# QualityMinds/cistgcn

Measured on AMD Instinct MI355X. Metric: sequences/sec (fwd+bwd) H3.6M 22-joint 50->25, higher is better.
Workload: dtype f32; 1 GPU; cistgcn64_b256_t50_v22; C=64, per_gpu_batch=256, global_batch=256, T_in=50, T_out=25, V=22, parallelism=dp1, graph=True, graph_branches=True, capture_kept=median, mixed_batches=False

## Files before the change

cistgcn_amd/_lib.py:

```python
import ctypes
import os
from ctypes import POINTER, c_double, c_float, c_int, c_int32, c_longlong, c_uint, c_ulonglong, c_void_p

HERE = os.path.dirname(os.path.abspath(__file__))
LIB_PATH = os.path.join(HERE, "libcistgcn_hip.so")

_handle = None
STAT_REPLICAS = 16
ALPHA_SLOTS = 64
_host_pointers_ok = False


class View4(ctypes.Structure):
    _fields_ = [("n", c_longlong * 4), ("s", c_longlong * 4)]


class NormAct(ctypes.Structure):
    _fields_ = [
        ("x", c_void_p), ("xv", View4),
        ("y", c_void_p), ("yv", View4),
        ("pre", c_void_p),
        ("add", c_void_p), ("av", View4),
        ("add_post", c_int),
        ("bn_mode", c_int),
        ("stats", c_void_p),
        ("gamma", c_void_p), ("beta", c_void_p),
        ("running_mean", c_void_p), ("running_var", c_void_p), ("num_batches_tracked", c_void_p),
        ("momentum", c_float), ("eps", c_float),
        ("save_mean", c_void_p), ("save_rstd", c_void_p),
        ("drop_p", c_float), ("seed", c_void_p), ("salt", c_uint),
        ("alpha", c_void_p), ("alpha_n", c_int),
        ("dy", c_void_p), ("dyv", View4),
        ("dx", c_void_p), ("dxv", View4),
        ("dadd", c_void_p), ("dav", View4),
        ("dpre", c_void_p),
        ("red", c_void_p),
        ("dgamma", c_void_p), ("dbeta", c_void_p), ("dalpha", c_void_p),
        ("ystats", c_void_p),
    ]


class ContractDesc(ctypes.Structure):
    _fields_ = [("A", c_void_p), ("X", c_void_p), ("Y", c_void_p), ("bias", c_void_p), ("stats", c_void_p), ("tab", c_void_p),
                ("G", c_int), ("M", c_int), ("N", c_int), ("K", c_int), ("splitk", c_int), ("kchunk", c_int),
                ("a_kfast", c_int), ("x_kfast", c_int), ("accumulate", c_int), ("x_vec", c_int), ("stat_ch", c_int), ("mode", c_int), ("block0", c_longlong),
                ("ws", c_void_p), ("chain", c_int), ("pad2", c_int)]


class StatsArgs(ctypes.Structure):
    _fields_ = [("x", c_void_p), ("xv", View4), ("pre", c_void_p), ("stats", c_void_p)]


class SumItem(ctypes.Structure):
    _fields_ = [("a", c_void_p), ("av", View4)]


class Rank1(ctypes.Structure):
    _fields_ = [("s", c_void_p), ("q", c_void_p), ("o", c_void_p), ("dout", c_void_p), ("ds", c_void_p), ("dq", c_void_p),
                ("domain", c_int), ("pad", c_int)]


class CopyItem(ctypes.Structure):
    _fields_ = [("y", c_void_p), ("yv", View4), ("a", c_void_p), ("av", View4)]


class TailBN(ctypes.Structure):
    _fields_ = [("stats", c_void_p), ("gamma", c_void_p), ("beta", c_void_p), ("running_mean", c_void_p), ("running_var", c_void_p),
                ("num_batches_tracked", c_void_p), ("momentum", c_float), ("eps", c_float), ("save", c_void_p)]


class DstdTail(ctypes.Structure):
    _fields_ = [("B", c_int), ("C", c_int), ("T", c_int), ("V", c_int), ("train", c_int), ("pad0", c_int),
                ("y", c_void_p * 2), ("r", c_void_p * 2), ("w", c_void_p * 2),
                ("bn_t", TailBN * 2), ("alpha_d", c_void_p * 2),
                ("bn_p", TailBN * 2), ("alpha_p", c_void_p * 2),
                ("Wc", c_void_p), ("bn_c", TailBN), ("alpha_c", c_void_p),
                ("gate", c_void_p), ("bres", c_void_p),
                ("drop_p", c_float), ("salt", c_uint * 2), ("pad1", c_int), ("seed", c_void_p),
                ("h0", c_void_p), ("pooled", c_void_p), ("out", c_void_p), ("ostats", c_void_p),
                ("tap_x", c_void_p * 2), ("tap_a", c_void_p * 2), ("tap_h", c_void_p),
                ("dout", c_void_p), ("dpooled", c_void_p), ("dgate", c_void_p), ("red_c", c_void_p),
                ("gp", c_void_p * 2), ("red_p", c_void_p * 2), ("dWc_ws", c_void_p), ("dWc", c_void_p),
                ("dr", c_void_p * 2), ("dw", c_void_p * 2), ("red_t", c_void_p * 2), ("dy", c_void_p * 2),
                ("dgamma_t", c_void_p * 2), ("dbeta_t", c_void_p * 2), ("dalpha_d", c_void_p * 2),
                ("dgamma_p", c_void_p * 2), ("dbeta_p", c_void_p * 2), ("dalpha_p", c_void_p * 2),
                ("dgamma_c", c_void_p), ("dbeta_c", c_void_p), ("dalpha_c", c_void_p)]


class AdjTail(ctypes.Structure):
    _fields_ = [("B", c_int), ("Kc", c_int), ("J", c_int), ("domain", c_int), ("train", c_int), ("pad0", c_int),
                ("s", c_void_p), ("q", c_void_p), ("W0", c_void_p), ("bn", TailBN), ("alpha", c_void_p), ("W4", c_void_p),
                ("drop_p", c_float), ("salt", c_uint), ("seed", c_void_p),
                ("e", c_void_p), ("adj", c_void_p), ("tap", c_void_p),
                ("dadj", c_void_p), ("g", c_void_p), ("red", c_void_p), ("ds", c_void_p), ("dq", c_void_p), ("part", c_void_p),
                ("dW0_ws", c_void_p), ("dW4_ws", c_void_p),
                ("dW0", c_void_p), ("dW4", c_void_p), ("dgamma", c_void_p), ("dbeta", c_void_p), ("dalpha", c_void_p)]


class PwMaps(ctypes.Structure):
    _fields_ = [("B", c_int), ("Cin", c_int), ("P", c_int), ("n", c_int), ("x", c_void_p),
                ("W", c_void_p * 4), ("M", c_int * 4), ("y", c_void_p * 4), ("stats", c_void_p * 4),
                ("dy", c_void_p * 4), ("dx", c_void_p), ("dW", c_void_p * 4), ("dW_ws", c_void_p),
                ("bias", c_void_p * 4), ("db", c_void_p * 4),
                ("yraw", c_void_p * 4), ("bn_save", c_void_p * 4), ("bn_gamma", c_void_p * 4), ("bn_beta", c_void_p * 4),
                ("bn_red", c_void_p * 4), ("prelu", c_void_p * 4), ("bn_train", c_int), ("pad", c_int)]


class FpnConv(ctypes.Structure):
    _fields_ = [("B", c_int), ("C", c_int), ("O", c_int), ("H", c_int), ("W", c_int), ("n", c_int), ("dil", c_int * 3), ("pad", c_int),
                ("x", c_void_p), ("xs", c_longlong * 3), ("w", c_void_p * 3), ("bias", c_void_p * 3), ("y", c_void_p * 3),
                ("dy", c_void_p * 3), ("dx", c_void_p), ("dw", c_void_p * 3), ("db", c_void_p * 3), ("ws", c_void_p)]


class RowsConv(ctypes.Structure):
    _fields_ = [("B", c_int), ("C", c_int), ("T", c_int), ("V", c_int), ("O", c_int), ("pad", c_int),
                ("x", c_void_p), ("W", c_void_p), ("y", c_void_p), ("stats", c_void_p),
                ("dy", c_void_p), ("dx", c_void_p), ("dW", c_void_p), ("ws", c_void_p),
                ("in_on", c_int), ("in_train", c_int), ("in_bn", TailBN), ("in_alpha", c_void_p), ("in_tap", c_void_p),
                ("sums", c_void_p), ("red", c_void_p), ("dgamma", c_void_p), ("dbeta", c_void_p), ("dalpha", c_void_p)]


class BlockInput(ctypes.Structure):
    _fields_ = [("B", c_int), ("C", c_int), ("T", c_int), ("V", c_int), ("train", c_int), ("ng", c_int),
                ("x", c_void_p), ("bn", TailBN), ("xn", c_void_p), ("rm", c_void_p), ("rq", c_void_p), ("out", c_void_p),
                ("g", c_void_p * 8), ("dout", c_void_p * 2), ("dout_ld", c_longlong * 2), ("pq", c_void_p), ("gsum", c_void_p), ("red", c_void_p),
                ("dx", c_void_p), ("dgamma", c_void_p), ("dbeta", c_void_p)]


class GatePath(ctypes.Structure):
    _fields_ = [("z", c_void_p), ("stats", c_void_p), ("stats_ld", c_longlong),
                ("bn2", TailBN), ("alpha2", c_void_p), ("Wl", c_void_p), ("bn3", TailBN), ("alpha3", c_void_p), ("W2", c_void_p),
                ("salt2", c_uint), ("salt3", c_uint), ("y", c_void_p), ("w", c_void_p), ("tap2", c_void_p), ("tap3", c_void_p),
                ("dw", c_void_p), ("dz", c_void_p), ("dstats", c_void_p), ("dWl", c_void_p), ("dW2", c_void_p),
                ("dgamma2", c_void_p), ("dbeta2", c_void_p), ("dalpha2", c_void_p), ("dgamma3", c_void_p), ("dbeta3", c_void_p), ("dalpha3", c_void_p),
                ("scratch", c_void_p), ("red", c_void_p)]


class GateHead(ctypes.Structure):
    _fields_ = [("B", c_int), ("C", c_int), ("S", c_int), ("train", c_int), ("n", c_int), ("pad", c_int),
                ("drop_p", c_float), ("pad2", c_int), ("seed", c_void_p), ("p", GatePath * 2)]


class MidItem(ctypes.Structure):
    _fields_ = [("kind", c_int), ("C", c_int), ("L", c_int), ("O", c_int), ("sb_", c_int), ("ns_", c_int),
                ("x", c_void_p), ("x_ld", c_longlong), ("bn", TailBN), ("stats_ld", c_longlong), ("alpha", c_void_p), ("W", c_void_p),
                ("salt", c_uint), ("pad", c_int), ("y", c_void_p), ("tap", c_void_p),
                ("dy", c_void_p), ("dx", c_void_p), ("dW", c_void_p), ("dgamma", c_void_p), ("dbeta", c_void_p), ("dalpha", c_void_p),
                ("g", c_void_p), ("part", c_void_p), ("wpart", c_void_p)]


class BlockMid(ctypes.Structure):
    _fields_ = [("B", c_int), ("train", c_int), ("n", c_int), ("pad", c_int),
                ("drop_p", c_float), ("pad2", c_int), ("seed", c_void_p), ("it", MidItem * 6)]


class CtxHeads(ctypes.Structure):
    _fields_ = [("B", c_int), ("P", c_int), ("C", c_int), ("train", c_int), ("x", c_void_p), ("xstats", c_void_p),
                ("w", c_void_p * 2), ("bn", TailBN * 2), ("alpha", c_void_p * 2),
                ("y", c_void_p * 2), ("arg", c_void_p), ("xsave", c_void_p), ("tap", c_void_p * 2),
                ("dy", c_void_p * 2), ("red", c_void_p), ("dx", c_void_p),
                ("dw", c_void_p * 2), ("dgamma", c_void_p * 2), ("dbeta", c_void_p * 2), ("dalpha", c_void_p * 2)]


class AttackStep(ctypes.Structure):
    _fields_ = [("B", c_int), ("T", c_int), ("V", c_int), ("mode", c_int), ("iterations", c_int), ("patience", c_int),
                ("epsilon", c_float), ("mu", c_float),
                ("x0", c_void_p), ("x", c_void_p), ("grad", c_void_p), ("g", c_void_p), ("mask", c_void_p), ("loss", c_void_p),
                ("best", c_void_p), ("stall", c_void_p), ("active", c_void_p), ("w", c_void_p), ("queries", c_void_p), ("n_active", c_void_p),
                ("steps", c_void_p), ("frozen_at", c_void_p)]


class DeepfoolStep(ctypes.Structure):
    _fields_ = [("B", c_int), ("T", c_int), ("To", c_int), ("V", c_int), ("patience", c_int), ("pad", c_int),
                ("x", c_void_p), ("grad", c_void_p), ("pred", c_void_p), ("mask", c_void_p), ("loss", c_void_p),
                ("best", c_void_p), ("stall", c_void_p), ("active", c_void_p), ("w", c_void_p), ("queries", c_void_p), ("n_active", c_void_p),
                ("steps", c_void_p), ("frozen_at", c_void_p)]


class EvalMetricsArgs(ctypes.Structure):
    _fields_ = [("B", c_int), ("To", c_int), ("J", c_int), ("Nb", c_int), ("frames", c_int), ("pad", c_int),
                ("pred", c_void_p), ("target", c_void_p), ("speeds", c_void_p), ("bones", c_void_p),
                ("out", c_void_p * 9), ("ws", c_void_p)]


class AttackMetricsArgs(ctypes.Structure):
    _fields_ = [("B", c_int), ("T", c_int), ("J", c_int), ("pad", c_int),
                ("adv", c_void_p), ("orig", c_void_p), ("out", c_void_p * 33), ("counts", c_void_p), ("gmax", c_void_p), ("ws", c_void_p)]


P = c_void_p
LL = c_longlong
_SIGNATURES = {
    "cg_contract": [P, P, P, P, P, P, c_int, c_int, c_int, c_int, c_int, c_int, c_int, LL, P],
    "cg_contract_many": [POINTER(ContractDesc), c_int, P],
    "cg_contract_kred_ws_floats": [c_int, c_int, c_int],
    "cg_chan_stats": [P, POINTER(View4), P, P, P],
    "cg_chan_stats_many": [POINTER(StatsArgs), c_int, P],
    "cg_norm_act_fwd_many": [POINTER(NormAct), c_int, P],
    "cg_norm_act_bwd_many": [POINTER(NormAct), POINTER(c_int), c_int, P],
    "cg_norm_act_bwd_reduce_many": [POINTER(NormAct), c_int, P],
    "cg_copy_many": [POINTER(CopyItem), c_int, P],
    "cg_chan_sum": [P, POINTER(View4), P, P],
    "cg_norm_act_fwd": [POINTER(NormAct), P],
    "cg_norm_act_bwd": [POINTER(NormAct), c_int, P],
    "cg_reduce_bc": [P, POINTER(View4), c_int, P, P, P],
    "cg_reduce_bc_bwd": [P, P, c_int, P, POINTER(View4), P],
    "cg_sum_many": [P, POINTER(View4), POINTER(SumItem), c_int, P],
    "cg_rank1_adj_fwd": [POINTER(Rank1), c_int, c_int, c_int, c_int, P],
    "cg_rank1_adj_bwd": [POINTER(Rank1), c_int, c_int, c_int, c_int, P],
    "cg_gather_joints": [P, P, P, LL, c_int, c_int, P],
    "cg_eval_scatter_mpjpe": [P, P, P, P, P, c_int, c_int, c_int, c_int, P],
    "cg_add3": [P, POINTER(View4), P, POINTER(View4), P, POINTER(View4), P, POINTER(View4), P],
    "cg_zero": [P, LL, P],
    "cg_feature_lift_fwd": [P, P, LL, LL, LL, P],
    "cg_feature_lift_bwd": [P, P, P, LL, LL, LL, P],
    "cg_dstd_stats_fwd": [P, P, c_int, c_int, c_int, c_int, P],
    "cg_dstd_stats_bwd": [P, P, P, c_int, c_int, c_int, c_int, P],
    "cg_se_gate_fwd": [P, P, P, P, c_int, c_int, c_int, P],
    "cg_se_gate_bwd": [P, P, P, P, P, P, P, P, c_int, c_int, c_int, c_int, P],
    "cg_cumsum": [P, POINTER(View4), P, POINTER(View4), c_int, P],
    "cg_mpjpe_fwd": [P, P, P, LL, P],
    "cg_mpjpe_bwd": [P, P, P, P, LL, P],
    "cg_seed_bump": [P, P],
    "cg_stgcn_domain_fwd": [P, P, P, P, P, P, c_int, c_int, c_int, c_int, c_int, c_int, P],
    "cg_stgcn_domain_bwd": [P, P, P, P, P, P, P, P, P, c_int, c_int, c_int, c_int, c_int, c_int, c_int, P],
    "cg_stgcn_domain_bwd_ws_floats": [c_int, c_int],
    "cg_stgcn_domain_planes_min_workgroups": [c_longlong],
    "cg_multi_copy": [P, P, P, P, P, c_int, P, c_int, c_float, P],
    "cg_scale": [P, LL, c_float, P],
    "cg_dstd_tail_fwd": [POINTER(DstdTail), c_int, P],
    "cg_dstd_tail_bwd": [POINTER(DstdTail), c_int, P],
    "cg_dstd_tail_ws_floats": [c_int],
    "cg_collapse_rows_fwd": [POINTER(RowsConv), P],
    "cg_collapse_rows_bwd": [POINTER(RowsConv), P],
    "cg_collapse_rows_ws_floats": [c_int, c_int, c_int],
    "cg_collapse_cols_fwd": [POINTER(RowsConv), P],
    "cg_collapse_cols_bwd": [POINTER(RowsConv), P],
    "cg_collapse_cols_supported": [c_int, c_int, c_int, c_int],
    "cg_collapse_cols_ws_floats": [c_int, c_int, c_int],
# ... 82 lines not shown
```

cistgcn_amd/csrc/dstd_tail.h:

```cpp
#pragma once

#define CG_TAIL_MAXW 8

struct CgTailBN {
  double* stats;
  const float* gamma; const float* beta;
  float* running_mean; float* running_var; long long* num_batches_tracked;
  float momentum, eps;
  float* save;
};

struct CgDstdTail {
  int B, C, T, V, train, pad0;
  const float* y[2];
  const float* r[2];
  const float* w[2];
  CgTailBN bn_t[2]; const float* alpha_d[2];
  CgTailBN bn_p[2]; const float* alpha_p[2];
  const float* Wc; CgTailBN bn_c; const float* alpha_c;
  const float* gate; const float* bres;
  float drop_p; unsigned int salt[2]; int pad1; const unsigned long long* seed;
  float* h0; float* pooled; float* out; double* ostats;
  float* tap_x[2]; float* tap_a[2]; float* tap_h;
  const float* dout; const float* dpooled; float* dgate;
  double* red_c;
  float* gp[2]; double* red_p[2];
  float* dWc_ws; float* dWc;
  float* dr[2]; float* dw[2]; double* red_t[2]; float* dy[2];
  float* dgamma_t[2]; float* dbeta_t[2]; float* dalpha_d[2];
  float* dgamma_p[2]; float* dbeta_p[2]; float* dalpha_p[2];
  float* dgamma_c; float* dbeta_c; float* dalpha_c;
};
```

cistgcn_amd/csrc/dstd_tail.hip:

```cpp
#include "cg_common.h"
#include "dstd_tail.h"
#include "cg_phase.h"
#include <stdlib.h>

HIP_DYNAMIC_SHARED(unsigned char, cg_dyn_lds)

static int cg_tail_rows(long long B, long long C, long long P) {
  long long target = (B * C * P) / 2048;
  target = target < 4096 ? 4096 : (target > 32768 ? 32768 : target);
  long long rb = target / (P > 0 ? P : 1);
  if (rb < 1) rb = 1;
  if (rb > B) rb = B;
  while (rb > 1 && C * ((B + rb - 1) / rb) < 512) rb = (rb + 1) / 2;
  return (int)rb;
}

__device__ __forceinline__ float cg_tail_x(const CgAff& at, float alpha_d, float y, float r, float keep, float& u) {
  u = cg_bn(at, y) * keep + r;
  return cg_prelu(u, alpha_d);
}

__device__ __forceinline__ float cg_tail_keep(const CgDstdTail& t, int i, unsigned long long seed, int b, int c, int p) {
  if (!(t.train && t.drop_p > 0.f)) return 1.f;
  const long long P = (long long)t.T * t.V;
  return cg_drop_scale(t.drop_p, seed, t.salt[i], ((unsigned long long)b * t.C + c) * P + p);
}

__device__ __forceinline__ void cg_tail_keep4(const CgDstdTail& t, int i, unsigned long long seed, unsigned long long idx0, float keep[4]);

__global__ void cg_tail_f1_kernel(CgDstdTail t, int rb) {
  __shared__ double red[32];
  const int i = blockIdx.z, c = blockIdx.x, b0 = blockIdx.y * rb;
  if (b0 >= t.B) return;
  const int P = t.T * t.V, nb = min(rb, t.B - b0), C = t.C;
  const int lane = threadIdx.x & 63, wave = __builtin_amdgcn_readfirstlane(threadIdx.x >> 6), nw = blockDim.x >> 6;
  const double cnt = (double)t.B * P;
  const CgAff at = cg_tail_aff(t.bn_t[i], c, C, cnt, t.train, false, blockIdx.y == 0 && threadIdx.x == 0);
  const float ad = t.alpha_d[i][0];
  const unsigned long long seed = (t.train && t.drop_p > 0.f) ? *t.seed : 0ull;
  const float* __restrict__ y = t.y[i]; const float* __restrict__ r = t.r[i];
  float* const tap = t.tap_x[i];
  double s = 0.0, q = 0.0;
  for (int br = wave; br < nb; br += nw) {
    const int b = b0 + br;
    const long long base = ((long long)b * C + c) * P;
    const float wv = t.w[i][(long long)b * C + c];
    if ((P & 3) == 0) {
      for (int p = 4 * lane; p < P; p += 256) {
        float keep[4];
        cg_tail_keep4(t, i, seed, (unsigned long long)(base + p), keep);
        const float4 y4 = *reinterpret_cast<const float4*>(y + base + p), r4 = *reinterpret_cast<const float4*>(r + base + p);
        const float yv[4] = {y4.x, y4.y, y4.z, y4.w}, rv[4] = {r4.x, r4.y, r4.z, r4.w};
        float xv[4];
#pragma unroll
        for (int j = 0; j < 4; ++j) {
          float u;
          xv[j] = cg_tail_x(at, ad, yv[j], rv[j], keep[j], u);
          const double z = (double)(wv * xv[j]);
          s += z; q += z * z;
        }
        if (tap) *reinterpret_cast<float4*>(tap + base + p) = make_float4(xv[0], xv[1], xv[2], xv[3]);
      }
    } else {
      for (int p = lane; p < P; p += 64) {
        float u;
        const float x = cg_tail_x(at, ad, y[base + p], r[base + p], cg_tail_keep(t, i, seed, b, c, p), u);
        const float z = wv * x;
        if (tap) tap[base + p] = x;
        s += (double)z; q += (double)z * (double)z;
      }
    }
  }
  s = cg_block_sum(s, red);
  q = cg_block_sum(q, red + 16);
  if (threadIdx.x == 0) {
    double* rep = t.bn_p[i].stats + (long long)(blockIdx.y % CG_STAT_REPLICAS) * 2 * C;
    atomicAdd(&rep[2 * c], s); atomicAdd(&rep[2 * c + 1], q);
  }
}

#define CG_TAIL_PT 64
#define CG_TAIL_PS (CG_TAIL_PT + 4)
#define CG_TAIL_THREADS 256
#define CG_TAIL_PT3 32
#define CG_TAIL_PS3 (CG_TAIL_PT3 + 4)
#define CG_TAIL_K3_TASKS 2

__device__ __forceinline__ void cg_tail_consts(const CgDstdTail& t, float* sK, bool backward, bool owner) {
  const int C = t.C;
  const double cnt = (double)t.B * t.T * t.V;
  for (int e = threadIdx.x; e < 2 * C; e += blockDim.x) {
    const int i = e / C, c = e - i * C;
    const CgAff at = cg_tail_aff(t.bn_t[i], c, C, cnt, t.train, backward || t.train != 0, owner);
    const CgAff ap = cg_tail_aff(t.bn_p[i], c, C, cnt, t.train, backward, owner);
    float* k = sK + 8 * e;
    k[0] = at.mean; k[1] = at.gamma * at.rstd; k[2] = at.beta; k[3] = t.alpha_d[i][0];
    k[4] = ap.mean; k[5] = ap.rstd; k[6] = ap.gamma; k[7] = ap.beta;
  }
}

struct CgTailHot {
  int C, P, train;
  float drop_p;
  unsigned int salt[2];
  float alpha_p[2];
  float* tap_a[2]; float* tap_x[2];
};
__device__ __forceinline__ CgTailHot cg_tail_hot(const CgDstdTail& t) {
  CgTailHot h;
  h.C = t.C; h.P = t.T * t.V; h.train = t.train; h.drop_p = t.drop_p;
#pragma unroll
  for (int i = 0; i < 2; ++i) {
    h.salt[i] = t.salt[i];
    h.alpha_p[i] = __builtin_bit_cast(float, __builtin_amdgcn_readfirstlane(__builtin_bit_cast(int, t.alpha_p[i][0])));
    h.tap_a[i] = t.tap_a[i]; h.tap_x[i] = t.tap_x[i];
  }
  return h;
}
__device__ __forceinline__ void cg_tail_keep4(const CgTailHot& h, int i, unsigned long long seed, unsigned long long idx0, float keep[4]) {
  if (!(h.train && h.drop_p > 0.f)) { keep[0] = keep[1] = keep[2] = keep[3] = 1.f; return; }
  const unsigned long long bits = cg_drop_bits(seed, h.salt[i], idx0 >> 2);
#pragma unroll
  for (int j = 0; j < 4; ++j) keep[j] = cg_drop_pick(bits, j, h.drop_p);
}

__device__ __forceinline__ void cg_tail_keep4(const CgDstdTail& t, int i, unsigned long long seed, unsigned long long idx0, float keep[4]) {
  if (!(t.train && t.drop_p > 0.f)) { keep[0] = keep[1] = keep[2] = keep[3] = 1.f; return; }
  const unsigned long long bits = cg_drop_bits(seed, t.salt[i], idx0 >> 2);
#pragma unroll
  for (int j = 0; j < 4; ++j) keep[j] = cg_drop_pick(bits, j, t.drop_p);
}

template <int PT>
__device__ __forceinline__ void cg_tail_act_load(const CgDstdTail& t, int b, int p0, int np, float4 yq[PT / 8], float4 rq[PT / 8], float wq[PT / 8]) {
  const int C = t.C, P = t.T * t.V;
#pragma unroll
  for (int q = 0; q < PT / 8; ++q) {
    const int i = q / (PT / 16), e = threadIdx.x + (q - i * (PT / 16)) * CG_TAIL_THREADS;
    const int c = e / (PT / 4), pp = 4 * (e - c * (PT / 4));
    yq[q] = make_float4(0.f, 0.f, 0.f, 0.f); rq[q] = yq[q]; wq[q] = 0.f;
    if (c < C && pp < np) {
      const float* yb = t.y[i] + (long long)b * C * P + p0;
      const float* rb = t.r[i] + (long long)b * C * P + p0;
      const int off = c * P + pp;
      yq[q] = *reinterpret_cast<const float4*>(yb + off); rq[q] = *reinterpret_cast<const float4*>(rb + off);
      wq[q] = t.w[i][(long long)b * C + c];
    }
  }
}

__device__ __forceinline__ float cg_tail_pre_p(float z, float mean, float rstd, float gamma, float beta) {
  const float zhat = (z - mean) * rstd;
  return gamma * zhat + beta;
}

template <int PT>
__device__ __forceinline__ void cg_tail_act_finish(const CgTailHot& t, const float* sK, unsigned long long seed, int b, int p0, int np,
                                                   const float4 yq[PT / 8], const float4 rq[PT / 8], const float wq[PT / 8], float* img, int what) {
  constexpr int PS = PT + 4;
  const int C = t.C, P = t.P;
#pragma unroll
  for (int q = 0; q < PT / 8; ++q) {
    const int i = q / (PT / 16), e = threadIdx.x + (q - i * (PT / 16)) * CG_TAIL_THREADS;
    const int c = e / (PT / 4), pp = 4 * (e - c * (PT / 4)), c2 = i * C + c;
    if (c >= C) continue;
    float val[4] = {0.f, 0.f, 0.f, 0.f};
    if (pp < np) {
      const float4 k0 = *reinterpret_cast<const float4*>(sK + 8 * c2), k1 = *reinterpret_cast<const float4*>(sK + 8 * c2 + 4);
      const long long off = ((long long)b * C + c) * P + p0 + pp;
      const float yv[4] = {yq[q].x, yq[q].y, yq[q].z, yq[q].w}, rv[4] = {rq[q].x, rq[q].y, rq[q].z, rq[q].w};
      float keep[4];
      cg_tail_keep4(t, i, seed, (unsigned long long)off, keep);
      const float wv = wq[q], ap = t.alpha_p[i];
      float xv[4];
#pragma unroll
      for (int j = 0; j < 4; ++j) {
        const float u = ((yv[j] - k0.x) * k0.y + k0.z) * keep[j] + rv[j];
        xv[j] = cg_prelu(u, k0.w);
        const float z = wv * xv[j];
        val[j] = what == 0 ? cg_prelu(cg_tail_pre_p(z, k1.x, k1.y, k1.z, k1.w), ap) : (z - k1.x) * k1.y;
      }
      if (what == 0) {
        if (t.tap_a[i]) *reinterpret_cast<float4*>(t.tap_a[i] + off) = make_float4(val[0], val[1], val[2], val[3]);
        if (!t.train && t.tap_x[i]) *reinterpret_cast<float4*>(t.tap_x[i] + off) = make_float4(xv[0], xv[1], xv[2], xv[3]);
      }
    }
    *reinterpret_cast<float4*>(img + c2 * PS + pp) = make_float4(val[0], val[1], val[2], val[3]);
  }
}

template <int PT>
__device__ __forceinline__ void cg_tail_stage_act(const CgDstdTail& t, const float* sK, unsigned long long seed, int b, int p0, int np,
                                                  float* img, int what) {
  constexpr int PS = PT + 4;
  const int C = t.C, P = t.T * t.V;
  if ((P & 3) == 0) {
#pragma unroll
    for (int i = 0; i < 2; ++i)
#pragma unroll 2
    for (int e = threadIdx.x; e < C * (PT / 4); e += CG_TAIL_THREADS) {
      const int c = e / (PT / 4), pp = 4 * (e - c * (PT / 4)), c2 = i * C + c;
      float val[4] = {0.f, 0.f, 0.f, 0.f};
      if (pp < np) {
        const int p = p0 + pp;
        const float4 k0 = *reinterpret_cast<const float4*>(sK + 8 * c2), k1 = *reinterpret_cast<const float4*>(sK + 8 * c2 + 4);
        const long long off = ((long long)b * C + c) * P + p;
        const float4 y4 = *reinterpret_cast<const float4*>(t.y[i] + off), r4 = *reinterpret_cast<const float4*>(t.r[i] + off);
        const float yv[4] = {y4.x, y4.y, y4.z, y4.w}, rv[4] = {r4.x, r4.y, r4.z, r4.w};
        float keep[4];
        cg_tail_keep4(t, i, seed, (unsigned long long)off, keep);
        const float wv = t.w[i][(long long)b * C + c], ap = t.alpha_p[i][0];
        float xv[4];
#pragma unroll
        for (int j = 0; j < 4; ++j) {
          const float u = ((yv[j] - k0.x) * k0.y + k0.z) * keep[j] + rv[j];
          xv[j] = cg_prelu(u, k0.w);
          const float z = wv * xv[j];
          val[j] = what == 0 ? cg_prelu(cg_tail_pre_p(z, k1.x, k1.y, k1.z, k1.w), ap) : (z - k1.x) * k1.y;
        }
        if (what == 0) {
          if (t.tap_a[i]) *reinterpret_cast<float4*>(t.tap_a[i] + off) = make_float4(val[0], val[1], val[2], val[3]);
          if (!t.train && t.tap_x[i]) *reinterpret_cast<float4*>(t.tap_x[i] + off) = make_float4(xv[0], xv[1], xv[2], xv[3]);
        }
      }
      *reinterpret_cast<float4*>(img + c2 * PS + pp) = make_float4(val[0], val[1], val[2], val[3]);
    }
    return;
  }
  for (int e = threadIdx.x; e < 2 * C * PT; e += CG_TAIL_THREADS) {
    const int c2 = e / PT, pp = e - c2 * PT;
    float val = 0.f;
    if (pp < np) {
      const int i = c2 / C, c = c2 - i * C, p = p0 + pp;
      const float* k = sK + 8 * c2;
      const long long off = ((long long)b * C + c) * P + p;
      const float keep = cg_tail_keep(t, i, seed, b, c, p);
      const float u = ((t.y[i][off] - k[0]) * k[1] + k[2]) * keep + t.r[i][off];
      const float z = t.w[i][(long long)b * C + c] * cg_prelu(u, k[3]);
      if (what == 0) {
        val = cg_prelu(cg_tail_pre_p(z, k[4], k[5], k[6], k[7]), t.alpha_p[i][0]);
        if (t.tap_a[i]) t.tap_a[i][off] = val;
        if (!t.train && t.tap_x[i]) t.tap_x[i][off] = cg_prelu(u, k[3]);
      }
      else val = (z - k[4]) * k[5];
    }
    img[c2 * PS + pp] = val;
  }
}

template <int MT_, int NT2_>
__global__ __launch_bounds__(CG_TAIL_THREADS, 2) void cg_tail_f2_kernel(CgDstdTail t, int tiles_per_sample, int total, int per) {
  const int C = t.C, C2 = 2 * C, CM = MT_ ? 16 * MT_ : (C + 15) & ~15, C2M = NT2_ ? 16 * NT2_ : (C2 + 15) & ~15, P = t.T * t.V;
  const int WS = C2M + 4;
  float* sAct = reinterpret_cast<float*>(cg_dyn_lds);
  float* sW = sAct + C2M * CG_TAIL_PS;
  float* sK = sW + CM * WS;
  double* sStat = reinterpret_cast<double*>(sK + 8 * C2M);
  const int tid = threadIdx.x, lane = tid & 63, wave = __builtin_amdgcn_readfirstlane(tid >> 6), l15 = lane & 15, slot = lane >> 4;
  const int wg = blockIdx.x;
  if (wg * per >= total) return;
  for (int e = tid; e < C2M * CG_TAIL_PS + CM * WS; e += CG_TAIL_THREADS) sAct[e] = 0.f;
  for (int e = tid; e < 2 * CM; e += CG_TAIL_THREADS) sStat[e] = 0.0;
  __syncthreads();
  for (int e = tid; e < C * C2; e += CG_TAIL_THREADS) { const int co = e / C2, c2 = e - co * C2; sW[co * WS + c2] = t.Wc[e]; }
  cg_tail_consts(t, sK, false, wg == 0);
  const unsigned long long seed = (t.train && t.drop_p > 0.f) ? *t.seed : 0ull;
  const CgTailHot hot = cg_tail_hot(t);
  const int MT = CM / 16;
  constexpr int nw = CG_TAIL_THREADS / 64;
  const bool vec = (P & 3) == 0;
  float4 yq[CG_TAIL_PT / 8], rq[CG_TAIL_PT / 8];
  float wq[CG_TAIL_PT / 8];
  double fsum[MT_ ? (2 * MT_ + nw - 1) / nw : 1][2];
#pragma unroll
  for (int i = 0; i < (MT_ ? (2 * MT_ + nw - 1) / nw : 1); ++i) fsum[i][0] = fsum[i][1] = 0.0;
  if (vec) {
    const int lid = wg * per, b = lid / tiles_per_sample, p0 = (lid - b * tiles_per_sample) * CG_TAIL_PT;
    cg_tail_act_load<CG_TAIL_PT>(t, b, p0, min(CG_TAIL_PT, P - p0), yq, rq, wq);
  }
  for (int it = 0; it < per; ++it) {
    const int lid = wg * per + it;
    if (lid >= total) break;
    const int b = lid / tiles_per_sample, tile = lid - b * tiles_per_sample, p0 = tile * CG_TAIL_PT, np = min(CG_TAIL_PT, P - p0);
    __syncthreads();
    if (vec) cg_tail_act_finish<CG_TAIL_PT>(hot, sK, seed, b, p0, np, yq, rq, wq, sAct, 0);
    else cg_tail_stage_act<CG_TAIL_PT>(t, sK, seed, b, p0, np, sAct, 0);
    __syncthreads();
    if (vec && it + 1 < per && lid + 1 < total) {
      const int l2 = lid + 1, b2 = l2 / tiles_per_sample, q0 = (l2 - b2 * tiles_per_sample) * CG_TAIL_PT;
      cg_tail_act_load<CG_TAIL_PT>(t, b2, q0, min(CG_TAIL_PT, P - q0), yq, rq, wq);
    }
    float* hb = t.h0 + (long long)b * C * P + p0;
    constexpr int NTASK = MT_ ? (2 * MT_ + nw - 1) / nw : 1;
    cg_f32x4 facc[NTASK][2];
    if (MT_) {
#pragma unroll
      for (int ti = 0; ti < NTASK; ++ti) facc[ti][0] = facc[ti][1] = cg_f32x4{0.f, 0.f, 0.f, 0.f};
      if (2 * MT_ >= nw || wave < 2 * MT_) {
        const int n0 = 32 * (wave & 1);
#pragma unroll
        for (int k0 = 0; k0 < 16 * NT2_; k0 += 16) {
          float b0v[4], b1v[4];
          cg_tfrag<1>(cg_tfrag_ptr<1>(sAct + n0, CG_TAIL_PS, l15, slot), CG_TAIL_PS, k0, b0v);
          cg_tfrag<1>(cg_tfrag_ptr<1>(sAct + n0 + 16, CG_TAIL_PS, l15, slot), CG_TAIL_PS, k0, b1v);
#pragma unroll
          for (int ti = 0; ti < NTASK; ++ti) {
            float av[4];
            cg_tfrag<0>(cg_tfrag_ptr<0>(sW + 16 * ((wave >> 1) + (nw / 2) * ti) * WS, WS, l15, slot), WS, k0, av);
#pragma unroll
            for (int s = 0; s < 4; ++s) {
              facc[ti][0] = __builtin_amdgcn_mfma_f32_16x16x4f32(b0v[s], av[s], facc[ti][0], 0, 0, 0);
              facc[ti][1] = __builtin_amdgcn_mfma_f32_16x16x4f32(b1v[s], av[s], facc[ti][1], 0, 0, 0);
            }
          }
        }
      }
    }
#pragma unroll
    for (int ti = 0; ti < (MT_ ? NTASK : 2); ++ti) {
      const int w = wave + nw * ti;
      if (w >= MT * 2) break;
      const int mt = w >> 1, n0 = 32 * (w & 1), n1 = n0 + 16;
      cg_f32x4 c0 = cg_f32x4{0.f, 0.f, 0.f, 0.f}, c1 = c0;
      if (MT_) { c0 = facc[MT_ ? ti : 0][0]; c1 = facc[MT_ ? ti : 0][1]; }
      else {
        const float* ap = cg_tfrag_ptr<0>(sW + 16 * mt * WS, WS, l15, slot);
        const float* bp0 = cg_tfrag_ptr<1>(sAct + n0, CG_TAIL_PS, l15, slot);
        const float* bp1 = cg_tfrag_ptr<1>(sAct + n1, CG_TAIL_PS, l15, slot);
        for (int k0 = 0; k0 < C2M; k0 += 16) {
          float av[4], b0v[4], b1v[4];
          cg_tfrag<0>(ap, WS, k0, av); cg_tfrag<1>(bp0, CG_TAIL_PS, k0, b0v); cg_tfrag<1>(bp1, CG_TAIL_PS, k0, b1v);
#pragma unroll
          for (int s = 0; s < 4; ++s) {
            c0 = __builtin_amdgcn_mfma_f32_16x16x4f32(b0v[s], av[s], c0, 0, 0, 0);
            c1 = __builtin_amdgcn_mfma_f32_16x16x4f32(b1v[s], av[s], c1, 0, 0, 0);
          }
        }
      }
      const int co = 16 * mt + l15;
      const bool cok = co < C;
      float s1 = 0.f, s2 = 0.f;
#pragma unroll
      for (int h = 0; h < 2; ++h) {
        const int pq = (h ? n1 : n0) + 4 * slot;
        const cg_f32x4 cc = h ? c1 : c0;
        if (cok && pq < np) {
          float* dst = hb + (long long)co * P + pq;
          if (vec) *reinterpret_cast<float4*>(dst) = make_float4(cc[0], cc[1], cc[2], cc[3]);
#pragma unroll
          for (int q = 0; q < 4; ++q) {
            if (pq + q < np) {
              if (!vec) dst[q] = cc[q];
              s1 += cc[q]; s2 += cc[q] * cc[q];
            }
          }
        }
      }
      if (t.train) {
        if (MT_) { fsum[MT_ ? ti : 0][0] += (double)s1; fsum[MT_ ? ti : 0][1] += (double)s2; }
        else {
          s1 += __shfl_xor(s1, 16, 64); s2 += __shfl_xor(s2, 16, 64);
          s1 += __shfl_xor(s1, 32, 64); s2 += __shfl_xor(s2, 32, 64);
          if (slot == 0 && cok) { atomicAdd(&sStat[2 * co], (double)s1); atomicAdd(&sStat[2 * co + 1], (double)s2); }
        }
      }
    }
  }
  if (t.train && MT_) {
#pragma unroll
    for (int ti = 0; ti < (MT_ ? (2 * MT_ + nw - 1) / nw : 1); ++ti) {
      const int w = wave + nw * ti, co = 16 * (w >> 1) + l15;
      if (w < MT * 2 && co < C) { atomicAdd(&sStat[2 * co], fsum[ti][0]); atomicAdd(&sStat[2 * co + 1], fsum[ti][1]); }
    }
  }
  if (t.train) {
    __syncthreads();
    double* rep = t.bn_c.stats + (long long)(blockIdx.x % CG_STAT_REPLICAS) * 2 * C;
    for (int e = tid; e < 2 * C; e += CG_TAIL_THREADS) atomicAdd(&rep[e], sStat[e]);
  }
}

__global__ void cg_tail_f3_kernel(CgDstdTail t, int rb) {
  const int c = blockIdx.x, b0 = blockIdx.y * rb, P = t.T * t.V, C = t.C;
  if (b0 >= t.B) return;
  const int nb = min(rb, t.B - b0), lane = threadIdx.x & 63, wave = __builtin_amdgcn_readfirstlane(threadIdx.x >> 6), nw = blockDim.x >> 6;
  const CgAff ac = cg_tail_aff(t.bn_c, c, C, (double)t.B * P, t.train, false, blockIdx.y == 0 && threadIdx.x == 0);
  const float alpha = t.alpha_c[0];
  for (int br = wave; br < nb; br += nw) {
    const int b = b0 + br;
    const float* __restrict__ h0 = t.h0 + ((long long)b * C + c) * P;
    float s = 0.f;
    if ((P & 3) == 0) {
      for (int p = 4 * lane; p < P; p += 256) {
        const float4 h4 = *reinterpret_cast<const float4*>(h0 + p);
        s += (cg_prelu(cg_bn(ac, h4.x), alpha) + cg_prelu(cg_bn(ac, h4.y), alpha)) + (cg_prelu(cg_bn(ac, h4.z), alpha) + cg_prelu(cg_bn(ac, h4.w), alpha));
      }
    } else {
      for (int p = lane; p < P; p += 64) s += cg_prelu(cg_bn(ac, h0[p]), alpha);
    }
    const double sd = cg_wave_sum((double)s);
    if (lane == 0) t.pooled[(long long)b * C + c] = (float)(sd / (double)P);
  }
}

__global__ void cg_tail_f4_kernel(CgDstdTail t, int rb) {
  __shared__ double red[32];
  const int c = blockIdx.x, b0 = blockIdx.y * rb;
  if (b0 >= t.B) return;
  const int P = t.T * t.V, nb = min(rb, t.B - b0), C = t.C;
  const int lane = threadIdx.x & 63, wave = __builtin_amdgcn_readfirstlane(threadIdx.x >> 6), nw = blockDim.x >> 6;
  const CgAff ac = cg_tail_aff(t.bn_c, c, C, (double)t.B * P, t.train, true, false);
  const float alpha = t.alpha_c[0];
  float* const tap = t.tap_h;
  double s = 0.0, q = 0.0;
  for (int br = wave; br < nb; br += nw) {
    const int b = b0 + br;
    const long long base = ((long long)b * C + c) * P;
    const float gate = t.gate[(long long)b * C + c];
    if ((P & 3) == 0) {
      for (int p = 4 * lane; p < P; p += 256) {
        const float4 h4 = *reinterpret_cast<const float4*>(t.h0 + base + p), r4 = *reinterpret_cast<const float4*>(t.bres + base + p);
        const float hv[4] = {h4.x, h4.y, h4.z, h4.w}, rv[4] = {r4.x, r4.y, r4.z, r4.w};
        float h[4], v[4];
#pragma unroll
        for (int j = 0; j < 4; ++j) { h[j] = cg_prelu(cg_bn(ac, hv[j]), alpha); v[j] = h[j] * gate + rv[j]; s += (double)v[j]; q += (double)v[j] * (double)v[j]; }
        if (tap) *reinterpret_cast<float4*>(tap + base + p) = make_float4(h[0], h[1], h[2], h[3]);
        *reinterpret_cast<float4*>(t.out + base + p) = make_float4(v[0], v[1], v[2], v[3]);
      }
    } else {
      for (int p = lane; p < P; p += 64) {
        const float h = cg_prelu(cg_bn(ac, t.h0[base + p]), alpha);
        if (tap) tap[base + p] = h;
        const float v = h * gate + t.bres[base + p];
        t.out[base + p] = v;
        s += (double)v; q += (double)v * (double)v;
      }
    }
  }
  if (t.ostats) {
    s = cg_block_sum(s, red);
    q = cg_block_sum(q, red + 16);
    if (threadIdx.x == 0) {
      double* rep = t.ostats + (long long)(blockIdx.y % CG_STAT_REPLICAS) * 2 * C;
      atomicAdd(&rep[2 * c], s); atomicAdd(&rep[2 * c + 1], q);
    }
  }
}

__global__ void cg_tail_k1_kernel(CgDstdTail t, int rb) {
  const int c = blockIdx.x, b0 = blockIdx.y * rb, P = t.T * t.V, C = t.C;
  if (b0 >= t.B) return;
  const int nb = min(rb, t.B - b0), lane = threadIdx.x & 63, wave = __builtin_amdgcn_readfirstlane(threadIdx.x >> 6), nw = blockDim.x >> 6;
  const CgAff ac = cg_tail_aff(t.bn_c, c, C, 0.0, t.train, true, false);
  const float alpha = t.alpha_c[0];
  for (int br = wave; br < nb; br += nw) {
    const int b = b0 + br;
    const long long base = ((long long)b * C + c) * P;
    float s = 0.f;
    if ((P & 3) == 0) {
      for (int p = 4 * lane; p < P; p += 256) {
        const float4 d4 = *reinterpret_cast<const float4*>(t.dout + base + p), h4 = *reinterpret_cast<const float4*>(t.h0 + base + p);
        s += (d4.x * cg_prelu(cg_bn(ac, h4.x), alpha) + d4.y * cg_prelu(cg_bn(ac, h4.y), alpha)) +
             (d4.z * cg_prelu(cg_bn(ac, h4.z), alpha) + d4.w * cg_prelu(cg_bn(ac, h4.w), alpha));
      }
    } else {
      for (int p = lane; p < P; p += 64) s += t.dout[base + p] * cg_prelu(cg_bn(ac, t.h0[base + p]), alpha);
    }
    const double sd = cg_wave_sum((double)s);
    if (lane == 0) t.dgate[(long long)b * C + c] = (float)sd;
  }
}

__device__ __forceinline__ float cg_tail_gc(const CgDstdTail& t, const CgAff& ac, float alpha, long long off, int b, int c, float invP, float& u) {
  u = cg_bn(ac, t.h0[off]);
  const float dh = t.dout[off] * t.gate[(long long)b * t.C + c] + t.dpooled[(long long)b * t.C + c] * invP;
  return u > 0.f ? dh : alpha * dh;
}

__global__ void cg_tail_k2_kernel(CgDstdTail t, int rb) {
  __shared__ double red[48];
  const int c = blockIdx.x, b0 = blockIdx.y * rb;
  if (b0 >= t.B) return;
  const int P = t.T * t.V, nb = min(rb, t.B - b0), C = t.C;
  const int lane = threadIdx.x & 63, wave = __builtin_amdgcn_readfirstlane(threadIdx.x >> 6), nw = blockDim.x >> 6;
  const CgAff ac = cg_tail_aff(t.bn_c, c, C, 0.0, t.train, true, false);
  const float alpha = t.alpha_c[0], invP = 1.f / (float)P;
  double s1 = 0.0, s2 = 0.0, sa = 0.0;
  for (int br = wave; br < nb; br += nw) {
    const int b = b0 + br;
    const long long base = ((long long)b * C + c) * P;
    const float gate = t.gate[(long long)b * C + c], dp = t.dpooled[(long long)b * C + c] * invP;
    if ((P & 3) == 0) {
      for (int p = 4 * lane; p < P; p += 256) {
        const float4 d4 = *reinterpret_cast<const float4*>(t.dout + base + p), h4 = *reinterpret_cast<const float4*>(t.h0 + base + p);
        const float dv[4] = {d4.x, d4.y, d4.z, d4.w}, hv[4] = {h4.x, h4.y, h4.z, h4.w};
#pragma unroll
        for (int j = 0; j < 4; ++j) {
          const float u = cg_bn(ac, hv[j]), dh = dv[j] * gate + dp;
          const float g = u > 0.f ? dh : alpha * dh;
          s1 += (double)g; s2 += (double)g * (double)((hv[j] - ac.mean) * ac.rstd);
          sa += u > 0.f ? 0.0 : (double)dh * (double)u;
        }
      }
    } else {
      for (int p = lane; p < P; p += 64) {
        float u;
        const float g = cg_tail_gc(t, ac, alpha, base + p, b, c, invP, u);
        s1 += (double)g;
        s2 += (double)g * (double)((t.h0[base + p] - ac.mean) * ac.rstd);
        if (!(u > 0.f)) sa += (double)(t.dout[base + p] * gate + dp) * (double)u;
      }
    }
  }
  s1 = cg_block_sum(s1, red); s2 = cg_block_sum(s2, red + 16); sa = cg_block_sum(sa, red + 32);
  if (threadIdx.x == 0) {
    atomicAdd(&t.red_c[2 * c], s1); atomicAdd(&t.red_c[2 * c + 1], s2); atomicAdd(&t.red_c[2 * C + ((c + 5 * (int)blockIdx.y) & (CG_ALPHA_SLOTS - 1))], sa);
  }
}

#ifdef CG_TAIL_STAMPS
__device__ unsigned long long* cg_tail_stamp_buf = nullptr;
extern "C" int cg_tail_set_stamps(void* p) { return (int)hipMemcpyToSymbol(HIP_SYMBOL(cg_tail_stamp_buf), &p, sizeof(p)); }
#define CG_TSTAMP()                                                                                     \
  do {                                                                                                  \
    if (threadIdx.x == 0 && cg_tail_stamp_buf && nst < 255) cg_tail_stamp_buf[blockIdx.x * 256 + (++nst)] = __builtin_amdgcn_s_memtime(); \
  } while (0)
#define CG_TSTAMP_END() do { if (threadIdx.x == 0 && cg_tail_stamp_buf) cg_tail_stamp_buf[blockIdx.x * 256] = nst; } while (0)
#else
#define CG_TSTAMP() do { } while (0)
#define CG_TSTAMP_END() do { } while (0)
#endif

template <int MT_, int NT2_>
__global__ __launch_bounds__(CG_TAIL_THREADS, 2) void cg_tail_k3_kernel(CgDstdTail t, int tiles_per_sample, int total, int per, int replicas) {
  const int C = t.C, C2 = 2 * C, CM = MT_ ? 16 * MT_ : (C + 15) & ~15, C2M = NT2_ ? 16 * NT2_ : (C2 + 15) & ~15, P = t.T * t.V;
  const int WS = C2M + 4;
  float* sZ = reinterpret_cast<float*>(cg_dyn_lds);
  float* sDH = sZ + C2M * CG_TAIL_PS3;
  float* sW = sDH + CM * CG_TAIL_PS3;
  float* sK = sW + CM * WS;
  float* sKc = sK + 8 * C2M;
  double* sRed = reinterpret_cast<double*>(sKc + 8 * CM);
  const int tid = threadIdx.x, lane = tid & 63, wave = __builtin_amdgcn_readfirstlane(tid >> 6), l15 = lane & 15, slot = lane >> 4, nw = CG_TAIL_THREADS / 64;
  const int wg = blockIdx.x;
  if (wg * per >= total) return;
  int nst = 0; (void)nst;
  CG_TSTAMP();
  for (int e = tid; e < C2M * CG_TAIL_PS3 + CM * CG_TAIL_PS3 + CM * WS; e += CG_TAIL_THREADS) sZ[e] = 0.f;
  for (int e = tid; e < 2 * C2M + 2; e += CG_TAIL_THREADS) sRed[e] = 0.0;
  __syncthreads();
  for (int e = tid; e < C * C2; e += CG_TAIL_THREADS) { const int co = e / C2, c2 = e - co * C2; sW[co * WS + c2] = t.Wc[e]; }
  cg_tail_consts(t, sK, true, false);
  const double cnt = (double)t.B * P;
  for (int c = tid; c < C; c += CG_TAIL_THREADS) {
    const CgAff ac = cg_tail_aff(t.bn_c, c, C, 0.0, t.train, true, false);
    float* kc = sKc + 8 * c;
    kc[0] = ac.mean; kc[1] = ac.rstd; kc[2] = ac.gamma * ac.rstd; kc[3] = ac.beta;
    kc[4] = t.train ? (float)(t.red_c[2 * c] / cnt) : 0.f; kc[5] = t.train ? (float)(t.red_c[2 * c + 1] / cnt) : 0.f;
  }
  const unsigned long long seed = (t.train && t.drop_p > 0.f) ? *t.seed : 0ull;
  const CgTailHot hot = cg_tail_hot(t);
  const bool train = t.train != 0;
  float* const gp0 = t.gp[0]; float* const gp1 = t.gp[1];
  const int MT = CM / 16, NT2 = C2M / 16;
  const float invP = 1.f / (float)P;
  cg_f32x4 wacc[CG_TAIL_MAXW];
#pragma unroll
  for (int u = 0; u < CG_TAIL_MAXW; ++u) wacc[u] = cg_f32x4{0.f, 0.f, 0.f, 0.f};
  const float alpha_c = t.alpha_c[0];
  const float alpha_p0 = t.alpha_p[0][0], alpha_p1 = t.alpha_p[1][0];
  float racc[CG_TAIL_K3_TASKS][3];
#pragma unroll
  for (int i = 0; i < CG_TAIL_K3_TASKS * 3; ++i) (&racc[0][0])[i] = 0.f;
  CG_TSTAMP();
  const bool vec = (P & 3) == 0;
  constexpr int DQ = CG_TAIL_PT3 / 16;
  float4 yq[CG_TAIL_PT3 / 8], rq[CG_TAIL_PT3 / 8];
  float wq[CG_TAIL_PT3 / 8];
  float4 h4[DQ], d4[DQ];
  float gt[DQ], dp[DQ];
  auto dh_load = [&](int b, int p0, int np) {
#pragma unroll
    for (int q = 0; q < DQ; ++q) {
      const int e = tid + q * CG_TAIL_THREADS, c = e / (CG_TAIL_PT3 / 4), pp = 4 * (e - c * (CG_TAIL_PT3 / 4));
      h4[q] = make_float4(0.f, 0.f, 0.f, 0.f); d4[q] = h4[q]; gt[q] = 0.f; dp[q] = 0.f;
      if (c < C && pp < np) {
        const long long off = ((long long)b * C + c) * P + p0 + pp;
        h4[q] = *reinterpret_cast<const float4*>(t.h0 + off); d4[q] = *reinterpret_cast<const float4*>(t.dout + off);
        gt[q] = t.gate[(long long)b * C + c]; dp[q] = t.dpooled[(long long)b * C + c];
      }
    }
  };
  if (vec) {
    const int lid = wg * per, b = lid / tiles_per_sample, p0 = (lid - b * tiles_per_sample) * CG_TAIL_PT3;
    cg_tail_act_load<CG_TAIL_PT3>(t, b, p0, min(CG_TAIL_PT3, P - p0), yq, rq, wq);
    dh_load(b, p0, min(CG_TAIL_PT3, P - p0));
  }
  for (int it = 0; it < per; ++it) {
    const int lid = wg * per + it;
    if (lid >= total) break;
    const int b = lid / tiles_per_sample, tile = lid - b * tiles_per_sample, p0 = tile * CG_TAIL_PT3, np = min(CG_TAIL_PT3, P - p0);
    __syncthreads();
    CG_TSTAMP();
    if (vec) {
      cg_tail_act_finish<CG_TAIL_PT3>(hot, sK, seed, b, p0, np, yq, rq, wq, sZ, 1);
      CG_TSTAMP();
#pragma unroll
      for (int q = 0; q < DQ; ++q) {
        const int e = tid + q * CG_TAIL_THREADS, c = e / (CG_TAIL_PT3 / 4), pp = 4 * (e - c * (CG_TAIL_PT3 / 4));
        if (c >= C) continue;
        float val[4] = {0.f, 0.f, 0.f, 0.f};
        if (pp < np) {
          const float4 kcA = *reinterpret_cast<const float4*>(sKc + 8 * c);
          const float2 kcB = *reinterpret_cast<const float2*>(sKc + 8 * c + 4);
          const float hv[4] = {h4[q].x, h4[q].y, h4[q].z, h4[q].w}, dv[4] = {d4[q].x, d4[q].y, d4[q].z, d4[q].w};
#pragma unroll
          for (int j = 0; j < 4; ++j) {
            const float u = (hv[j] - kcA.x) * kcA.z + kcA.w;
            const float dh = dv[j] * gt[q] + dp[q] * invP;
            const float g = u > 0.f ? dh : alpha_c * dh;
            val[j] = train ? kcA.z * (g - kcB.x - (hv[j] - kcA.x) * kcA.y * kcB.y) : g * kcA.z;
          }
        }
        *reinterpret_cast<float4*>(sDH + c * CG_TAIL_PS3 + pp) = make_float4(val[0], val[1], val[2], val[3]);
      }
    } else {
      cg_tail_stage_act<CG_TAIL_PT3>(t, sK, seed, b, p0, np, sZ, 1);
      CG_TSTAMP();
      for (int e = tid; e < C * CG_TAIL_PT3; e += CG_TAIL_THREADS) {
        const int c = e / CG_TAIL_PT3, pp = e - c * CG_TAIL_PT3;
        float val = 0.f;
        if (pp < np) {
          const float* kc = sKc + 8 * c;
          const long long off = ((long long)b * C + c) * P + p0 + pp;
          const float hv = t.h0[off];
          const float u = (hv - kc[0]) * kc[2] + kc[3];
          const float dh = t.dout[off] * t.gate[(long long)b * C + c] + t.dpooled[(long long)b * C + c] * invP;
          const float g = u > 0.f ? dh : alpha_c * dh;
          val = t.train ? kc[2] * (g - kc[4] - (hv - kc[0]) * kc[1] * kc[5]) : g * kc[2];
        }
        sDH[c * CG_TAIL_PS3 + pp] = val;
      }
    }
    __syncthreads();
    if (vec && it + 1 < per && lid + 1 < total) {
      const int b2 = (lid + 1) / tiles_per_sample, q0 = (lid + 1 - b2 * tiles_per_sample) * CG_TAIL_PT3;
      cg_tail_act_load<CG_TAIL_PT3>(t, b2, q0, min(CG_TAIL_PT3, P - q0), yq, rq, wq);
      dh_load(b2, q0, min(CG_TAIL_PT3, P - q0));
    }
    CG_TSTAMP();
    if (MT_) {
      constexpr int G = NT2_ >= nw ? NT2_ / nw : 1;
      static_assert(NT2_ == 0 || NT2_ % nw == 0 || (NT2_ < nw && MT_ == 1), "tile split of the four waves");
      if (NT2_ >= nw || wave < NT2_) {
#pragma unroll
        for (int k0 = 0; k0 < CG_TAIL_PT3; k0 += 16) {
          float afr[G][4];
#pragma unroll
          for (int g = 0; g < G; ++g) {
            const int n2 = g * nw + wave, c2 = 16 * n2 + l15;
            const bool cok = c2 < C2;
            const float gam = cok ? sK[8 * c2 + 6] : 0.f, bet = cok ? sK[8 * c2 + 7] : 0.f, alp = cok ? (c2 >= C ? alpha_p1 : alpha_p0) : 0.f;
            float bv[4];
            cg_tfrag<0>(cg_tfrag_ptr<0>(sZ + 16 * n2 * CG_TAIL_PS3, CG_TAIL_PS3, l15, slot), CG_TAIL_PS3, k0, bv);
#pragma unroll
            for (int s = 0; s < 4; ++s) afr[g][s] = cg_prelu(gam * bv[s] + bet, alp);
          }
#pragma unroll
          for (int mt = 0; mt < (MT_ ? MT_ : 1); ++mt) {
            float av[4];
            cg_tfrag<0>(cg_tfrag_ptr<0>(sDH + 16 * mt * CG_TAIL_PS3, CG_TAIL_PS3, l15, slot), CG_TAIL_PS3, k0, av);
#pragma unroll
            for (int g = 0; g < G; ++g)
#pragma unroll
              for (int s = 0; s < 4; ++s)
                wacc[mt * G + g] = __builtin_amdgcn_mfma_f32_16x16x4f32(av[s], afr[g][s], wacc[mt * G + g], 0, 0, 0);
          }
        }
      }
    } else {
#pragma unroll
    for (int u = 0; u < CG_TAIL_MAXW; ++u) {      const int id = u * nw + wave;
      if (id < MT * NT2) {
        const int mt = id / NT2, n2 = id - mt * NT2, c2 = 16 * n2 + l15;
        const int i = c2 >= C ? 1 : 0, c = c2 - i * C;
        const bool cok = c2 < C2;
        const float gam = cok ? sK[8 * c2 + 6] : 0.f, bet = cok ? sK[8 * c2 + 7] : 0.f, alp = cok ? (i ? alpha_p1 : alpha_p0) : 0.f;
        (void)c;
        const float* ap = cg_tfrag_ptr<0>(sDH + 16 * mt * CG_TAIL_PS3, CG_TAIL_PS3, l15, slot);
        const float* bp = cg_tfrag_ptr<0>(sZ + 16 * n2 * CG_TAIL_PS3, CG_TAIL_PS3, l15, slot);
        for (int k0 = 0; k0 < CG_TAIL_PT3; k0 += 16) {
          float av[4], bv[4];
          cg_tfrag<0>(ap, CG_TAIL_PS3, k0, av); cg_tfrag<0>(bp, CG_TAIL_PS3, k0, bv);
#pragma unroll
          for (int s = 0; s < 4; ++s) {
            const float a = cg_prelu(gam * bv[s] + bet, alp);
            wacc[u] = __builtin_amdgcn_mfma_f32_16x16x4f32(av[s], a, wacc[u], 0, 0, 0);
          }
        }
      }
    }
    }
    CG_TSTAMP();
    static_assert(CG_TAIL_PT3 == 32, "one pair of position tiles per task: task w = channel tile w");
    cg_f32x4 dacc[CG_TAIL_K3_TASKS][2];
    if (MT_) {
#pragma unroll
      for (int ti = 0; ti < CG_TAIL_K3_TASKS; ++ti) dacc[ti][0] = dacc[ti][1] = cg_f32x4{0.f, 0.f, 0.f, 0.f};
      if (NT2_ >= nw || wave < NT2_) {
#pragma unroll
        for (int k0 = 0; k0 < 16 * (MT_ ? MT_ : 1); k0 += 16) {
          float b0v[4], b1v[4];
          cg_tfrag<1>(cg_tfrag_ptr<1>(sDH, CG_TAIL_PS3, l15, slot), CG_TAIL_PS3, k0, b0v);
          cg_tfrag<1>(cg_tfrag_ptr<1>(sDH + 16, CG_TAIL_PS3, l15, slot), CG_TAIL_PS3, k0, b1v);
#pragma unroll
          for (int ti = 0; ti < CG_TAIL_K3_TASKS; ++ti) {
            if (nw * ti >= NT2_ && ti > 0) break;
            float av[4];
            cg_tfrag<1>(cg_tfrag_ptr<1>(sW + 16 * (wave + nw * ti), WS, l15, slot), WS, k0, av);
#pragma unroll
            for (int s = 0; s < 4; ++s) {
              dacc[ti][0] = __builtin_amdgcn_mfma_f32_16x16x4f32(b0v[s], av[s], dacc[ti][0], 0, 0, 0);
              dacc[ti][1] = __builtin_amdgcn_mfma_f32_16x16x4f32(b1v[s], av[s], dacc[ti][1], 0, 0, 0);
            }
          }
        }
      }
    }
#pragma unroll
    for (int ti = 0; ti < CG_TAIL_K3_TASKS; ++ti) {
      const int w = wave + nw * ti;
      if (w >= NT2 * (CG_TAIL_PT3 / 32)) break;
      const int mt = w / (CG_TAIL_PT3 / 32), n0 = 32 * (w % (CG_TAIL_PT3 / 32)), n1 = n0 + 16;
      cg_f32x4 c0 = cg_f32x4{0.f, 0.f, 0.f, 0.f}, c1 = c0;
      if (MT_) { c0 = dacc[ti][0]; c1 = dacc[ti][1]; }
      else {
        const float* ap = cg_tfrag_ptr<1>(sW + 16 * mt, WS, l15, slot);
        const float* bp0 = cg_tfrag_ptr<1>(sDH + n0, CG_TAIL_PS3, l15, slot);
        const float* bp1 = cg_tfrag_ptr<1>(sDH + n1, CG_TAIL_PS3, l15, slot);
        for (int k0 = 0; k0 < CM; k0 += 16) {
          float av[4], b0v[4], b1v[4];
          cg_tfrag<1>(ap, WS, k0, av); cg_tfrag<1>(bp0, CG_TAIL_PS3, k0, b0v); cg_tfrag<1>(bp1, CG_TAIL_PS3, k0, b1v);
#pragma unroll
          for (int s = 0; s < 4; ++s) {
            c0 = __builtin_amdgcn_mfma_f32_16x16x4f32(b0v[s], av[s], c0, 0, 0, 0);
            c1 = __builtin_amdgcn_mfma_f32_16x16x4f32(b1v[s], av[s], c1, 0, 0, 0);
          }
        }
      }
      const int c2 = 16 * mt + l15;
      const bool cok = c2 < C2;
      const int i = c2 >= C ? 1 : 0, c = cok ? c2 - i * C : 0;
      const float gam = cok ? sK[8 * c2 + 6] : 0.f, bet = cok ? sK[8 * c2 + 7] : 0.f, alp = cok ? (i ? alpha_p1 : alpha_p0) : 0.f;
      float* gpr = (i ? gp1 : gp0) + ((long long)b * C + c) * P + p0;
#pragma unroll
      for (int h = 0; h < 2; ++h) {
        const int pq = (h ? n1 : n0) + 4 * slot;
        const cg_f32x4 cc = h ? c1 : c0;
        if (cok && pq < np) {
          const float4 z4 = *reinterpret_cast<const float4*>(sZ + c2 * CG_TAIL_PS3 + pq);
          const float zh[4] = {z4.x, z4.y, z4.z, z4.w};
          float gq[4];
#pragma unroll
          for (int q = 0; q < 4; ++q) {
            const float v = gam * zh[q] + bet, da = cc[q];
            const bool in = pq + q < np;
            gq[q] = v > 0.f ? da : alp * da;
            if (in) {
              racc[ti][0] += gq[q]; racc[ti][1] += gq[q] * zh[q];
              if (!(v > 0.f)) racc[ti][2] += da * v;
            }
          }
          if (vec) *reinterpret_cast<float4*>(gpr + pq) = make_float4(gq[0], gq[1], gq[2], gq[3]);
          else {
#pragma unroll
            for (int q = 0; q < 4; ++q) if (pq + q < np) gpr[pq + q] = gq[q];
          }
        }
      }
    }
  }
  CG_TSTAMP();
#pragma unroll
  for (int ti = 0; ti < CG_TAIL_K3_TASKS; ++ti) {
    const int w = wave + nw * ti;
    if (w >= NT2 * (CG_TAIL_PT3 / 32)) break;
    const int c2 = 16 * (w / (CG_TAIL_PT3 / 32)) + l15;
    float s1 = racc[ti][0], s2 = racc[ti][1], sa = racc[ti][2];
    s1 += __shfl_xor(s1, 16, 64); s2 += __shfl_xor(s2, 16, 64); sa += __shfl_xor(sa, 16, 64);
    s1 += __shfl_xor(s1, 32, 64); s2 += __shfl_xor(s2, 32, 64); sa += __shfl_xor(sa, 32, 64);
    if (slot == 0 && c2 < C2) {
      atomicAdd(&sRed[2 * c2], (double)s1); atomicAdd(&sRed[2 * c2 + 1], (double)s2); atomicAdd(&sRed[2 * C2M + (c2 >= C ? 1 : 0)], (double)sa);
    }
  }
  __syncthreads();
  for (int e = tid; e < 2 * C2; e += CG_TAIL_THREADS) {
    const int c2 = e >> 1, i = c2 >= C ? 1 : 0, c = c2 - i * C;
    atomicAdd(&t.red_p[i][2 * c + (e & 1)], sRed[e]);
  }
  if (tid < 2) atomicAdd(&t.red_p[tid][2 * C + ((int)blockIdx.x & (CG_ALPHA_SLOTS - 1))], sRed[2 * C2M + tid]);
  float* dW = t.dWc_ws + (long long)(blockIdx.x % replicas) * C * C2;
#pragma unroll
  for (int u = 0; u < CG_TAIL_MAXW; ++u) {
    const int id = u * nw + wave;
    if (id < MT * NT2) {
      const int mt = id / NT2, n2 = id - mt * NT2;
#pragma unroll
      for (int q = 0; q < 4; ++q) {
        const int co = 16 * mt + 4 * slot + q, c2 = 16 * n2 + l15;
        if (co < C && c2 < C2) atomicAdd(&dW[co * C2 + c2], wacc[u][q]);
      }
    }
  }
  CG_TSTAMP();
  CG_TSTAMP_END();
}

__global__ void cg_tail_k4_kernel(CgDstdTail t, int rb) {
  const int i = blockIdx.z, c = blockIdx.x, b0 = blockIdx.y * rb, P = t.T * t.V;
  if (b0 >= t.B) return;
  const int nb = min(rb, t.B - b0), lane = threadIdx.x & 63, wave = __builtin_amdgcn_readfirstlane(threadIdx.x >> 6), nw = blockDim.x >> 6;
  const double cnt = (double)t.B * P;
  const CgAff at = cg_tail_aff(t.bn_t[i], c, t.C, 0.0, t.train, true, false);
  const CgAff ap = cg_tail_aff(t.bn_p[i], c, t.C, 0.0, t.train, true, false);
  const float ad = t.alpha_d[i][0], scale_p = ap.gamma * ap.rstd;
  const unsigned long long seed = (t.train && t.drop_p > 0.f) ? *t.seed : 0ull;
  float m1 = 0.f, m2 = 0.f;
  if (t.train) { m1 = (float)(t.red_p[i][2 * c] / cnt); m2 = (float)(t.red_p[i][2 * c + 1] / cnt); }
  double s1 = 0.0, s2 = 0.0, sa = 0.0;
  for (int br = wave; br < nb; br += nw) {
    const int b = b0 + br;
    const float wv = t.w[i][(long long)b * t.C + c];
    const long long base = ((long long)b * t.C + c) * P;
    float sw = 0.f;
    if ((P & 3) == 0) {
      for (int p = 4 * lane; p < P; p += 256) {
        float keep[4];
        cg_tail_keep4(t, i, seed, (unsigned long long)(base + p), keep);
        const float4 y4 = *reinterpret_cast<const float4*>(t.y[i] + base + p), r4 = *reinterpret_cast<const float4*>(t.r[i] + base + p);
        const float4 g4 = *reinterpret_cast<const float4*>(t.gp[i] + base + p);
        const float yv[4] = {y4.x, y4.y, y4.z, y4.w}, rv[4] = {r4.x, r4.y, r4.z, r4.w}, gv[4] = {g4.x, g4.y, g4.z, g4.w};
        float gd[4];
#pragma unroll
        for (int j = 0; j < 4; ++j) {
          float u;
          const float x = cg_tail_x(at, ad, yv[j], rv[j], keep[j], u);
          const float z = wv * x;
          const float dz = t.train ? scale_p * (gv[j] - m1 - (z - ap.mean) * ap.rstd * m2) : gv[j] * scale_p;
          sw += dz * x;
          const float dx = wv * dz;
          gd[j] = u > 0.f ? dx : ad * dx;
          if (!(u > 0.f)) sa += (double)dx * (double)u;
          const float gt = gd[j] * keep[j];
          s1 += (double)gt; s2 += (double)gt * (double)((yv[j] - at.mean) * at.rstd);
        }
        *reinterpret_cast<float4*>(t.dr[i] + base + p) = make_float4(gd[0], gd[1], gd[2], gd[3]);
      }
    } else {
      for (int p = lane; p < P; p += 64) {
        const float keep = cg_tail_keep(t, i, seed, b, c, p);
        float u;
        const float yv = t.y[i][base + p];
        const float x = cg_tail_x(at, ad, yv, t.r[i][base + p], keep, u);
        const float z = wv * x;
        const float g = t.gp[i][base + p];
        const float dz = t.train ? scale_p * (g - m1 - (z - ap.mean) * ap.rstd * m2) : g * scale_p;
        sw += dz * x;
        const float dx = wv * dz;
        const float gd = u > 0.f ? dx : ad * dx;
        t.dr[i][base + p] = gd;
        if (!(u > 0.f)) sa += (double)dx * (double)u;
        const float gt = gd * keep;
        s1 += (double)gt; s2 += (double)gt * (double)((yv - at.mean) * at.rstd);
      }
    }
    double swd = (double)sw;
    swd = cg_wave_sum(swd);
    if (lane == 0) t.dw[i][(long long)b * t.C + c] = (float)swd;
  }
  s1 = cg_wave_sum(s1); s2 = cg_wave_sum(s2); sa = cg_wave_sum(sa);
  if (lane == 0) {
    atomicAdd(&t.red_t[i][2 * c], s1); atomicAdd(&t.red_t[i][2 * c + 1], s2);
    atomicAdd(&t.red_t[i][2 * t.C + ((c + 5 * (int)blockIdx.y + 17 * wave) & (CG_ALPHA_SLOTS - 1))], sa);
  }
}

__global__ void cg_tail_k5_kernel(CgDstdTail t, int rb) {
  const int i = blockIdx.z, c = blockIdx.x, b0 = blockIdx.y * rb;
  if (b0 >= t.B) return;
  const int P = t.T * t.V, nb = min(rb, t.B - b0), C = t.C;
  const int lane = threadIdx.x & 63, wave = __builtin_amdgcn_readfirstlane(threadIdx.x >> 6), nw = blockDim.x >> 6;
  const double cnt = (double)t.B * P;
  const CgAff at = cg_tail_aff(t.bn_t[i], c, C, 0.0, t.train, true, false);
  const unsigned long long seed = (t.train && t.drop_p > 0.f) ? *t.seed : 0ull;
  const bool train = t.train != 0;
  float m1 = 0.f, m2 = 0.f;
  if (train) { m1 = (float)(t.red_t[i][2 * c] / cnt); m2 = (float)(t.red_t[i][2 * c + 1] / cnt); }
  const float scale = at.gamma * at.rstd, rm2 = at.rstd * m2;
  const float* __restrict__ dr = t.dr[i]; const float* __restrict__ y = t.y[i]; float* __restrict__ dy = t.dy[i];
  for (int br = wave; br < nb; br += nw) {
    const int b = b0 + br;
    const long long base = ((long long)b * C + c) * P;
    if ((P & 3) == 0) {
      for (int p = 4 * lane; p < P; p += 256) {
        float keep[4];
        cg_tail_keep4(t, i, seed, (unsigned long long)(base + p), keep);
        const float4 g4 = *reinterpret_cast<const float4*>(dr + base + p);
        const float gv[4] = {g4.x, g4.y, g4.z, g4.w};
        float o[4];
        if (train) {
          const float4 y4 = *reinterpret_cast<const float4*>(y + base + p);
          const float yv[4] = {y4.x, y4.y, y4.z, y4.w};
#pragma unroll
          for (int j = 0; j < 4; ++j) o[j] = scale * (gv[j] * keep[j] - m1 - (yv[j] - at.mean) * rm2);
        } else {
#pragma unroll
          for (int j = 0; j < 4; ++j) o[j] = gv[j] * keep[j] * scale;
        }
        *reinterpret_cast<float4*>(dy + base + p) = make_float4(o[0], o[1], o[2], o[3]);
      }
    } else {
      for (int p = lane; p < P; p += 64) {
        const float gt = dr[base + p] * cg_tail_keep(t, i, seed, b, c, p);
        dy[base + p] = train ? scale * (gt - m1 - (y[base + p] - at.mean) * rm2) : gt * scale;
      }
    }
  }
  if (blockIdx.y == 0 && threadIdx.x == 0) {
    t.dgamma_t[i][c] = (float)t.red_t[i][2 * c + 1]; t.dbeta_t[i][c] = (float)t.red_t[i][2 * c];
    t.dgamma_p[i][c] = (float)t.red_p[i][2 * c + 1]; t.dbeta_p[i][c] = (float)t.red_p[i][2 * c];
    if (i == 0) { t.dgamma_c[c] = (float)t.red_c[2 * c + 1]; t.dbeta_c[c] = (float)t.red_c[2 * c]; }
    if (c == 0) {
      t.dalpha_d[i][0] = (float)cg_alpha_sum(t.red_t[i] + 2 * t.C); t.dalpha_p[i][0] = (float)cg_alpha_sum(t.red_p[i] + 2 * t.C);
      if (i == 0) t.dalpha_c[0] = (float)cg_alpha_sum(t.red_c + 2 * t.C);
    }
  }
}

__global__ void cg_tail_fold_kernel(const float* __restrict__ ws, int replicas, int n, float* __restrict__ dW) {
  const int i = blockIdx.x * blockDim.x + threadIdx.x;
  if (i >= n) return;
  float s = 0.f;
  for (int r = 0; r < replicas; ++r) s += ws[(long long)r * n + i];
  dW[i] = s;
}

#define CG_TAIL_REPLICAS 16

static int cg_tail_shape_ok(int B, int C, int T, int V) { return B > 0 && C > 0 && T > 0 && V > 0 && C <= 64 && B <= 65535; }
static dim3 cg_tail_row_grid(int B, int C, int rb) { return dim3((unsigned)C, (unsigned)((B + rb - 1) / rb), 1); }

static int cg_tail_check(const CgDstdTail* t) {
  if (!t) return CG_EARG;
  if (!cg_tail_shape_ok(t->B, t->C, t->T, t->V)) return CG_ESHAPE;
  for (int i = 0; i < 2; ++i)
    if (!t->y[i] || !t->r[i] || !t->w[i] || !t->alpha_d[i] || !t->alpha_p[i] || !t->bn_t[i].gamma || !t->bn_p[i].gamma || !t->bn_t[i].save ||
        !t->bn_p[i].save) return CG_EARG;
  if (!t->Wc || !t->bn_c.gamma || !t->bn_c.save || !t->alpha_c || !t->h0) return CG_EARG;
  if (t->train && t->drop_p > 0.f && !t->seed) return CG_EARG;
  return CG_OK;
}

extern "C" long long cg_dstd_tail_ws_floats(int C) { return (long long)CG_TAIL_REPLICAS * C * 2 * C; }

struct CgTailRanges { int tps, total, per, nwg; };
static CgTailRanges cg_tail_ranges(int B, int P, int PT) {
  CgTailRanges r;
  r.tps = (P + PT - 1) / PT; r.total = B * r.tps;
  r.per = (r.total + 511) / 512; r.nwg = (r.total + r.per - 1) / r.per;
  return r;
}

static size_t cg_tail_gemm_lds(int C, bool bwd) {
  const int CM = (C + 15) & ~15, C2M = (2 * C + 15) & ~15, WS = C2M + 4;
  size_t f = (size_t)C2M * (bwd ? CG_TAIL_PS3 : CG_TAIL_PS) + (size_t)CM * WS + (size_t)8 * C2M;
  if (bwd) f += (size_t)CM * CG_TAIL_PS3 + (size_t)8 * CM;
  return f * sizeof(float) + (bwd ? (size_t)(2 * C2M + 2) : (size_t)2 * CM) * sizeof(double) + 16;
}

extern "C" int cg_dstd_tail_geometry(int B, int C, int T, int V, int* out) {
  if (!out) return CG_EARG;
  if (!cg_tail_shape_ok(B, C, T, V)) return CG_ESHAPE;
  const int P = T * V;
  const int rb = cg_tail_rows(B, C, P);
  out[0] = rb; out[1] = (int)cg_tail_row_grid(B, C, rb).y;
  const CgTailRanges f2 = cg_tail_ranges(B, P, CG_TAIL_PT), k3 = cg_tail_ranges(B, P, CG_TAIL_PT3);
  out[2] = CG_TAIL_PT; out[3] = f2.tps; out[4] = f2.total; out[5] = f2.per; out[6] = f2.nwg;
  out[7] = CG_TAIL_PT3; out[8] = k3.tps; out[9] = k3.total; out[10] = k3.per; out[11] = k3.nwg;
  return CG_OK;
}

extern "C" int cg_dstd_tail_fwd(const CgDstdTail* t, int phase, void* stream_) {
  int st = cg_tail_check(t);
  if (st != CG_OK) return st;
  hipStream_t stream = (hipStream_t)stream_;
  const int P = t->T * t->V;
  const int rb = cg_tail_rows(t->B, t->C, P);
  const dim3 rows = cg_tail_row_grid(t->B, t->C, rb);
  if (phase == 1) {
    if (!t->train) return CG_OK;
    if (!t->bn_t[0].stats || !t->bn_t[1].stats || !t->bn_p[0].stats || !t->bn_p[1].stats) return CG_EARG;
    hipLaunchKernelGGL(cg_tail_f1_kernel, dim3(rows.x, rows.y, 2), dim3(256), 0, stream, *t, rb);
  } else if (phase == 2) {
    if (t->train && (!t->bn_p[0].stats || !t->bn_p[1].stats || !t->bn_c.stats)) return CG_EARG;
    const CgTailRanges rg = cg_tail_ranges(t->B, P, CG_TAIL_PT);
    const int tps = rg.tps, total = rg.total, per = rg.per, nwg = rg.nwg;
    const size_t lds = cg_tail_gemm_lds(t->C, false);
    const int mt = (t->C + 15) / 16, nt2 = (2 * t->C + 15) / 16;
#define CG_TAIL_F2_LAUNCH(M, N)                                                                                               \
    {                                                                                                                        \
      hipError_t e = cg_lds_limit((const void*)cg_tail_f2_kernel<M, N>, lds);                                                \
      if (e != hipSuccess) return (int)e;                                                                                    \
      hipLaunchKernelGGL((cg_tail_f2_kernel<M, N>), dim3((unsigned)nwg), dim3(CG_TAIL_THREADS), lds, stream, *t, tps, total, per); \
    }
    if (mt == 4 && nt2 == 8) CG_TAIL_F2_LAUNCH(4, 8)
    else if (mt == 2 && nt2 == 4) CG_TAIL_F2_LAUNCH(2, 4)
    else if (mt == 1 && nt2 == 2) CG_TAIL_F2_LAUNCH(1, 2)
    else if (mt == 1 && nt2 == 1) CG_TAIL_F2_LAUNCH(1, 1)
    else CG_TAIL_F2_LAUNCH(0, 0)
#undef CG_TAIL_F2_LAUNCH
  } else if (phase == 3) {
    if (!t->pooled || (t->train && !t->bn_c.stats)) return CG_EARG;
    hipLaunchKernelGGL(cg_tail_f3_kernel, rows, dim3(256), 0, stream, *t, rb);
  } else if (phase == 4) {
    if (!t->gate || !t->bres || !t->out) return CG_EARG;
    hipLaunchKernelGGL(cg_tail_f4_kernel, rows, dim3(256), 0, stream, *t, rb);
  } else return CG_EARG;
  return cg_launch_status();
}

extern "C" int cg_dstd_tail_bwd(const CgDstdTail* t, int phase, void* stream_) {
  int st = cg_tail_check(t);
  if (st != CG_OK) return st;
  if (!t->dout || !t->gate) return CG_EARG;
  hipStream_t stream = (hipStream_t)stream_;
  const int P = t->T * t->V, C = t->C;
  const int rb = cg_tail_rows(t->B, C, P);
  const dim3 rows = cg_tail_row_grid(t->B, C, rb);
  if (phase == 1) {
    if (!t->dgate) return CG_EARG;
    hipLaunchKernelGGL(cg_tail_k1_kernel, rows, dim3(256), 0, stream, *t, rb);
  } else if (phase == 2) {
    if (!t->dpooled || !t->red_c) return CG_EARG;
    hipLaunchKernelGGL(cg_tail_k2_kernel, rows, dim3(256), 0, stream, *t, rb);
  } else if (phase == 3) {
    if (!t->dpooled || !t->red_c || !t->gp[0] || !t->gp[1] || !t->red_p[0] || !t->red_p[1] || !t->dWc_ws || !t->dWc) return CG_EARG;
    const CgTailRanges rg = cg_tail_ranges(t->B, P, CG_TAIL_PT3);
    const int tps = rg.tps, total = rg.total, per = rg.per, nwg = rg.nwg;
    const size_t lds = cg_tail_gemm_lds(C, true);
    const int mt = (C + 15) / 16, nt2 = (2 * C + 15) / 16;
#define CG_TAIL_K3_LAUNCH(M, N)                                                                                               \
    {                                                                                                                        \
      hipError_t e = cg_lds_limit((const void*)cg_tail_k3_kernel<M, N>, lds);                                                \
      if (e != hipSuccess) return (int)e;                                                                                    \
      hipLaunchKernelGGL((cg_tail_k3_kernel<M, N>), dim3((unsigned)nwg), dim3(CG_TAIL_THREADS), lds, stream, *t, tps, total, per, CG_TAIL_REPLICAS); \
    }
    if (mt == 4 && nt2 == 8) CG_TAIL_K3_LAUNCH(4, 8)
    else if (mt == 2 && nt2 == 4) CG_TAIL_K3_LAUNCH(2, 4)
    else if (mt == 1 && nt2 == 2) CG_TAIL_K3_LAUNCH(1, 2)
    else if (mt == 1 && nt2 == 1) CG_TAIL_K3_LAUNCH(1, 1)
    else CG_TAIL_K3_LAUNCH(0, 0)
#undef CG_TAIL_K3_LAUNCH
    st = cg_launch_status();
    if (st != CG_OK) return st;
    const int n = C * 2 * C;
    hipLaunchKernelGGL(cg_tail_fold_kernel, dim3((unsigned)((n + 255) / 256)), dim3(256), 0, stream, t->dWc_ws, CG_TAIL_REPLICAS, n, t->dWc);
  } else if (phase == 4) {
    if (!t->gp[0] || !t->gp[1] || !t->dr[0] || !t->dr[1] || !t->dw[0] || !t->dw[1] || !t->red_t[0] || !t->red_t[1] || !t->red_p[0]) return CG_EARG;
    hipLaunchKernelGGL(cg_tail_k4_kernel, dim3(rows.x, rows.y, 2), dim3(256), 0, stream, *t, rb);
  } else if (phase == 5) {
    if (!t->dy[0] || !t->dy[1] || !t->dr[0] || !t->dr[1] || !t->red_t[0] || !t->red_t[1] || !t->dgamma_t[0] || !t->dgamma_p[0] || !t->dgamma_c) return CG_EARG;
    hipLaunchKernelGGL(cg_tail_k5_kernel, dim3(rows.x, rows.y, 2), dim3(256), 0, stream, *t, rb);
  } else return CG_EARG;
  return cg_launch_status();
}
```

cistgcn_amd/models/CISTGCN/CISTGCN.py:

```python
import torch
import torch.nn as nn

from ... import ops
from ..layers.SE import SELayer1d, SELayer2d


class Stage(nn.Module):

    def __init__(self, **slots):
        super().__init__()
        for k, m in slots.items():
            self.add_module(k.lstrip("s"), m)

    def __getitem__(self, i):
        return self._modules[str(i)]


def _conv(cin, cout, k=1, bias=False, **kw):
    return nn.Conv2d(cin, cout, k, bias=bias, **kw)


def _init_small(root, gain, convs):
    for m in root.modules():
        if isinstance(m, nn.Linear):
# ... 18 lines not shown
        self.expansor = Stage(s0=_conv(ch, ch), s1=nn.BatchNorm2d(ch), s3=nn.PReLU(), s4=_conv(ch, ch))
        for part in (self.time_compress, self.joint_compress, self.expansor):
            _init_small(part, 0.05, True)


class GraphWeights(nn.Module):

    def __init__(self, time_dim, joints_dim, domain, interpretable):
        super().__init__()
        if not interpretable:
            n, s = (time_dim, joints_dim) if domain == "time" else (joints_dim, time_dim)
            self.A = nn.Parameter(torch.empty(n, s, s).uniform_(-1.0 / s ** 0.5, 1.0 / s ** 0.5))


class DomainLayer(nn.Module):

    def __init__(self, cin, cout, time_dim, joints_dim, domain, interpretable):
        super().__init__()
        self.domain, self.interpretable = domain, bool(interpretable)
        self.gcn = GraphWeights(time_dim, joints_dim, domain, interpretable)
        self.tcn = Stage(s0=_conv(cin, cout, bias=True), s1=nn.BatchNorm2d(cout))
        self.residual = Stage(s0=_conv(cin, cout, bias=True), s1=nn.BatchNorm2d(cout)) if cin != cout else nn.Identity()
        self.map_to_adj = Map2Adj(cin, time_dim, joints_dim, domain) if interpretable else nn.Identity()
        self.prelu = nn.PReLU()


class DSTDBlock(nn.Module):

    def __init__(self, cin, cout, interpretable, time_dim, joints_dim, reduction):
        super().__init__()
        self.dsgn = DomainLayer(cin, cout, time_dim, joints_dim, "space", interpretable)
        self.tsgn = DomainLayer(cin, cout, time_dim, joints_dim, "time", interpretable)
        self.compressor = Stage(s0=_conv(2 * cout, cout), s1=nn.BatchNorm2d(cout), s2=nn.PReLU(),
                                s3=SELayer2d(cout, reduction=reduction))
        self.residual = Stage(s0=_conv(cin, cout, bias=True), s1=nn.BatchNorm2d(cout)) if cin != cout else nn.Identity()
        mid = max(1, cout // 2)
        self.global_norm = nn.BatchNorm2d(cin)
        def gate_conv():
            return Stage(s0=_conv(cin, mid, (time_dim, 1)), s1=nn.BatchNorm2d(mid), s3=nn.PReLU(),
                         s4=_conv(mid, cout, (1, joints_dim)), s5=nn.BatchNorm2d(cout), s7=nn.PReLU())
        def gate_map():
            return Stage(s0=nn.Linear(cout + 2 + 2 * time_dim, cout, bias=False), s1=nn.BatchNorm1d(cout), s3=nn.PReLU(),
                         s4=nn.Linear(cout, cout, bias=False))
        self.conv_s, self.conv_t = gate_conv(), gate_conv()
        self.map_s, self.map_t = gate_map(), gate_map()
        self.prelu1 = Stage(s0=nn.BatchNorm2d(cout), s1=nn.PReLU())
        self.prelu2 = Stage(s0=nn.BatchNorm2d(cout), s1=nn.PReLU())


class FPN(nn.Module):

    def __init__(self, cin, cout, k):
        super().__init__()
        if k != 3:
            raise ValueError("txc_kernel_size %d is not supported by the MI355X path (reference YAMLs use 3)" % k)
        for i, d in enumerate((1, 2, 3)):
            self.add_module("block%d" % (i + 1), Stage(s0=_conv(cin, cout, 3, bias=True, padding=d, dilation=d),
                                                       s1=nn.BatchNorm2d(cout), s3=nn.PReLU()))
        self.compress = _conv(3 * cout + cin, cout, bias=True)


class ContextLayer(nn.Module):

    def __init__(self, hidden, out_seq, joints, reduction):
        super().__init__()
        def ctx_conv(k):
            return Stage(s0=_conv(1, hidden, k), s1=nn.BatchNorm2d(hidden), s2=nn.PReLU())
        self.context_conv1, self.context_conv2, self.context_conv3 = ctx_conv(1), ctx_conv((out_seq, 1)), ctx_conv(1)
        def head():
            return Stage(s0=nn.Linear(hidden, out_seq, bias=False), s2=nn.PReLU())
        self.map1, self.map2, self.map3 = head(), head(), head()
        self.fmap_s = Stage(s0=nn.Linear(3 * out_seq, joints, bias=False), s1=nn.BatchNorm1d(joints))
        self.fmap_t = Stage(s0=nn.Linear(3 * out_seq, out_seq, bias=False), s1=nn.BatchNorm1d(out_seq))
        self.norm_map = Stage(s0=nn.Conv1d(out_seq, out_seq, 1, bias=False), s1=nn.BatchNorm1d(out_seq), s3=nn.PReLU(),
                              s4=SELayer1d(out_seq, reduction=reduction),
                              s5=nn.Conv1d(out_seq, out_seq, 1, bias=False), s6=nn.BatchNorm1d(out_seq), s8=nn.PReLU())
        self.fconv = Stage(s0=_conv(1, 3), s1=nn.BatchNorm2d(3), s2=nn.PReLU(), s3=_conv(3, 3), s4=nn.BatchNorm2d(3), s5=nn.PReLU())
        self.SE = SELayer2d(out_seq, reduction=reduction)


def _pointwise(x, conv, stats=False):
    w = conv.weight.view(conv.out_channels, conv.in_channels)
    if x.dim() == 4 and x.shape[0] * x.shape[2] * x.shape[3] >= _PWM_MIN_POSITIONS and ops.pointwise_maps_ok(x, [w]):
        return ops.pointwise_maps(x, [w], stats, biases=[conv.bias])[0]
    spec = "oc,bchw->bohw" if x.dim() == 4 else "oc,bcv->bov"
    bl = "o" if conv.bias is not None else None
    return ops.contract_stats(spec, w, x, conv.bias, bl) if stats else (ops.contract(spec, w, x, conv.bias, bl), None)


_PWM_MIN_POSITIONS = 32768


def _collapse_rows(x, conv, stats=False):
    w = conv.weight.view(conv.out_channels, conv.in_channels, x.shape[2])
    y, st = ops.contract_stats("och,bchw->bow", w, x) if stats else (ops.contract("och,bchw->bow", w, x), None)
    return y.view(y.shape[0], y.shape[1], 1, y.shape[2]), st


def _collapse_cols(x, conv, stats=False):
    w = conv.weight.view(conv.out_channels, conv.in_channels, x.shape[3])
    y, st = ops.contract_stats("ocw,bchw->boh", w, x) if stats else (ops.contract("ocw,bchw->boh", w, x), None)
    return y.view(y.shape[0], y.shape[1], y.shape[2], 1), st


def _linear(x, lin, stats=False):
    return ops.contract_stats("oi,bi->bo", lin.weight, x) if stats else (ops.contract("oi,bi->bo", lin.weight, x), None)


def _pw_item(x, conv, stats):
    w = conv.weight.view(conv.out_channels, conv.in_channels)
    spec = "oc,bchw->bohw" if x.dim() == 4 else "oc,bcv->bov"
    return (spec, w, x, conv.bias, "o" if conv.bias is not None else None, "o" if stats else None), None


def _rows_item(x, conv, stats):
    w = conv.weight.view(conv.out_channels, conv.in_channels, x.shape[2])
    return ("och,bchw->bow", w, x, None, None, "o" if stats else None), (lambda y: y.view(y.shape[0], y.shape[1], 1, y.shape[2]))


def _cols_item(x, conv, stats):
    w = conv.weight.view(conv.out_channels, conv.in_channels, x.shape[3])
    return ("ocw,bchw->boh", w, x, None, None, "o" if stats else None), (lambda y: y.view(y.shape[0], y.shape[1], y.shape[2], 1))


def _lin_item(x, lin, stats):
    return ("oi,bi->bo", lin.weight, x, None, None, "o" if stats else None), None


def _run_items(items):
    outs = ops.contract_many([it for it, _ in items])
    return [((post(y) if post is not None else y), st) for (y, st), (_, post) in zip(outs, items)]


class CISTGCN(nn.Module):

    def __init__(self, arch, learn):
        super().__init__()
        p = arch.model_params
        self.clipping = p.clipping
        self.n_input, self.n_output, self.n_joints = p.input_n, p.output_n, p.joints
        self.n_txcnn_layers = p.n_txcnn_layers
        self.txc_kernel_size = [p.txc_kernel_size] * 2
        self.input_gcn, self.output_gcn = p.input_gcn, p.output_gcn
        self.reduction, self.hidden_dim = p.reduction, p.hidden_dim
        self.dropout = float(learn.dropout)
        self.in_ch = 10
        self.fused_domain = True
        self.staged = True
        self.fused_tail = True
        self.fused_adj = True
        self.fused_maps = True
        self.fused_defer = True
        self.fused_mid = True
        self.stack_min_elements = 1 << 21
        widths = [self.in_ch] + list(p.input_gcn.model_complexity) + [self.in_ch]
        widths_o = [3] + list(p.output_gcn.model_complexity)
        T, V, To = self.n_input, self.n_joints, self.n_output

        self.st_gcnns = nn.ModuleList()
        self.txcnns = nn.ModuleList()
        self.se = nn.ModuleList()
        self.in_conv = nn.ModuleList()
        self.context_layer = nn.ModuleList()
        self.trans = nn.ModuleList()
        for i in range(len(widths) - 1):
            self.st_gcnns.append(DSTDBlock(widths[i], widths[i + 1], p.input_gcn.interpretable[i], T, V, self.reduction))
        self.context_layer = ContextLayer(self.hidden_dim, To, V, self.reduction)
        self.txcnns.append(FPN(T, To, p.txc_kernel_size))
        for _ in range(1, self.n_txcnn_layers):
            self.txcnns.append(FPN(To, To, p.txc_kernel_size))
        self.prelus = nn.ModuleList(nn.PReLU() for _ in range(self.n_txcnn_layers))
        self.dim_conversor = Stage(s0=_conv(self.in_ch, 3), s1=nn.BatchNorm2d(3), s2=nn.PReLU(), s3=_conv(3, 3), s4=nn.PReLU(3))
        self.st_gcnns_o = nn.ModuleList()
        for i in range(len(widths_o) - 1):
            self.st_gcnns_o.append(DSTDBlock(widths_o[i], widths_o[i + 1], p.output_gcn.interpretable[i], V, To, self.reduction))
        for part in (self.st_gcnns_o, self.st_gcnns, self.txcnns):
            _init_small(part, 0.1, False)
        self._site = 0
        self.backward_cut = None
        self.act_trace = None
        self.drop_trace = None
        self.branch_streams = False
        self._streams, self._next_stream = [], 0

    def _parallel(self, thunks, inputs):
        if not (self.branch_streams and inputs[0].is_cuda) or len(thunks) < 2:
            return [t() for t in thunks]
        cur = torch.cuda.current_stream()
        while len(self._streams) < len(thunks) - 1:
            self._streams.append(torch.cuda.Stream(device=inputs[0].device))
        results = []
        for t, s in zip(thunks[:-1], self._streams):
            s.wait_stream(cur)
            with torch.cuda.stream(s):
                results.append(t())
        results.append(thunks[-1]())
        for s in self._streams[:len(thunks) - 1]:
            cur.wait_stream(s)
        return results

    def _na(self, x, bn=None, prelu=None, drop=False, **kw):
        return self._na_many([dict(x=x, bn=bn, prelu=prelu, drop=drop, **kw)])[0]

    def _lin(self, fn, x, layer, bn=True):
        return fn(x, layer, stats=bn and self.training)

    def _adjacency(self, layer, x):
        m = layer.map_to_adj
        B, _, T, V = x.shape

        def tower(t, collapse):
            h = self._na(self._lin(_pointwise, x, t[0]), bn=t[1], prelu=t[2])
            h = self._na(self._lin(collapse, h, t[3]), bn=t[4], drop=True)
            return _pointwise(h, t[6])[0]

        q, s = self._parallel([lambda: tower(m.time_compress, _collapse_rows), lambda: tower(m.joint_compress, _collapse_cols)], [x])
        q, s = q.view(B, T, V), s.view(B, V, T)
        if layer.domain == "space":
            o = ops.contract("bvt,bxv->bvtx", s, q)
        else:
            o = ops.contract("bvt,btw->btvw", s, q)
        e = m.expansor
        h = self._na(self._lin(_pointwise, o, e[0]), bn=e[1], drop=True, prelu=e[3])
        return _pointwise(h, e[4])[0]

    def _fused_stage_ok(self, conv):
        return self.fused_domain and conv.in_channels <= 128 and conv.out_channels <= 128

    def _domain(self, layer, xn):
        res = xn if isinstance(layer.residual, nn.Identity) else self._na(self._lin(_pointwise, xn, layer.residual[0]), bn=layer.residual[1])
        conv = layer.tcn[0]
        if layer.interpretable:
            adj = self._adjacency(layer, xn)
            layer.Adj = adj
            if self._fused_stage_ok(conv):
                w = conv.weight.view(conv.out_channels, conv.in_channels)
                y = ops.stgcn_domain(xn, adj, w, conv.bias, 0 if layer.domain == "space" else 1, self.training)
            else:
                spec = "bctv,bvtq->bcqv" if layer.domain == "space" else "bctv,btvw->bctw"
                y = self._lin(_pointwise, ops.contract(spec, xn, adj), conv)
        else:
            layer.Adj = xn
            spec = "bctv,vtq->bcqv" if layer.domain == "space" else "bctv,tvw->bctw"
            y = self._lin(_pointwise, ops.contract(spec, xn, layer.gcn.A), conv)
        return self._na(y, bn=layer.tcn[1], drop=True, add=res, prelu=layer.prelu)

    def _gate(self, conv, mp, xn, stats):
        h = self._na(self._lin(_collapse_rows, xn, conv[0]), bn=conv[1], drop=True, prelu=conv[3])
        h = self._na(self._lin(_collapse_cols, h, conv[4]), bn=conv[5], drop=True, prelu=conv[7])
        h = ops.cat_channels([h.view(h.shape[0], -1), stats])
        h = self._na(self._lin(_linear, h, mp[0]), bn=mp[1], drop=True, prelu=mp[3])
        return _linear(h, mp[4])[0]

    def _block(self, m, x):
        xn = self._na(x, bn=m.global_norm)
        stats = ops.dstd_stats(xn)
        m.w1, m.w2, x1, x2 = self._parallel([lambda: self._gate(m.conv_s, m.map_s, xn, stats),
                                             lambda: self._gate(m.conv_t, m.map_t, xn, stats),
                                             lambda: self._domain(m.dsgn, xn), lambda: self._domain(m.tsgn, xn)], [xn, stats])
        a = self._na(x1, pre=m.w1, bn=m.prelu1[0], prelu=m.prelu1[1])
        b = self._na(x2, pre=m.w2, bn=m.prelu2[0], prelu=m.prelu2[1])
        c = m.compressor
        h = self._na(self._lin(_pointwise, ops.cat_channels([a, b]), c[0]), bn=c[1], prelu=c[2])
        gate = ops.se_gate(ops.mean_bc(h), c[3].w1, c[3].w2)
        res = xn if isinstance(m.residual, nn.Identity) else self._na(self._lin(_pointwise, xn, m.residual[0]), bn=m.residual[1])
        return self._na(h, pre=gate, add=res, add_post=True)

    def _na_many(self, calls):
        out = []
        for kw in calls:
            kw = dict(kw)
            self._site += 1
            drop = kw.pop("drop", False)
            kw.update(train=self.training, drop_p=self.dropout if drop else 0.0, salt=self._site)
            if drop and self.drop_trace is not None:
                self.drop_trace[kw.get("bn") if kw.get("bn") is not None else kw.get("prelu")] = self._site
            out.append(kw)
        ys = ops.norm_act_many(out)
        if self.act_trace is not None:
            for kw, y in zip(out, ys):
                if kw.get("prelu") is not None:
                    y = y[0] if isinstance(y, tuple) else y
                    add = kw.get("add") if kw.get("add_post") else None
                    self.act_trace[kw["prelu"]] = (y.detach(), add.detach() if add is not None else None)
        return ys

    @staticmethod
    def _map_groups(x, ws):
        groups, rows = [], 0
        for i, w in enumerate(ws):
            if not ops.pointwise_maps_ok(x, [w]):
                return None
            r = (w.shape[0] + 15) // 16 * 16
            if not groups or rows + r > 128 or len(groups[-1]) == 4:
                groups.append([])
                rows = 0
            groups[-1].append(i)
            rows += r
        return groups

    def _block_staged(self, m, x):
        tr = self.training
        doms = (m.dsgn, m.tsgn)
        if not all(d.interpretable for d in doms):
            return self._block(m, x)
        x_in, x_sums = x if isinstance(x, tuple) else (x, None)
# ... 132 lines not shown
        if res_done is not None:
            self._site += len(res_done)
            r = r + res_done
        gs, gt, t1 = r[0], r[1], r[2:6]
        res = r[6:8] if has_res else x_res
        bres = r[-1] if has_bres else x_bres
        items = [] if mid_g else [_cols_item(gs, m.conv_s[4], tr), _cols_item(gt, m.conv_t[4], tr)]
        rows3, cols3 = {}, {}
        for i, a in enumerate(maps):
            c3 = a.time_compress[3]
            x3 = t1[2 * i][0] if isinstance(t1[2 * i], tuple) else t1[2 * i]
            w3 = c3.weight.view(c3.out_channels, c3.in_channels, -1)
            if big and c3.bias is None and ops.collapse_rows_ok(x3, w3):
                y3, st3 = ops.collapse_rows(x3, w3, tr, transform=tower_tr[2 * i] if tower_tr else None)
                rows3[i] = (y3.unsqueeze(2), st3)
            else:
                assert tower_tr is None, "a deferred tower map needs its collapsing kernel"
                items.append(_rows_item(t1[2 * i], c3, tr))
            c4 = a.joint_compress[3]
            x4 = t1[2 * i + 1][0] if isinstance(t1[2 * i + 1], tuple) else t1[2 * i + 1]
            w4 = c4.weight.view(c4.out_channels, c4.in_channels, -1)
            if big and c4.bias is None and ops.collapse_cols_ok(x4, w4):
                y4, st4 = ops.collapse_cols(x4, w4, tr, transform=tower_tr[2 * i + 1] if tower_tr else None)
                cols3[i] = (y4.unsqueeze(3), st4)
            else:
                assert tower_tr is None, "a deferred tower map needs its collapsing kernel"
                items.append(_cols_item(t1[2 * i + 1], c4, tr))
        if tower_tr and self.act_trace is not None:
            tp_ = [b_ for a_ in maps for b_ in (a_.time_compress[2], a_.joint_compress[2])]
            for mod, tr_ in zip(tp_, tower_tr):
                self.act_trace[mod] = (tr_["tap"].detach(), None)
        o = ([None, None] if mid_g else []) + (_run_items(items) if items else [])
        if rows3 or cols3:
            rest, o = o[2:], o[:2]
            for i in range(len(maps)):
                o.append(rows3[i] if i in rows3 else rest.pop(0))
                o.append(cols3[i] if i in cols3 else rest.pop(0))
        Cg = m.conv_s[4].out_channels
        gate_fused = mid_g or (o[0][0].shape[1] == Cg and o[0][0].numel() == B * Cg and
                               ops.gate_head_ok(B, Cg, stats_s.shape[1], (m.conv_s[7], m.conv_t[7], m.map_s[3], m.map_t[3])))
        tower_calls = []
        for i, a in enumerate(maps):
            tower_calls += [dict(x=o[2 + 2 * i], bn=a.time_compress[4], drop=True), dict(x=o[3 + 2 * i], bn=a.joint_compress[4], drop=True)]
        tower_mid = [(a.time_compress, a.joint_compress)[k] for a in maps for k in (0, 1)]
        mid_t = (mid_on and gate_fused and len(rows3) == len(maps) and len(cols3) == len(maps) and all(c[6].bias is None for c in tower_mid)
                 and ops.block_mid_ok(B, [(1, o[2 + k][0].shape[1], o[2 + k][0].numel() // (B * o[2 + k][0].shape[1]), c[6].out_channels, None)
                                          for k, c in enumerate(tower_mid)]))
        if gate_fused:
            s2 = (self._site + 1, self._site + 2)
            self._site += 2
            if mid_t:
                tower_salts = tuple(self._site + 1 + k for k in range(len(tower_mid)))
                self._site += len(tower_mid)
                if self.drop_trace is not None:
                    for c, salt in zip(tower_mid, tower_salts):
                        self.drop_trace[c[4]] = salt
                r = [None] * (2 + len(tower_mid))
            else:
                r = [None, None] + self._na_many(tower_calls)
            s3 = (self._site + 1, self._site + 2)
            self._site += 2
            if self.drop_trace is not None:
                self.drop_trace[m.conv_s[5]], self.drop_trace[m.conv_t[5]], self.drop_trace[m.map_s[1]], self.drop_trace[m.map_t[1]] = s2[0], s2[1], s3[0], s3[1]
            mid_out = []
            if mid_g or mid_t:
                mitems = []
                if mid_g:
                    for i, cv in enumerate((m.conv_s, m.conv_t)):
                        mitems.append(dict(kind=0, x=mid_x[i], bn=cv[1], prelu=cv[3], weight=cv[4].weight.view(Cg, -1, V), salt=mid_salts[i],
                                           stats=(gate_sums, i * mid_x[i].shape[1], 2 * mid_x[i].shape[1]) if tr else None))
                if mid_t:
                    for k, c in enumerate(tower_mid):
                        y, st = o[2 + k]
                        mitems.append(dict(kind=1, x=y.view(B, y.shape[1], -1), bn=c[4], prelu=None, weight=c[6].weight.view(c[6].out_channels, y.shape[1]),
                                           salt=tower_salts[k], stats=(st, 0, y.shape[1]) if tr else None))
                mtaps = [] if self.act_trace is not None else None
                mid_out = ops.block_mid(mitems, tr, drop_p=self.dropout, taps=mtaps)
                if mid_g:
                    o[0], o[1] = (mid_out[0], None), (mid_out[1], None)
                    mid_out = mid_out[2:]
                    if mtaps is not None:
                        self.act_trace[m.conv_s[3]], self.act_trace[m.conv_t[3]] = (mtaps[0].unsqueeze(2), None), (mtaps[1].unsqueeze(2), None)
            taps = [] if self.act_trace is not None else None
            m.w1, m.w2 = ops.gate_head([o[0][0].view(B, Cg), o[1][0].view(B, Cg)], [stats_s, stats_t], [m.conv_s, m.conv_t], [m.map_s, m.map_t], tr,
                                       drop_p=self.dropout, salts=((s2[0], s3[0]), (s2[1], s3[1])), taps=taps)
            if taps is not None:
                self.act_trace[m.conv_s[7]], self.act_trace[m.map_s[3]] = (taps[0], None), (taps[1], None)
                self.act_trace[m.conv_t[7]], self.act_trace[m.map_t[3]] = (taps[2], None), (taps[3], None)
            items, g = [], None
        else:
            calls = [dict(x=o[0], bn=m.conv_s[5], drop=True, prelu=m.conv_s[7]), dict(x=o[1], bn=m.conv_t[5], drop=True, prelu=m.conv_t[7])]
            r = self._na_many(calls + tower_calls)
            hs = ops.cat_channels([r[0].view(B, -1), stats_s])
            ht = ops.cat_channels([r[1].view(B, -1), stats_t])
            items = [_lin_item(hs, m.map_s[0], tr), _lin_item(ht, m.map_t[0], tr)]
        if mid_t:
            o = [(y, None) for y in mid_out]
        else:
            for i, a in enumerate(maps):
                items += [_pw_item(r[2 + 2 * i], a.time_compress[6], False), _pw_item(r[3 + 2 * i], a.joint_compress[6], False)]
            o = _run_items(items)
        if gate_fused:
            o = [None, None] + o
        else:
            g = self._na_many([dict(x=o[0], bn=m.map_s[1], drop=True, prelu=m.map_s[3]), dict(x=o[1], bn=m.map_t[1], drop=True, prelu=m.map_t[3])])
        seeds = []
        for i, d in enumerate(doms):
            q, s = o[2 + 2 * i][0].view(B, T, V), o[3 + 2 * i][0].view(B, V, T)
            seeds.append((0 if d.domain == "space" else 1, s, q))
        if adj_fused:
            if not gate_fused:
                o = _run_items([_lin_item(g[0], m.map_s[4], False), _lin_item(g[1], m.map_t[4], False)])
                m.w1, m.w2 = o[0][0], o[1][0]
            self._site += 2
            if self.drop_trace is not None:
                self.drop_trace[maps[0].expansor[1]], self.drop_trace[maps[1].expansor[1]] = self._site - 1, self._site
            taps = [] if self.act_trace is not None else None
            adj = ops.map2adj_tail(seeds, [a.expansor for a in maps], tr, drop_p=self.dropout, salts=(self._site - 1, self._site), taps=taps)
            adj = [(a, None) for a in adj]
            if taps is not None:
                for a, tap in zip(maps, taps):
                    self.act_trace[a.expansor[3]] = (tap, None)
        else:
            if T <= 64 and V <= 64:
                oo = ops.rank1_adj(seeds)
            else:
                oo = [y for y, _ in ops.contract_many([("bvt,bxv->bvtx" if dom == 0 else "bvt,btw->btvw", s, q, None, None, None)
                                                       for dom, s, q in seeds])]
            items = [] if gate_fused else [_lin_item(g[0], m.map_s[4], False), _lin_item(g[1], m.map_t[4], False)]
            items += [_pw_item(oo[i], a.expansor[0], tr) for i, a in enumerate(maps)]
            o = _run_items(items)
            if gate_fused:
                o = [None, None] + o
            else:
                m.w1, m.w2 = o[0][0], o[1][0]
            e = self._na_many([dict(x=o[2 + i], bn=a.expansor[1], drop=True, prelu=a.expansor[3]) for i, a in enumerate(maps)])
            adj = _run_items([_pw_item(e[i], a.expansor[4], False) for i, a in enumerate(maps)])
        ys = []
        for i, d in enumerate(doms):
            d.Adj = adj[i][0]
            conv = d.tcn[0]
            if self._fused_stage_ok(conv):
                wmat = conv.weight.view(conv.out_channels, conv.in_channels)
                ys.append(ops.stgcn_domain(x_dom[i], d.Adj, wmat, conv.bias, 0 if d.domain == "space" else 1, tr))
            else:
                spec = "bctv,bvtq->bcqv" if d.domain == "space" else "bctv,btvw->bctw"
                ys.append(self._lin(_pointwise, ops.contract(spec, x_dom[i], d.Adj), conv))
        c = m.compressor
        if self.fused_tail and c[0].out_channels <= 64 and all(isinstance(y, tuple) and (y[1] is not None or not tr) for y in ys):
            self._site += 2
            if self.drop_trace is not None:
                self.drop_trace[doms[0].tcn[1]], self.drop_trace[doms[1].tcn[1]] = self._site - 1, self._site
            taps = [] if self.act_trace is not None else None
            out, ost = ops.dstd_tail([y[0] for y in ys], [y[1] for y in ys], res, (m.w1, m.w2),
                                     (doms[0].tcn[1], doms[1].tcn[1], m.prelu1[0], m.prelu2[0], c[1]),
                                     (doms[0].prelu, doms[1].prelu, m.prelu1[1], m.prelu2[1], c[2]), c[0].weight, c[3], bres, tr,
                                     drop_p=self.dropout, salts=(self._site - 1, self._site), emit_stats=tr, taps=taps)
            if taps is not None:
                for mod, tap in zip((doms[0].prelu, doms[1].prelu, m.prelu1[1], m.prelu2[1], c[2]), taps):
                    self.act_trace[mod] = (tap, None)
            self._site += 4
            return (out, ost) if tr else out
        x12 = self._na_many([dict(x=ys[i], bn=d.tcn[1], drop=True, add=res[i], prelu=d.prelu) for i, d in enumerate(doms)])
        ab = self._na_many([dict(x=x12[0], pre=m.w1, bn=m.prelu1[0], prelu=m.prelu1[1]),
                            dict(x=x12[1], pre=m.w2, bn=m.prelu2[0], prelu=m.prelu2[1])])
        h = self._na(self._lin(_pointwise, ops.cat_channels(ab), c[0]), bn=c[1], prelu=c[2])
        h_pool, h = ops.fanout(h, 2)
        gate = ops.se_gate(ops.mean_bc(h_pool), c[3].w1, c[3].w2)
        return self._na(h, pre=gate, add=bres, add_post=True, emit_stats=tr)

    def _fpn(self, m, x, x_pool=None):
        blocks = (m.block1, m.block2, m.block3)
        ys = ops.dilated_convs(x, [b[0] for b in blocks])
        outs = self._na_many([dict(x=y, bn=b[1], prelu=b[3]) for y, b in zip(ys, blocks)])
        outs.append(ops.mean_bc(x if x_pool is None else x_pool))
        return _pointwise(ops.cat_channels(outs, bcast=(False, False, False, True)), m.compress)[0]

    def _context(self, m, x7):
        B, To, V, _ = x7.shape
        x = x7.view(B, 1, To, V * 3)
        c1, c2, c3 = m.context_conv1, m.context_conv2, m.context_conv3
        tr = self.training
        w13 = [c[0].weight.view(c[0].out_channels, c[0].in_channels) for c in (c1, c3)]
        if c1[0].bias is None and c3[0].bias is None and ops.context_heads_ok(x, c1[0].out_channels):
            xa, xb = ops.fanout(x, 2)
            taps = [] if self.act_trace is not None else None
            y1, ym = ops.context_heads(xa, c1, c3, tr, taps=taps)
            if taps is not None:
                self.act_trace[c1[2]], self.act_trace[c3[2]] = (taps[0], None), (taps[1], None)
            y2 = ops.max_bc(self._na(_run_items([_rows_item(xb, c2[0], tr)])[0], bn=c2[1], prelu=c2[2]))
            self._site += 2
            return self._context_tail(m, x7, y1, y2, ym)
        if self.fused_maps and B * To * V * 3 * sum(w.shape[0] for w in w13) >= self.stack_min_elements and ops.pointwise_maps_ok(x, w13):
            xa, xb = ops.fanout(x, 2)
            y13 = ops.pointwise_maps(xa, w13, tr, biases=[c1[0].bias, c3[0].bias])
            o = [y13[0], _run_items([_rows_item(xb, c2[0], tr)])[0], y13[1]]
        else:
            o = _run_items([_pw_item(x, c1[0], tr), _rows_item(x, c2[0], tr), _pw_item(x, c3[0], tr)])
        r = self._na_many([dict(x=o[i], bn=c[1], prelu=c[2]) for i, c in enumerate((c1, c2, c3))])
        return self._context_tail(m, x7, ops.max_bc(r[0]), ops.max_bc(r[1]), ops.mean_bc(r[2]))

    def _context_tail(self, m, x7, y1, y2, ym):
        B, To, V, _ = x7.shape
        tr = self.training
        o = _run_items([_lin_item(y, h[0], False) for y, h in ((y1, m.map1), (y2, m.map2), (ym, m.map3))])
        heads = self._na_many([dict(x=o[i][0], drop=True, prelu=h[2]) for i, h in enumerate((m.map1, m.map2, m.map3))])
        y = ops.cat_channels(heads)
        o = _run_items([_lin_item(y, m.fmap_s[0], tr), _lin_item(y, m.fmap_t[0], tr)])
        m.joints, m.displacements = self._na_many([dict(x=o[0], bn=m.fmap_s[1], drop=True), dict(x=o[1], bn=m.fmap_t[1], drop=True)])
        m.seq_joints = ops.contract("bt,bv->btv", m.displacements, m.joints)
        n = m.norm_map
        h = self._na(self._lin(_pointwise, m.seq_joints, n[0]), bn=n[1], drop=True, prelu=n[3])
        h_pool, h = ops.fanout(h, 2)
        h = self._na(h, pre=ops.se_gate(ops.mean_bc(h_pool), n[4].w1, n[4].w2))
        h = self._na(self._lin(_pointwise, h, n[5]), bn=n[6], drop=True, prelu=n[8])
        m.seq_joints_n = h
        f = m.fconv
        h = self._na(self._lin(_pointwise, h.view(B, 1, To, V), f[0]), bn=f[1], prelu=f[2])
        h = self._na(self._lin(_pointwise, h, f[3]), bn=f[4], prelu=f[5])
        m.seq_joints_dims = h
        hp_pool, hp = ops.fanout(h.permute(0, 2, 3, 1), 2)
        return self._na(hp, pre=ops.se_gate(ops.mean_bc(hp_pool), m.SE.w1, m.SE.w2))

    def forward(self, x):
        if x.dim() != 4 or x.shape[1] != self.n_input or x.shape[2] != self.n_joints or x.shape[3] != 3:
            raise ValueError("expected input of shape (B, %d, %d, 3), got %s" % (self.n_input, self.n_joints, tuple(x.shape)))
        if torch.jit.is_tracing():
            net = self

            class HotPath(torch.autograd.Function):
                @staticmethod
                def forward(ctx, inp):
                    state = torch._C._get_tracing_state()
                    torch._C._set_tracing_state(None)
                    try:
                        with torch.no_grad():
                            return net._forward(inp.detach(), bump_seed=False)[0]
                    finally:
                        torch._C._set_tracing_state(state)

                @staticmethod
                def backward(ctx, g):
                    raise RuntimeError("the traced CISTGCN graph is for display only")

            return HotPath.apply(x),
        return self._forward(x, bump_seed=self.training and self.dropout > 0.0)

    def _forward(self, x, bump_seed):
        ops.begin_step(x.device, bump_seed=bump_seed)
        self._site, self._next_stream = 0, 0
        h = ops.feature_lift(x)
        block = self._block_staged if self.staged else self._block
        for i, blk in enumerate(self.st_gcnns):
            h = block(blk, h)
            if self.backward_cut is not None and self.backward_cut[0] == i:
                h = self.backward_cut[1](h)
        h = h[0] if isinstance(h, tuple) else h
        h = h.permute(0, 2, 1, 3)
        ha = ops.fanout(h, 2)
        z = self._na(self._fpn(self.txcnns[0], ha[0], ha[1]), prelu=self.prelus[0])
        for i in range(1, self.n_txcnn_layers):
            za = ops.fanout(z, 3)
            z = self._na(self._fpn(self.txcnns[i], za[0], za[1]), prelu=self.prelus[i], add=za[2], add_post=True)
        d = self.dim_conversor
        z = self._na(self._lin(_pointwise, z.permute(0, 2, 1, 3), d[0]), bn=d[1], prelu=d[2])
        z = self._na(_pointwise(z, d[3])[0], prelu=d[4])
        x7, x7o = ops.fanout(ops.cumsum_time(z.permute(0, 2, 3, 1)), 2)
        def output_blocks():
            x8 = x7o.permute(0, 3, 2, 1)
            for blk in self.st_gcnns_o:
                x8 = block(blk, x8)
            return x8[0] if isinstance(x8, tuple) else x8
        act, x8 = self._parallel([lambda: self._context(self.context_layer, x7), output_blocks], [x7])
        return ops.add3(x[:, -1:], x8.permute(0, 3, 2, 1), act),
```

cistgcn_amd/ops.py:

```python
import ctypes
import os

import numpy as np
import torch

from . import _lib
from ._lib import NormAct, View4

_vp = ctypes.c_void_p


def _ptr(t):
    return _vp(t.data_ptr()) if t is not None else None


def _stream(t):
    if t.is_cuda:
        return _vp(torch.cuda.current_stream(t.device).cuda_stream)
    if not _lib._host_pointers_ok:
        raise RuntimeError("cistgcn_amd operators run on MI355X only: got a %s tensor (no CPU path exists)" % t.device)
    return None


def _chk(t, name="tensor"):
# ... 1451 lines not shown
        if t.dim() != 4 or t.shape != x.shape or t.shape[-1] != 3 or not t.is_contiguous():
            raise ValueError("attack_step: %s must be a contiguous (B,T,V,3) tensor like x, got %s" % (name, tuple(t.shape)))
    B, T, V, _ = x.shape
    a = _lib.AttackStep()
    a.B, a.T, a.V, a.mode, a.iterations, a.patience = B, T, V, m, int(iterations), int(patience)
    a.epsilon, a.mu = float(epsilon), float(mu)
    a.x0, a.x, a.grad = _ptr(x0), _ptr(x), _ptr(grad)
    if mask is not None:
        _chk(mask, "mask")
        if tuple(mask.shape) != (T, V) or not mask.is_contiguous():
            raise ValueError("attack_step: mask must be a contiguous (T,V) tensor, got %s" % (tuple(mask.shape),))
        a.mask = _ptr(mask)
    if m == 2:
        if g is None or g.shape != x.shape or g.dtype != torch.float32 or not g.is_contiguous():
            raise ValueError("attack_step: MI-FGSM needs its momentum g, float32 and shaped like x")
        a.g = _ptr(g)
    if m != 0:
        if loss is None or state is None or loss.numel() != B or state.B != B or loss.dtype != torch.float32 or not loss.is_contiguous():
            raise ValueError("attack_step: the iterative modes need loss (B,) and an AttackState of the same batch")
        a.loss, a.best, a.stall, a.active = _ptr(loss), _ptr(state.best), _ptr(state.stall), _ptr(state.active)
        a.w, a.queries, a.n_active = _ptr(state.w), _ptr(state.queries), _ptr(state.n_active)
        a.steps, a.frozen_at = _ptr(state.steps), _ptr(state.frozen_at)
    _lib.call("cg_attack_step", ctypes.byref(a), _stream(x))
    return x


def deepfool_step(x, grad, pred, mask=None, loss=None, state=None, patience=5):
    for t, name in ((x, "x"), (grad, "grad")):
        if t.dtype != torch.float32 or t.dim() != 4 or t.shape != x.shape or t.shape[-1] != 3 or not t.is_contiguous():
            raise ValueError("deepfool_step: %s must be a contiguous float32 (B,T,V,3) tensor like x, got %s %s" % (name, t.dtype, tuple(t.shape)))
    B, T, V, _ = x.shape
    if pred.dtype != torch.float32 or pred.dim() != 4 or pred.shape[0] != B or pred.shape[3] != 3 or not pred.is_contiguous():
        raise ValueError("deepfool_step: pred must be a contiguous float32 (B,To,V,3) tensor, got %s %s" % (pred.dtype, tuple(pred.shape)))
    if pred.shape[2] != V:
        raise ValueError("deepfool_step: the prediction's joints are broadcast onto the input's, so both need the same V: got %d and %d"
                         % (pred.shape[2], V))
    if min(B, T, V, pred.shape[1]) < 1:
        raise ValueError("deepfool_step: empty operand, x %s pred %s" % (tuple(x.shape), tuple(pred.shape)))
    for t, name in ((grad, "grad"), (pred, "pred"), (mask, "mask"), (loss, "loss")):
        if t is not None and t.device != x.device:
            raise ValueError("deepfool_step: x is on %s, %s on %s" % (x.device, name, t.device))
    a = _lib.DeepfoolStep()
    a.B, a.T, a.To, a.V, a.patience = B, T, pred.shape[1], V, int(patience)
    a.x, a.grad, a.pred = _ptr(x), _ptr(grad), _ptr(pred)
    if mask is not None:
        if mask.dtype != torch.float32 or tuple(mask.shape) != (T, V) or not mask.is_contiguous():
            raise ValueError("deepfool_step: mask must be a contiguous float32 (T,V) tensor, got %s %s" % (mask.dtype, tuple(mask.shape)))
        a.mask = _ptr(mask)
    if (loss is None) != (state is None):
        raise ValueError("deepfool_step: loss (B,) and an AttackState go together")
    if state is not None:
        if loss.numel() != B or state.B != B or loss.dtype != torch.float32 or not loss.is_contiguous():
            raise ValueError("deepfool_step: loss must be a contiguous float32 (B,) tensor and the AttackState of the same batch")
        a.loss, a.best, a.stall, a.active = _ptr(loss), _ptr(state.best), _ptr(state.stall), _ptr(state.active)
        a.w, a.queries, a.n_active = _ptr(state.w), _ptr(state.queries), _ptr(state.n_active)
        a.steps, a.frozen_at = _ptr(state.steps), _ptr(state.frozen_at)
    _lib.call("cg_deepfool_step", ctypes.byref(a), _stream(x))
    return x


class _StgcnDomain(torch.autograd.Function):
    @staticmethod
    def forward(ctx, x, adj, w, bias, domain, want_stats):
        ctx.set_materialize_grads(False)
        if not (x.is_contiguous() and adj.is_contiguous() and w.is_contiguous()):
            raise ValueError("stgcn_domain expects contiguous x (B,C,T,V), Adj and W")
        B, Cin, T, V = x.shape
        Cout = w.shape[0]
        exp = (B, V, T, T) if domain == 0 else (B, T, V, V)
        if tuple(adj.shape) != exp or w.numel() != Cout * Cin:
            raise ValueError("stgcn_domain: adjacency %s / weight %s do not match x %s" % (tuple(adj.shape), tuple(w.shape), tuple(x.shape)))
        y = torch.empty(B, Cout, T, V, dtype=torch.float32, device=x.device)
        stats = _arena(x.device).take(2 * Cout * _lib.STAT_REPLICAS) if want_stats else None
        _lib.call("cg_stgcn_domain_fwd", _ptr(x), _ptr(adj), _ptr(w), _ptr(bias), _ptr(y), _ptr(stats),
                  B, Cin, Cout, T, V, domain, _stream(x))
        ctx.domain = domain
        ctx.save_for_backward(x, adj, w)
        if want_stats:
            ctx.mark_non_differentiable(stats)
            return y, stats
        return y, None

    @staticmethod
    def backward(ctx, dy, _):
        x, adj, w = ctx.saved_tensors
        B, Cin, T, V = x.shape
        Cout = w.shape[0]
        dy = dy if dy.is_contiguous() else _copy(dy)
        dx = torch.empty_like(x)
        dadj = torch.empty_like(adj)
        dw = torch.empty_like(w)
        db = torch.empty(Cout, dtype=torch.float32, device=x.device)
        ws, _ = _zeros(_lib.lib().cg_stgcn_domain_bwd_ws_floats(Cin, Cout), x.device)
        _lib.call("cg_stgcn_domain_bwd", _ptr(x), _ptr(adj), _ptr(w), _ptr(dy), _ptr(dx), _ptr(dadj), _ptr(dw), _ptr(db),
                  _ptr(ws), B, Cin, Cout, T, V, ctx.domain, 1, _stream(x))
        return dx, dadj, dw, db, None, None


def stgcn_domain(x, adj, w, bias, domain, want_stats=False):
    return _StgcnDomain.apply(x, adj, w, bias, domain, want_stats)


def _tail_bn(dst, bn, stats, save, train):
    dst.stats = stats.data_ptr() if stats is not None else None
    dst.gamma, dst.beta = bn.weight.data_ptr(), bn.bias.data_ptr()
    dst.running_mean, dst.running_var = bn.running_mean.data_ptr(), bn.running_var.data_ptr()
    dst.num_batches_tracked = bn.num_batches_tracked.data_ptr() if train else None
    dst.momentum, dst.eps = bn.momentum, bn.eps
    dst.save = save.data_ptr()


class _DstdTail(torch.autograd.Function):

    @staticmethod
    def forward(ctx, cfg, *ts):
        ctx.set_materialize_grads(False)
        (y1, y2, r1, r2, w1, w2, gt1, bt1, ad1, gt2, bt2, ad2, gp1, bp1, ap1, gp2, bp2, ap2, wc, gc, bc, ac, sw1, sw2, bres) = ts
        for t in (y1, y2, r1, r2, w1, w2, bres):
            _chk(t)
            if not t.is_contiguous():
                raise ValueError("dstd_tail expects contiguous tensors")
        B, C, T, V = y1.shape
        dev, train = y1.device, bool(cfg["train"])
        f32 = torch.float32
        t = _lib.DstdTail()
        t.B, t.C, t.T, t.V, t.train = B, C, T, V, 1 if train else 0
        saves = torch.empty(5, 2, C, dtype=f32, device=dev)
        t.y[0], t.y[1], t.r[0], t.r[1], t.w[0], t.w[1] = (v.data_ptr() for v in (y1, y2, r1, r2, w1, w2))
        arena = _arena(dev)
        zst = [arena.take(2 * C * _lib.STAT_REPLICAS) for _ in range(2)] if train else [None, None]
        hst = arena.take(2 * C * _lib.STAT_REPLICAS) if train else None
        bns = cfg["bn"]
        _tail_bn(t.bn_t[0], bns[0], cfg["ystats"][0], saves[0], train); _tail_bn(t.bn_t[1], bns[1], cfg["ystats"][1], saves[1], train)
        _tail_bn(t.bn_p[0], bns[2], zst[0], saves[2], train); _tail_bn(t.bn_p[1], bns[3], zst[1], saves[3], train)
        _tail_bn(t.bn_c, bns[4], hst, saves[4], train)
        t.alpha_d[0], t.alpha_d[1], t.alpha_p[0], t.alpha_p[1] = ad1.data_ptr(), ad2.data_ptr(), ap1.data_ptr(), ap2.data_ptr()
        t.Wc, t.alpha_c, t.bres = wc.data_ptr(), ac.data_ptr(), bres.data_ptr()
        p = float(cfg.get("drop_p", 0.0)) if train else 0.0
        t.drop_p = p
        if p > 0.0:
            t.seed = seed_state(dev).data_ptr()
        t.salt[0], t.salt[1] = cfg["salts"]
        h0 = torch.empty(B, C, T, V, dtype=f32, device=dev)
        pooled = torch.empty(B, C, dtype=f32, device=dev)
        out = torch.empty(B, C, T, V, dtype=f32, device=dev)
        ostats = arena.take(2 * C * _lib.STAT_REPLICAS) if cfg.get("emit_stats") else None
        t.h0, t.pooled, t.out, t.ostats = h0.data_ptr(), pooled.data_ptr(), out.data_ptr(), _ptr(ostats)
        taps = cfg.get("taps")
        if taps is not None:
            for k in range(5):
                taps.append(torch.empty(B, C, T, V, dtype=f32, device=dev))
            t.tap_x[0], t.tap_x[1], t.tap_a[0], t.tap_a[1], t.tap_h = (v.data_ptr() for v in taps[-5:])
        stream = _stream(y1)
        for phase in (1, 2, 3):
            _lib.call("cg_dstd_tail_fwd", ctypes.byref(t), phase, stream)
        gate = torch.empty(B, C, dtype=f32, device=dev)
        H = sw1.shape[0]
        _lib.call("cg_se_gate_fwd", _ptr(pooled), _ptr(sw1), _ptr(sw2), _ptr(gate), B, C, H, stream)
        t.gate = gate.data_ptr()
        _lib.call("cg_dstd_tail_fwd", ctypes.byref(t), 4, stream)
        ctx.cfg, ctx.p = cfg, p
        ctx.seed_epoch = seed_epoch(dev) if p > 0.0 else None
        ctx.save_for_backward(*ts, h0, pooled, gate, saves)
        if ostats is not None:
            ctx.mark_non_differentiable(ostats)
        return out, ostats

    @staticmethod
    def backward(ctx, dout, _=None):
        sv = ctx.saved_tensors
        (y1, y2, r1, r2, w1, w2, gt1, bt1, ad1, gt2, bt2, ad2, gp1, bp1, ap1, gp2, bp2, ap2, wc, gc, bc, ac, sw1, sw2, bres) = sv[:25]
        h0, pooled, gate, saves = sv[25:]
        cfg = ctx.cfg
        _check_seed_epoch(ctx, y1.device, "dstd_tail")
        B, C, T, V = y1.shape
        dev, train, f32 = y1.device, bool(cfg["train"]), torch.float32
        dout = dout if dout.is_contiguous() else _copy(dout)
        t = _lib.DstdTail()
        t.B, t.C, t.T, t.V, t.train = B, C, T, V, 1 if train else 0
        t.y[0], t.y[1], t.r[0], t.r[1], t.w[0], t.w[1] = (v.data_ptr() for v in (y1, y2, r1, r2, w1, w2))
        bns = cfg["bn"]
        for dst, bn, k in ((t.bn_t[0], bns[0], 0), (t.bn_t[1], bns[1], 1), (t.bn_p[0], bns[2], 2), (t.bn_p[1], bns[3], 3), (t.bn_c, bns[4], 4)):
            _tail_bn(dst, bn, None, saves[k], False)
        t.alpha_d[0], t.alpha_d[1], t.alpha_p[0], t.alpha_p[1] = ad1.data_ptr(), ad2.data_ptr(), ap1.data_ptr(), ap2.data_ptr()
        t.Wc, t.alpha_c, t.bres, t.gate, t.h0 = wc.data_ptr(), ac.data_ptr(), bres.data_ptr(), gate.data_ptr(), h0.data_ptr()
        t.drop_p = ctx.p
        if ctx.p > 0.0:
            t.seed = seed_state(dev).data_ptr()
        t.salt[0], t.salt[1] = cfg["salts"]
        t.dout = dout.data_ptr()
        stream = _stream(y1)
        dgate = torch.empty(B, C, dtype=f32, device=dev)
        t.dgate = dgate.data_ptr()
        _lib.call("cg_dstd_tail_bwd", ctypes.byref(t), 1, stream)
        H = sw1.shape[0]
        dpooled = torch.empty(B, C, dtype=f32, device=dev)
        ws_floats = int(_lib.lib().cg_dstd_tail_ws_floats(C))
        zb, _ = _zeros(2 * C * H + ws_floats, dev)
        dsw1, dsw2 = zb[:C * H].view(sw1.shape), zb[C * H:2 * C * H].view(sw2.shape)
        _lib.call("cg_se_gate_bwd", _ptr(pooled), _ptr(sw1), _ptr(sw2), _ptr(gate), _ptr(dgate), _ptr(dpooled), _ptr(dsw1), _ptr(dsw2),
                  B, C, H, 1, stream)
        arena = _arena(dev)
        red_c = arena.take(2 * C + _lib.ALPHA_SLOTS)
        red_p = [arena.take(2 * C + _lib.ALPHA_SLOTS) for _ in range(2)]
        red_t = [arena.take(2 * C + _lib.ALPHA_SLOTS) for _ in range(2)]
        big = [torch.empty(B, C, T, V, dtype=f32, device=dev) for _ in range(6)]
        dws = [torch.empty(B, C, dtype=f32, device=dev) for _ in range(2)]
        small = torch.empty(15, C, dtype=f32, device=dev)
        dwc = torch.empty(C, 2 * C, dtype=f32, device=dev)
        t.dpooled, t.red_c = dpooled.data_ptr(), red_c.data_ptr()
        for i in range(2):
            t.gp[i], t.red_p[i], t.dr[i], t.dw[i], t.red_t[i], t.dy[i] = (big[i].data_ptr(), red_p[i].data_ptr(), big[2 + i].data_ptr(),
                                                                          dws[i].data_ptr(), red_t[i].data_ptr(), big[4 + i].data_ptr())
            t.dgamma_t[i], t.dbeta_t[i], t.dgamma_p[i], t.dbeta_p[i] = (small[2 * i].data_ptr(), small[2 * i + 1].data_ptr(),
                                                                        small[4 + 2 * i].data_ptr(), small[5 + 2 * i].data_ptr())
            t.dalpha_d[i], t.dalpha_p[i] = small[10 + i].data_ptr(), small[12 + i].data_ptr()
        t.dgamma_c, t.dbeta_c, t.dalpha_c = small[8].data_ptr(), small[9].data_ptr(), small[14].data_ptr()
        t.dWc_ws, t.dWc = zb[2 * C * H:].data_ptr(), dwc.data_ptr()
        for phase in (2, 3, 4, 5):
            _lib.call("cg_dstd_tail_bwd", ctypes.byref(t), phase, stream)
        al = lambda k: small[k, :1].reshape(1)
        grads = (big[4], big[5], big[2], big[3], dws[0], dws[1],
                 small[0], small[1], al(10), small[2], small[3], al(11),
                 small[4], small[5], al(12), small[6], small[7], al(13),
                 dwc.view(wc.shape), small[8], small[9], al(14), dsw1, dsw2, dout)
        return (None,) + tuple(g if ctx.needs_input_grad[1 + k] else None for k, g in enumerate(grads))


def dstd_tail(ys, ystats, rs, ws, bns, alphas, wc, se, bres, train, drop_p=0.0, salts=(0, 0), emit_stats=False, taps=None):
    C = ys[0].shape[1]
    cfg = {"train": bool(train), "drop_p": float(drop_p), "salts": tuple(int(s) for s in salts), "ystats": tuple(ystats), "bn": tuple(bns),
           "emit_stats": bool(emit_stats), "taps": taps}
    ts = (ys[0], ys[1], rs[0], rs[1], ws[0], ws[1],
          bns[0].weight, bns[0].bias, alphas[0].weight, bns[1].weight, bns[1].bias, alphas[1].weight,
          bns[2].weight, bns[2].bias, alphas[2].weight, bns[3].weight, bns[3].bias, alphas[3].weight,
          wc.view(C, 2 * C), bns[4].weight, bns[4].bias, alphas[4].weight, se.w1, se.w2, bres)
    return _DstdTail.apply(cfg, *ts)


class _Map2AdjTail(torch.autograd.Function):

    @staticmethod
    def _items(cfg, ts, train, saves, stats, e, dev, p):
        n = len(ts) // 7
        items = (_lib.AdjTail * n)()
        for i in range(n):
            s, q, w0, gamma, beta, alpha, w4 = ts[7 * i:7 * i + 7]
            B, V, T = s.shape
            t = items[i]
            dom = cfg["domains"][i]
            t.B, t.domain, t.train = B, dom, 1 if train else 0
            t.Kc, t.J = (V, T) if dom == 0 else (T, V)
            t.s, t.q, t.W0, t.alpha, t.W4 = s.data_ptr(), q.data_ptr(), w0.data_ptr(), alpha.data_ptr(), w4.data_ptr()
            _tail_bn(t.bn, cfg["bn"][i], stats[i] if stats is not None else None, saves[i], train and stats is not None)
            t.drop_p, t.salt = p, cfg["salts"][i]
            if p > 0.0:
                t.seed = seed_state(dev).data_ptr()
            t.e = e[i].data_ptr()
        return items

    @staticmethod
    def forward(ctx, cfg, *ts):
        ctx.set_materialize_grads(False)
        n = len(ts) // 7
        for i in range(n):
            for t in ts[7 * i:7 * i + 2]:
                _chk(t)
                if not t.is_contiguous():
                    raise ValueError("map2adj_tail expects contiguous tower outputs")
        dev, train, f32 = ts[0].device, bool(cfg["train"]), torch.float32
        p = float(cfg.get("drop_p", 0.0)) if train else 0.0
        arena = _arena(dev)
        shapes = []
        for i in range(n):
            B, V, T = ts[7 * i].shape
            Kc, J = (V, T) if cfg["domains"][i] == 0 else (T, V)
            shapes.append((B, Kc, J, J))
        saves = [torch.empty(2, sh[1], dtype=f32, device=dev) for sh in shapes]
        stats = [arena.take(2 * sh[1] * _lib.STAT_REPLICAS) for sh in shapes] if train else None
        e = [torch.empty(sh, dtype=f32, device=dev) for sh in shapes]
        adj = [torch.empty(sh, dtype=f32, device=dev) for sh in shapes]
        items = _Map2AdjTail._items(cfg, ts, train, saves, stats, e, dev, p)
        taps = cfg.get("taps")
        for i in range(n):
            items[i].adj = adj[i].data_ptr()
            if taps is not None:
                taps.append(torch.empty(shapes[i], dtype=f32, device=dev))
                items[i].tap = taps[-1].data_ptr()
        stream = _stream(ts[0])
        for phase in (1, 2):
            _lib.call("cg_map2adj_tail_fwd", items, n, phase, stream)
        ctx.cfg, ctx.p, ctx.n = cfg, p, n
        ctx.seed_epoch = seed_epoch(dev) if p > 0.0 else None
        ctx.save_for_backward(*ts, *e, *saves)
        return tuple(adj)

    @staticmethod
    def backward(ctx, *dadj):
        n, cfg = ctx.n, ctx.cfg
        sv = ctx.saved_tensors
        ts, e, saves = sv[:7 * n], sv[7 * n:8 * n], sv[8 * n:9 * n]
        dev, train, f32 = ts[0].device, bool(cfg["train"]), torch.float32
        if any(d is None for d in dadj):
            raise RuntimeError("map2adj_tail: every adjacency needs a gradient")
        _check_seed_epoch(ctx, dev, "map2adj_tail")
        dadj = [d if d.is_contiguous() else _copy(d) for d in dadj]
        items = _Map2AdjTail._items(cfg, ts, train, saves, None, e, dev, ctx.p)
        arena = _arena(dev)
        grads, keep = [], []
        stream = _stream(ts[0])
        for i in range(n):
            t = items[i]
            Kc = t.Kc
            ws = int(_lib.lib().cg_map2adj_tail_ws_floats(Kc))
            zb, _ = _zeros(ws, dev)
            red = arena.take(int(_lib.lib().cg_map2adj_tail_red_doubles(Kc)))
            g = torch.empty_like(e[i])
            part = torch.empty(int(_lib.lib().cg_map2adj_tail_part_floats(t.B, Kc, t.J)), dtype=f32, device=dev)
            t.part = part.data_ptr()
            keep += [g, zb, part]
            ds, dq = torch.empty_like(ts[7 * i]), torch.empty_like(ts[7 * i + 1])
            dw = torch.empty(2, Kc, Kc, dtype=f32, device=dev)
            small = torch.empty(3, Kc, dtype=f32, device=dev)
            t.dadj, t.g, t.red, t.ds, t.dq = dadj[i].data_ptr(), g.data_ptr(), red.data_ptr(), ds.data_ptr(), dq.data_ptr()
            t.dW0_ws, t.dW4_ws = zb[:ws // 2].data_ptr(), zb[ws // 2:].data_ptr()
            t.dW0, t.dW4, t.dgamma, t.dbeta, t.dalpha = dw[0].data_ptr(), dw[1].data_ptr(), small[0].data_ptr(), small[1].data_ptr(), small[2].data_ptr()
            grads += [ds, dq, dw[0].view(ts[7 * i + 2].shape), small[0], small[1], small[2, :1].reshape(1), dw[1].view(ts[7 * i + 6].shape)]
        for phase in (1, 2):
            _lib.call("cg_map2adj_tail_bwd", items, n, phase, stream)
        del keep
        return (None,) + tuple(g if ctx.needs_input_grad[1 + k] else None for k, g in enumerate(grads))


def map2adj_tail(seeds, expansors, train, drop_p=0.0, salts=(0, 0), taps=None):
    cfg = {"train": bool(train), "drop_p": float(drop_p), "salts": tuple(int(s) for s in salts), "domains": tuple(int(d) for d, _, _ in seeds),
           "bn": tuple(e[1] for e in expansors), "taps": taps}
    ts = []
    for (dom, s, q), e in zip(seeds, expansors):
        kc = e[0].out_channels
        ts += [s, q, e[0].weight.view(kc, kc), e[1].weight, e[1].bias, e[3].weight, e[4].weight.view(kc, kc)]
    return _Map2AdjTail.apply(cfg, *ts)


def block_input_ok(x):
    if x.dim() != 4 or not x.is_contiguous() or x.dtype != torch.float32:
        return False
    B, C, T, V = x.shape
    return bool(_lib.lib().cg_block_input_supported(B, C, T, V))


_BLOCK_INPUT_MAXG = 8


class _BlockInput(torch.autograd.Function):

    @staticmethod
    def _block(x, bn, save, train):
        B, C, T, V = x.shape
        t = _lib.BlockInput()
        t.B, t.C, t.T, t.V, t.train = B, C, T, V, 1 if train else 0
        t.x = x.data_ptr()
        _tail_bn(t.bn, bn, None, save, train)
        return t

    @staticmethod
    def forward(ctx, cfg, x, gamma, beta):
        ctx.set_materialize_grads(False)
        _chk(x)
        dev, f32, train, n = x.device, torch.float32, bool(cfg["train"]), int(cfg["n"])
        B, C, T, V = x.shape
        save = torch.empty(2, C, dtype=f32, device=dev)
        t = _BlockInput._block(x, cfg["bn"], save, train)
        stream = _stream(x)
        if train:
            if B * T * V <= 1:
                raise ValueError("Expected more than 1 value per channel when training, got input size %s" % (tuple(x.shape),))
            stats = cfg.get("stats")
            if stats is None:
                stats = _arena(dev).take(2 * C * _lib.STAT_REPLICAS)
                it = _lib.StatsArgs()
                it.x, it.xv, it.pre, it.stats = x.data_ptr(), _view4(x), None, stats.data_ptr()
                _lib.call("cg_chan_stats_many", (_lib.StatsArgs * 1)(it), 1, stream)
            t.bn.stats = stats.data_ptr()
        xn = torch.empty_like(x)
        rows = torch.empty(2, B, C, T, dtype=f32, device=dev)
# ... 722 lines not shown
```

include/cistgcn_hip.h:

```cpp
#ifndef CISTGCN_HIP_H
#define CISTGCN_HIP_H
#include <stdint.h>
#ifdef __cplusplus
extern "C" {
#endif

#define CG_STAT_REPLICAS 16
#define CG_ALPHA_SLOTS 64

typedef struct CgView4 {
  long long n[4];
  long long s[4];
} CgView4;

int cg_contract(const float* A, const float* X, float* Y, const float* bias, double* stats, const int32_t* tables,
                int G, int M, int N, int K, int splitk, int a_kfast, int x_kfast,
                long long y_dense_numel, void* stream);

typedef struct CgContractDesc {
  const float* A; const float* X; float* Y; const float* bias; double* stats; const int32_t* tab;
  int G, M, N, K, splitk, kchunk , a_kfast, x_kfast;
  int accumulate;
  int x_vec;
  int stat_ch;
  int mode;
  long long block0;
  float* ws;
  int chain;
  int pad2;
} CgContractDesc;
int cg_contract_many(const CgContractDesc* descs, int n, void* stream);
long long cg_contract_kred_ws_floats(int G, int M, int N);

int cg_chan_stats(const float* x, const CgView4* xv, const float* pre, double* stats, void* stream);
typedef struct CgStatsArgs { const float* x; CgView4 xv; const float* pre; double* stats; } CgStatsArgs;
int cg_chan_stats_many(const CgStatsArgs* items, int n, void* stream);
int cg_chan_sum(const float* x, const CgView4* xv, float* out, void* stream);

typedef struct CgNormAct {
  const float* x;  CgView4 xv;
  float* y;        CgView4 yv;
  const float* pre;
  const float* add; CgView4 av;
  int add_post;
  int bn_mode;
  const double* stats;
  const float* gamma; const float* beta;
  float* running_mean; float* running_var; long long* num_batches_tracked;
  float momentum, eps;
  float* save_mean; float* save_rstd;
  float drop_p; const unsigned long long* seed; unsigned int salt;
  const float* alpha; int alpha_n;
  const float* dy; CgView4 dyv;
  float* dx; CgView4 dxv;
  float* dadd; CgView4 dav;
  float* dpre;
  double* red;
  float* dgamma; float* dbeta; float* dalpha;
  double* ystats;
} CgNormAct;
int cg_norm_act_fwd(const CgNormAct* a, void* stream);
int cg_norm_act_bwd(const CgNormAct* a, int need_reduce, void* stream);
int cg_norm_act_fwd_many(const CgNormAct* arr, int n, void* stream);
int cg_norm_act_bwd_many(const CgNormAct* arr, const int* need_reduce, int n, void* stream);
int cg_norm_act_bwd_reduce_many(const CgNormAct* arr, int n, void* stream);

int cg_reduce_bc(const float* x, const CgView4* xv, int kind, float* out, int32_t* arg, void* stream);
int cg_reduce_bc_bwd(const float* dout, const int32_t* arg, int kind, float* dx, const CgView4* dxv, void* stream);

typedef struct CgSumItem { const float* a; CgView4 av; } CgSumItem;
int cg_sum_many(float* y, const CgView4* yv, const CgSumItem* items, int n, void* stream);
int cg_add3(float* y, const CgView4* yv, const float* a, const CgView4* av, const float* b, const CgView4* bv,
            const float* c, const CgView4* cv, void* stream);
typedef struct CgCopyItem { float* y; CgView4 yv; const float* a; CgView4 av; } CgCopyItem;
int cg_copy_many(const CgCopyItem* items, int n, void* stream);
int cg_zero(void* p, long long bytes, void* stream);

int cg_feature_lift_fwd(const float* x, float* f, long long B, long long T, long long V, void* stream);
int cg_feature_lift_bwd(const float* x, const float* df, float* dx, long long B, long long T, long long V, void* stream);
int cg_dstd_stats_fwd(const float* x, float* out, int B, int C, int T, int V, void* stream);
int cg_dstd_stats_bwd(const float* x, const float* dout, float* dx, int B, int C, int T, int V, void* stream);
int cg_se_gate_fwd(const float* pooled, const float* W1, const float* W2, float* gate, int B, int C, int H, void* stream);
int cg_se_gate_bwd(const float* pooled, const float* W1, const float* W2, const float* gate, const float* dgate,
                   float* dpooled, float* dW1, float* dW2, int B, int C, int H, int prezeroed, void* stream);
typedef struct CgRank1 { const float* s; const float* q; float* o; const float* dout; float* ds; float* dq; int domain; int pad; } CgRank1;
int cg_rank1_adj_fwd(const CgRank1* items, int n, int B, int T, int V, void* stream);
int cg_rank1_adj_bwd(const CgRank1* items, int n, int B, int T, int V, void* stream);
int cg_cumsum(const float* x, const CgView4* xv, float* y, const CgView4* yv, int reverse, void* stream);
int cg_mpjpe_fwd(const float* pred, const float* tgt, float* loss, long long N, void* stream);
int cg_mpjpe_bwd(const float* pred, const float* tgt, const float* gloss, float* dpred, long long N, void* stream);
int cg_seed_bump(unsigned long long* seed, void* stream);

long long cg_stgcn_domain_planes_min_workgroups(long long n);
int cg_stgcn_domain_fwd(const float* x, const float* adj, const float* W, const float* bias, float* y, double* ystats,
                        int B, int Cin, int Cout, int T, int V, int domain, void* stream);
long long cg_stgcn_domain_bwd_ws_floats(int Cin, int Cout);
int cg_stgcn_domain_bwd(const float* x, const float* adj, const float* W, const float* dy, float* dx, float* dadj,
                        float* dW, float* dbias, float* ws, int B, int Cin, int Cout, int T, int V, int domain,
                        int ws_prezeroed, void* stream);

typedef struct CgTailBN {
  double* stats;
  const float* gamma; const float* beta;
  float* running_mean; float* running_var; long long* num_batches_tracked;
  float momentum, eps;
  float* save;
} CgTailBN;
typedef struct CgDstdTail {
  int B, C, T, V, train, pad0;
  const float* y[2]; const float* r[2]; const float* w[2];
  CgTailBN bn_t[2]; const float* alpha_d[2];
  CgTailBN bn_p[2]; const float* alpha_p[2];
  const float* Wc; CgTailBN bn_c; const float* alpha_c;
  const float* gate; const float* bres;
  float drop_p; unsigned int salt[2]; int pad1; const unsigned long long* seed;
  float* h0; float* pooled; float* out; double* ostats;
  float* tap_x[2]; float* tap_a[2]; float* tap_h;
  const float* dout; const float* dpooled; float* dgate;
  double* red_c;
  float* gp[2]; double* red_p[2];
  float* dWc_ws; float* dWc;
  float* dr[2]; float* dw[2]; double* red_t[2]; float* dy[2];
  float* dgamma_t[2]; float* dbeta_t[2]; float* dalpha_d[2];
  float* dgamma_p[2]; float* dbeta_p[2]; float* dalpha_p[2];
  float* dgamma_c; float* dbeta_c; float* dalpha_c;
} CgDstdTail;
int cg_dstd_tail_fwd(const CgDstdTail* t, int phase, void* stream);
int cg_dstd_tail_bwd(const CgDstdTail* t, int phase, void* stream);
long long cg_dstd_tail_ws_floats(int C);

typedef struct CgRowsConv {
  int B, C, T, V, O, pad;
  const float* x; const float* W;
  float* y; double* stats;
  const float* dy; float* dx; float* dW;
  float* ws;
  int in_on, in_train;
  CgTailBN in_bn;
  const float* in_alpha;
  float* in_tap;
  double* sums;
  double* red;
  float* dgamma; float* dbeta; float* dalpha;
} CgRowsConv;
int cg_collapse_rows_fwd(const CgRowsConv* t, void* stream);
int cg_collapse_rows_bwd(const CgRowsConv* t, void* stream);
long long cg_collapse_rows_ws_floats(int C, int T, int O);
int cg_collapse_cols_fwd(const CgRowsConv* t, void* stream);
int cg_collapse_cols_bwd(const CgRowsConv* t, void* stream);
int cg_collapse_cols_supported(int C, int T, int V, int O);
long long cg_collapse_cols_ws_floats(int C, int V, int O);
long long cg_collapse_sums_ws_floats(int C, int rows);

typedef struct CgFpnConv {
  int B, C, O, H, W, n;
  int dil[3]; int pad;
  const float* x; long long xs[3];
  const float* w[3]; const float* bias[3];
  float* y[3];
  const float* dy[3];
  float* dx;
  float* dw[3]; float* db[3];
  float* ws;
} CgFpnConv;
int cg_fpn_conv_fwd(const CgFpnConv* t, void* stream);
int cg_fpn_conv_bwd(const CgFpnConv* t, void* stream);
int cg_fpn_conv_supported(int B, int C, int O, int H, int W);
long long cg_fpn_conv_ws_floats(int B, int C, int O, int n);

#define CG_PWM_MAXN 4
typedef struct CgPwMaps {
  int B, Cin, P, n;
  const float* x;
  const float* W[CG_PWM_MAXN]; int M[CG_PWM_MAXN];
  float* y[CG_PWM_MAXN];
  double* stats[CG_PWM_MAXN];
  const float* dy[CG_PWM_MAXN];
  float* dx;
  float* dW[CG_PWM_MAXN];
  float* dW_ws;
  const float* bias[CG_PWM_MAXN];
  float* db[CG_PWM_MAXN];
  const float* yraw[CG_PWM_MAXN];
  const float* bn_save[CG_PWM_MAXN]; const float* bn_gamma[CG_PWM_MAXN]; const float* bn_beta[CG_PWM_MAXN];
  const double* bn_red[CG_PWM_MAXN]; const float* prelu[CG_PWM_MAXN];
  int bn_train, pad;
} CgPwMaps;
int cg_pointwise_maps_fwd(const CgPwMaps* t, void* stream);
int cg_pointwise_maps_bwd(const CgPwMaps* t, void* stream);
long long cg_pointwise_maps_ws_floats(int Cin);

typedef struct CgAdjTail {
  int B, Kc, J, domain, train, pad0;
  const float* s; const float* q;
  const float* W0; CgTailBN bn; const float* alpha; const float* W4;
  float drop_p; unsigned int salt; const unsigned long long* seed;
  float* e; float* adj;
  float* tap;
  const float* dadj; float* g; double* red;
  float* ds; float* dq; float* part;
  float* dW0_ws; float* dW4_ws;
  float* dW0; float* dW4; float* dgamma; float* dbeta; float* dalpha;
} CgAdjTail;
int cg_map2adj_tail_fwd(const CgAdjTail* items, int n, int phase, void* stream);
int cg_map2adj_tail_bwd(const CgAdjTail* items, int n, int phase, void* stream);
long long cg_map2adj_tail_ws_floats(int Kc);
long long cg_map2adj_tail_part_floats(int B, int Kc, int J);
long long cg_map2adj_tail_red_doubles(int Kc);

#define CG_BIN_MAXG 8
typedef struct CgBlockInput {
  int B, C, T, V, train, ng;
  const float* x;
  CgTailBN bn;
  float* xn;
  float* rm; float* rq;
  float* out;
  const float* g[CG_BIN_MAXG];
  const float* dout[2];
  long long dout_ld[2];
  float* pq;
  float* gsum;
  double* red;
  float* dx; float* dgamma; float* dbeta;
} CgBlockInput;
int cg_block_input_fwd(const CgBlockInput* t, void* stream);
int cg_block_input_bwd(const CgBlockInput* t, void* stream);
int cg_block_input_supported(int B, int C, int T, int V);

typedef struct CgGatePath {
  const float* z;
  const float* stats; long long stats_ld;
  CgTailBN bn2; const float* alpha2;
  const float* Wl;
  CgTailBN bn3; const float* alpha3;
  const float* W2;
  unsigned int salt2, salt3;
  float* y;
  float* w;
  float* tap2; float* tap3;
  const float* dw;
  float* dz;
  float* dstats;
  float* dWl; float* dW2;
  float* dgamma2; float* dbeta2; float* dalpha2; float* dgamma3; float* dbeta3; float* dalpha3;
  float* scratch;
  double* red;
} CgGatePath;
typedef struct CgGateHead {
  int B, C, S, train, n, pad;
  float drop_p; int pad2; const unsigned long long* seed;
  CgGatePath p[2];
} CgGateHead;
int cg_gate_head_fwd(const CgGateHead* t, void* stream);
int cg_gate_head_bwd(const CgGateHead* t, void* stream);
int cg_gate_head_supported(int B, int C, int S);
long long cg_gate_head_scratch_floats(int B, int C, int S);

typedef struct CgMidItem {
  int kind, C, L, O;
  int sb_, ns_;
  const float* x; long long x_ld;
  CgTailBN bn; long long stats_ld;
  const float* alpha;
  const float* W;
  unsigned int salt; int pad;
  float* y;
  float* tap;
  const float* dy;
  float* dx;
  float* dW; float* dgamma; float* dbeta; float* dalpha;
  float* g;
  double* part;
  float* wpart;
} CgMidItem;
typedef struct CgBlockMid {
  int B, train, n, pad;
  float drop_p; int pad2; const unsigned long long* seed;
// ... 92 lines not shown
```

Measured before the change: 14970 sequences/sec.

## Precompute tail BN backward sums via forward moments and row sums, fuse final passes

During forward training, the tail now accumulates extra per-channel moments of the pre-activation slope terms. Backward gains per-(b,c) row sums and a small reduction kernel for the concat-BN statistics. Partial q-sums are collected inside the k3 kernel. Together these let the last two backward phases collapse into one fused k45 kernel that derives the time-BN reduction algebraically instead of doing a separate full pass, and shares the residual gradient buffer when both branches use the same residual. The cost is extra atomics, registers and an added float64 buffer, plus sensitivity to numerical differences in the reformulated sums.

```diff
diff --git a/cistgcn_amd/_lib.py b/cistgcn_amd/_lib.py
--- a/cistgcn_amd/_lib.py
+++ b/cistgcn_amd/_lib.py
@@ -84,7 +84,8 @@
                 ("dr", c_void_p * 2), ("dw", c_void_p * 2), ("red_t", c_void_p * 2), ("dy", c_void_p * 2),
                 ("dgamma_t", c_void_p * 2), ("dbeta_t", c_void_p * 2), ("dalpha_d", c_void_p * 2),
                 ("dgamma_p", c_void_p * 2), ("dbeta_p", c_void_p * 2), ("dalpha_p", c_void_p * 2),
-                ("dgamma_c", c_void_p), ("dbeta_c", c_void_p), ("dalpha_c", c_void_p)]
+                ("dgamma_c", c_void_p), ("dbeta_c", c_void_p), ("dalpha_c", c_void_p),
+                ("rows_c", c_void_p), ("fmom", c_void_p * 2), ("red_q", c_void_p * 2), ("rs_shared", c_int), ("pad2", c_int)]
 
 
 class AdjTail(ctypes.Structure):
diff --git a/cistgcn_amd/csrc/dstd_tail.h b/cistgcn_amd/csrc/dstd_tail.h
--- a/cistgcn_amd/csrc/dstd_tail.h
+++ b/cistgcn_amd/csrc/dstd_tail.h
@@ -30,4 +30,10 @@
   float* dgamma_t[2]; float* dbeta_t[2]; float* dalpha_d[2];
   float* dgamma_p[2]; float* dbeta_p[2]; float* dalpha_p[2];
   float* dgamma_c; float* dbeta_c; float* dalpha_c;
+  double* rows_c;
+  double* fmom[2];
+  double* red_q[2];
+  int rs_shared, pad2;
 };
+#define CG_TAIL_ROWSUMS 6
+#define CG_TAIL_FMOM 4
diff --git a/cistgcn_amd/csrc/dstd_tail.hip b/cistgcn_amd/csrc/dstd_tail.hip
--- a/cistgcn_amd/csrc/dstd_tail.hip
+++ b/cistgcn_amd/csrc/dstd_tail.hip
@@ -4,6 +4,12 @@
 #include <stdlib.h>
 
 HIP_DYNAMIC_SHARED(unsigned char, cg_dyn_lds)
+
+#if defined(__HIP_DEVICE_COMPILE__)
+#define CG_REFORM(x) asm volatile("" : "+v"(x))
+#else
+#define CG_REFORM(x) do { } while (0)
+#endif
 
 static int cg_tail_rows(long long B, long long C, long long P) {
   long long target = (B * C * P) / 2048;
@@ -28,8 +34,9 @@
 
 __device__ __forceinline__ void cg_tail_keep4(const CgDstdTail& t, int i, unsigned long long seed, unsigned long long idx0, float keep[4]);
 
+template <bool MOM>
 __global__ void cg_tail_f1_kernel(CgDstdTail t, int rb) {
-  __shared__ double red[32];
+  __shared__ double red[32 + 16 * CG_TAIL_FMOM];
   const int i = blockIdx.z, c = blockIdx.x, b0 = blockIdx.y * rb;
   if (b0 >= t.B) return;
   const int P = t.T * t.V, nb = min(rb, t.B - b0), C = t.C;
@@ -41,6 +48,7 @@
   const float* __restrict__ y = t.y[i]; const float* __restrict__ r = t.r[i];
   float* const tap = t.tap_x[i];
   double s = 0.0, q = 0.0;
+  double mom[CG_TAIL_FMOM] = {0.0, 0.0, 0.0, 0.0};
   for (int br = wave; br < nb; br += nw) {
     const int b = b0 + br;
     const long long base = ((long long)b * C + c) * P;
@@ -58,6 +66,10 @@
           xv[j] = cg_tail_x(at, ad, yv[j], rv[j], keep[j], u);
           const double z = (double)(wv * xv[j]);
           s += z; q += z * z;
+          if (MOM) {
+            const double qd = (double)(keep[j] * (u > 0.f ? 1.f : ad) * wv), yh = (double)((yv[j] - at.mean) * at.rstd), qz = qd * z;
+            mom[0] += qd; mom[1] += qz; mom[2] += qd * yh; mom[3] += qz * yh;
+          }
         }
         if (tap) *reinterpret_cast<float4*>(tap + base + p) = make_float4(xv[0], xv[1], xv[2], xv[3]);
       }
@@ -76,6 +88,15 @@
   if (threadIdx.x == 0) {
     double* rep = t.bn_p[i].stats + (long long)(blockIdx.y % CG_STAT_REPLICAS) * 2 * C;
     atomicAdd(&rep[2 * c], s); atomicAdd(&rep[2 * c + 1], q);
+  }
+  if (MOM) {
+#pragma unroll
+    for (int k = 0; k < CG_TAIL_FMOM; ++k) mom[k] = cg_block_sum(mom[k], red + 32 + 16 * k);
+    if (threadIdx.x == 0) {
+      double* rep = t.fmom[i] + ((long long)(blockIdx.y % CG_STAT_REPLICAS) * C + c) * CG_TAIL_FMOM;
+#pragma unroll
+      for (int k = 0; k < CG_TAIL_FMOM; ++k) atomicAdd(&rep[k], mom[k]);
+    }
   }
 }
 
@@ -156,9 +177,11 @@
 
 template <int PT>
 __device__ __forceinline__ void cg_tail_act_finish(const CgTailHot& t, const float* sK, unsigned long long seed, int b, int p0, int np,
-                                                   const float4 yq[PT / 8], const float4 rq[PT / 8], const float wq[PT / 8], float* img, int what) {
+                                                   const float4 yq[PT / 8], const float4 rq[PT / 8], const float wq[PT / 8], float* img, int what,
+                                                   unsigned int* qbits = nullptr, bool want_bits = false) {
   constexpr int PS = PT + 4;
   const int C = t.C, P = t.P;
+  unsigned int bits = 0;
 #pragma unroll
   for (int q = 0; q < PT / 8; ++q) {
     const int i = q / (PT / 16), e = threadIdx.x + (q - i * (PT / 16)) * CG_TAIL_THREADS;
@@ -179,6 +202,7 @@
         xv[j] = cg_prelu(u, k0.w);
         const float z = wv * xv[j];
         val[j] = what == 0 ? cg_prelu(cg_tail_pre_p(z, k1.x, k1.y, k1.z, k1.w), ap) : (z - k1.x) * k1.y;
+        if (PT == 32 && want_bits) bits |= ((keep[j] > 0.f ? 1u : 0u) | (u > 0.f ? 2u : 0u)) << ((8 * q + 2 * j) & 31);
       }
       if (what == 0) {
         if (t.tap_a[i]) *reinterpret_cast<float4*>(t.tap_a[i] + off) = make_float4(val[0], val[1], val[2], val[3]);
@@ -187,6 +211,7 @@
     }
     *reinterpret_cast<float4*>(img + c2 * PS + pp) = make_float4(val[0], val[1], val[2], val[3]);
   }
+  if (PT == 32 && qbits) *qbits = bits;
 }
 
 template <int PT>
@@ -447,6 +472,7 @@
   }
 }
 
+template <bool ROWS>
 __global__ void cg_tail_k1_kernel(CgDstdTail t, int rb) {
   const int c = blockIdx.x, b0 = blockIdx.y * rb, P = t.T * t.V, C = t.C;
   if (b0 >= t.B) return;
@@ -457,18 +483,55 @@
     const int b = b0 + br;
     const long long base = ((long long)b * C + c) * P;
     float s = 0.f;
+    float rs[CG_TAIL_ROWSUMS] = {0.f, 0.f, 0.f, 0.f, 0.f, 0.f};
+    auto rows = [&](float d, float h0v) {
+      const float u = cg_bn(ac, h0v), hh = (h0v - ac.mean) * ac.rstd;
+      const bool pos = u > 0.f;
+      const float sl = pos ? 1.f : alpha, ds = d * sl;
+      rs[0] += ds; rs[1] += sl; rs[2] += ds * hh; rs[3] += sl * hh;
+      rs[4] += pos ? 0.f : d * u; rs[5] += pos ? 0.f : u;
+    };
     if ((P & 3) == 0) {
       for (int p = 4 * lane; p < P; p += 256) {
         const float4 d4 = *reinterpret_cast<const float4*>(t.dout + base + p), h4 = *reinterpret_cast<const float4*>(t.h0 + base + p);
         s += (d4.x * cg_prelu(cg_bn(ac, h4.x), alpha) + d4.y * cg_prelu(cg_bn(ac, h4.y), alpha)) +
              (d4.z * cg_prelu(cg_bn(ac, h4.z), alpha) + d4.w * cg_prelu(cg_bn(ac, h4.w), alpha));
+        if (ROWS) { rows(d4.x, h4.x); rows(d4.y, h4.y); rows(d4.z, h4.z); rows(d4.w, h4.w); }
       }
     } else {
-      for (int p = lane; p < P; p += 64) s += t.dout[base + p] * cg_prelu(cg_bn(ac, t.h0[base + p]), alpha);
+      for (int p = lane; p < P; p += 64) {
+        s += t.dout[base + p] * cg_prelu(cg_bn(ac, t.h0[base + p]), alpha);
+        if (ROWS) rows(t.dout[base + p], t.h0[base + p]);
+      }
     }
     const double sd = cg_wave_sum((double)s);
     if (lane == 0) t.dgate[(long long)b * C + c] = (float)sd;
-  }
+    if (ROWS) {
+      double* dst = t.rows_c + ((long long)b * C + c) * CG_TAIL_ROWSUMS;
+#pragma unroll
+      for (int k = 0; k < CG_TAIL_ROWSUMS; ++k) {
+        const double v = cg_wave_sum((double)rs[k]);
+        if (lane == 0) dst[k] = v;
+      }
+    }
+  }
+}
+
+__global__ void cg_tail_k2_rows_kernel(CgDstdTail t) {
+  __shared__ double red[48];
+  const int c = blockIdx.x, C = t.C;
+  const double invP = 1.0 / (double)(t.T * t.V);
+  double s1 = 0.0, s2 = 0.0, sa = 0.0;
+  for (int b = threadIdx.x; b < t.B; b += blockDim.x) {
+    const long long bc = (long long)b * C + c;
+    const double* r = t.rows_c + bc * CG_TAIL_ROWSUMS;
+    const double gate = (double)t.gate[bc], dp = (double)t.dpooled[bc] * invP;
+    s1 += gate * r[0] + dp * r[1]; s2 += gate * r[2] + dp * r[3]; sa += gate * r[4] + dp * r[5];
+  }
+  s1 = cg_block_sum(s1, red); s2 = cg_block_sum(s2, red + 16); sa = cg_block_sum(sa, red + 32);
+  if (threadIdx.x == 0) { t.red_c[2 * c] = s1; t.red_c[2 * c + 1] = s2; t.red_c[2 * C + c] = sa; }
+  if (c == 0)
+    for (int k = C + threadIdx.x; k < CG_ALPHA_SLOTS; k += blockDim.x) t.red_c[2 * C + k] = 0.0;
 }
 
 __device__ __forceinline__ float cg_tail_gc(const CgDstdTail& t, const CgAff& ac, float alpha, long long off, int b, int c, float invP, float& u) {
@@ -574,15 +637,27 @@
   for (int i = 0; i < CG_TAIL_K3_TASKS * 3; ++i) (&racc[0][0])[i] = 0.f;
   CG_TSTAMP();
   const bool vec = (P & 3) == 0;
+  const bool qsum = train && vec && t.red_q[0] != nullptr;
+  const float qkeep = (hot.train && hot.drop_p > 0.f) ? 1.0f / (1.0f - hot.drop_p) : 1.f;
+  const float alpha_d0 = __builtin_bit_cast(float, __builtin_amdgcn_readfirstlane(__builtin_bit_cast(int, t.alpha_d[0][0])));
+  const float alpha_d1 = __builtin_bit_cast(float, __builtin_amdgcn_readfirstlane(__builtin_bit_cast(int, t.alpha_d[1][0])));
+  float4 yk[CG_TAIL_PT3 / 8];
+  float wk[CG_TAIL_PT3 / 8];
+  unsigned int qbits = 0;
+  float qacc[CG_TAIL_PT3 / 8][2];
+#pragma unroll
+  for (int i = 0; i < CG_TAIL_PT3 / 8; ++i) qacc[i][0] = qacc[i][1] = 0.f;
   constexpr int DQ = CG_TAIL_PT3 / 16;
   float4 yq[CG_TAIL_PT3 / 8], rq[CG_TAIL_PT3 / 8];
   float wq[CG_TAIL_PT3 / 8];
   float4 h4[DQ], d4[DQ];
   float gt[DQ], dp[DQ];
   auto dh_load = [&](int b, int p0, int np) {
+    int tidr = tid;
+    CG_REFORM(tidr);
 #pragma unroll
     for (int q = 0; q < DQ; ++q) {
-      const int e = tid + q * CG_TAIL_THREADS, c = e / (CG_TAIL_PT3 / 4), pp = 4 * (e - c * (CG_TAIL_PT3 / 4));
+      const int e = tidr + q * CG_TAIL_THREADS, c = e / (CG_TAIL_PT3 / 4), pp = 4 * (e - c * (CG_TAIL_PT3 / 4));
       h4[q] = make_float4(0.f, 0.f, 0.f, 0.f); d4[q] = h4[q]; gt[q] = 0.f; dp[q] = 0.f;
       if (c < C && pp < np) {
         const long long off = ((long long)b * C + c) * P + p0 + pp;
@@ -603,7 +678,13 @@
     __syncthreads();
     CG_TSTAMP();
     if (vec) {
-      cg_tail_act_finish<CG_TAIL_PT3>(hot, sK, seed, b, p0, np, yq, rq, wq, sZ, 1);
+      unsigned int nbits = 0;
+      cg_tail_act_finish<CG_TAIL_PT3>(hot, sK, seed, b, p0, np, yq, rq, wq, sZ, 1, &nbits, qsum);
+      if (qsum) {
+        qbits = nbits;
+#pragma unroll
+        for (int q = 0; q < CG_TAIL_PT3 / 8; ++q) { yk[q] = yq[q]; wk[q] = wq[q]; }
+      }
       CG_TSTAMP();
 #pragma unroll
       for (int q = 0; q < DQ; ++q) {
@@ -703,6 +784,7 @@
     }
     CG_TSTAMP();
     static_assert(CG_TAIL_PT3 == 32, "one pair of position tiles per task: task w = channel tile w");
+    if (!MT_ && qsum) __syncthreads();
     cg_f32x4 dacc[CG_TAIL_K3_TASKS][2];
     if (MT_) {
 #pragma unroll
@@ -748,14 +830,16 @@
           }
         }
       }
-      const int c2 = 16 * mt + l15;
+      int l15e = l15, slote = slot;
+      CG_REFORM(l15e); CG_REFORM(slote);
+      const int c2 = 16 * mt + l15e;
       const bool cok = c2 < C2;
       const int i = c2 >= C ? 1 : 0, c = cok ? c2 - i * C : 0;
       const float gam = cok ? sK[8 * c2 + 6] : 0.f, bet = cok ? sK[8 * c2 + 7] : 0.f, alp = cok ? (i ? alpha_p1 : alpha_p0) : 0.f;
       float* gpr = (i ? gp1 : gp0) + ((long long)b * C + c) * P + p0;
 #pragma unroll
       for (int h = 0; h < 2; ++h) {
-        const int pq = (h ? n1 : n0) + 4 * slot;
+        const int pq = (h ? n1 : n0) + 4 * slote;
         const cg_f32x4 cc = h ? c1 : c0;
         if (cok && pq < np) {
           const float4 z4 = *reinterpret_cast<const float4*>(sZ + c2 * CG_TAIL_PS3 + pq);
@@ -771,10 +855,33 @@
               if (!(v > 0.f)) racc[ti][2] += da * v;
             }
           }
+          if (qsum) *reinterpret_cast<float4*>(sZ + c2 * CG_TAIL_PS3 + pq) = make_float4(gq[0], gq[1], gq[2], gq[3]);
           if (vec) *reinterpret_cast<float4*>(gpr + pq) = make_float4(gq[0], gq[1], gq[2], gq[3]);
           else {
 #pragma unroll
             for (int q = 0; q < 4; ++q) if (pq + q < np) gpr[pq + q] = gq[q];
+          }
+        }
+      }
+    }
+    if (qsum) {
+      __syncthreads();
+#pragma unroll
+      for (int q = 0; q < CG_TAIL_PT3 / 8; ++q) {
+        constexpr int QH = CG_TAIL_PT3 / 16;
+        const int i = q / QH, e = tid + (q - i * QH) * CG_TAIL_THREADS;
+        const int c = e / (CG_TAIL_PT3 / 4), pp = 4 * (e - c * (CG_TAIL_PT3 / 4)), c2 = i * C + c;
+        if (c < C && pp < np) {
+          const float4 g4 = *reinterpret_cast<const float4*>(sZ + c2 * CG_TAIL_PS3 + pp);
+          const float mt = sK[8 * c2];
+          const float fa = qkeep * wk[q], fb = fa * (i ? alpha_d1 : alpha_d0);
+          const float gv[4] = {g4.x, g4.y, g4.z, g4.w}, yv[4] = {yk[q].x, yk[q].y, yk[q].z, yk[q].w};
+#pragma unroll
+          for (int j = 0; j < 4; ++j) {
+            const unsigned int bj = qbits >> (8 * q + 2 * j);
+            const float f = (bj & 1u) ? ((bj & 2u) ? fa : fb) : 0.f;
+            const float fg = f * gv[j];
+            qacc[q][0] += fg; qacc[q][1] += fg * (yv[j] - mt);
           }
         }
       }
@@ -791,6 +898,21 @@
     s1 += __shfl_xor(s1, 32, 64); s2 += __shfl_xor(s2, 32, 64); sa += __shfl_xor(sa, 32, 64);
     if (slot == 0 && c2 < C2) {
       atomicAdd(&sRed[2 * c2], (double)s1); atomicAdd(&sRed[2 * c2 + 1], (double)s2); atomicAdd(&sRed[2 * C2M + (c2 >= C ? 1 : 0)], (double)sa);
+    }
+  }
+  if (qsum) {
+#pragma unroll
+    for (int q = 0; q < CG_TAIL_PT3 / 8; ++q) {
+      constexpr int QH = CG_TAIL_PT3 / 16;
+      const int i = q / QH, c = (tid + (q - i * QH) * CG_TAIL_THREADS) / (CG_TAIL_PT3 / 4);
+      float q1 = qacc[q][0], q2 = qacc[q][1];
+      q1 += __shfl_xor(q1, 1, 64); q2 += __shfl_xor(q2, 1, 64);
+      q1 += __shfl_xor(q1, 2, 64); q2 += __shfl_xor(q2, 2, 64);
+      q1 += __shfl_xor(q1, 4, 64); q2 += __shfl_xor(q2, 4, 64);
+      if ((tid & 7) == 0 && c < C) {
+        double* rq2 = (i ? t.red_q[1] : t.red_q[0]) + ((long long)(blockIdx.x % CG_STAT_REPLICAS) * C + c) * 2;
+        atomicAdd(&rq2[0], (double)q1); atomicAdd(&rq2[1], (double)q2);
+      }
     }
   }
   __syncthreads();
@@ -937,6 +1059,114 @@
   }
 }
 
+template <bool SHARED>
+__global__ void cg_tail_k45_kernel(CgDstdTail t, int rb) {
+  constexpr int ND = SHARED ? 2 : 1;
+  const int i0 = SHARED ? 0 : blockIdx.z, c = blockIdx.x, b0 = blockIdx.y * rb, P = t.T * t.V, C = t.C;
+  if (b0 >= t.B) return;
+  const int nb = min(rb, t.B - b0), lane = threadIdx.x & 63, wave = __builtin_amdgcn_readfirstlane(threadIdx.x >> 6), nw = blockDim.x >> 6;
+  const double cnt = (double)t.B * P;
+  const bool train = t.train != 0;
+  const unsigned long long seed = (t.train && t.drop_p > 0.f) ? *t.seed : 0ull;
+  CgAff at[ND], ap[ND];
+  float ad[ND], scale_p[ND], m1[ND], m2[ND], scale_t[ND], mt1[ND], rmt2[ND];
+  const float* __restrict__ yp[ND]; const float* __restrict__ gpp[ND]; float* __restrict__ dyp[ND];
+#pragma unroll
+  for (int d = 0; d < ND; ++d) {
+    const int i = i0 + d;
+    at[d] = cg_tail_aff(t.bn_t[i], c, C, 0.0, t.train, true, false);
+    ap[d] = cg_tail_aff(t.bn_p[i], c, C, 0.0, t.train, true, false);
+    ad[d] = t.alpha_d[i][0]; scale_p[d] = ap[d].gamma * ap[d].rstd; scale_t[d] = at[d].gamma * at[d].rstd;
+    m1[d] = m2[d] = mt1[d] = rmt2[d] = 0.f;
+    yp[d] = t.y[i]; gpp[d] = t.gp[i]; dyp[d] = t.dy[i];
+    if (train) {
+      m1[d] = (float)(t.red_p[i][2 * c] / cnt); m2[d] = (float)(t.red_p[i][2 * c + 1] / cnt);
+      double M[CG_TAIL_FMOM] = {0.0, 0.0, 0.0, 0.0};
+      for (int r = 0; r < CG_STAT_REPLICAS; ++r)
+#pragma unroll
+        for (int k = 0; k < CG_TAIL_FMOM; ++k) M[k] += t.fmom[i][((long long)r * C + c) * CG_TAIL_FMOM + k];
+      double A1 = 0.0, B1 = 0.0;
+      for (int r = 0; r < CG_STAT_REPLICAS; ++r) { A1 += t.red_q[i][((long long)r * C + c) * 2]; B1 += t.red_q[i][((long long)r * C + c) * 2 + 1]; }
+      B1 *= (double)at[d].rstd;
+      const double mp = (double)ap[d].mean, rp = (double)ap[d].rstd;
+      const double A3 = rp * (M[1] - mp * M[0]), B3 = rp * (M[3] - mp * M[2]);
+      const double St = (double)scale_p[d] * (A1 - (double)m1[d] * M[0] - (double)m2[d] * A3);
+      const double Sty = (double)scale_p[d] * (B1 - (double)m1[d] * M[2] - (double)m2[d] * B3);
+      mt1[d] = (float)(St / cnt); rmt2[d] = at[d].rstd * (float)(Sty / cnt);
+      if (blockIdx.y == 0 && threadIdx.x == 0) { t.red_t[i][2 * c] = St; t.red_t[i][2 * c + 1] = Sty; }
+    }
+  }
+  const float* __restrict__ r0p = t.r[i0]; float* __restrict__ dr0p = t.dr[i0];
+  double sa[ND], s1[ND], s2[ND];
+#pragma unroll
+  for (int d = 0; d < ND; ++d) sa[d] = s1[d] = s2[d] = 0.0;
+  for (int br = wave; br < nb; br += nw) {
+    const int b = b0 + br;
+    const long long base = ((long long)b * C + c) * P;
+    float wv[ND], sw[ND];
+#pragma unroll
+    for (int d = 0; d < ND; ++d) { wv[d] = t.w[i0 + d][(long long)b * C + c]; sw[d] = 0.f; }
+    for (int p = 4 * lane; p < P; p += 256) {
+      const float4 r4 = *reinterpret_cast<const float4*>(r0p + base + p);
+      const float rv[4] = {r4.x, r4.y, r4.z, r4.w};
+      float gsum[4] = {0.f, 0.f, 0.f, 0.f};
+#pragma unroll
+      for (int d = 0; d < ND; ++d) {
+        float keep[4];
+        cg_tail_keep4(t, i0 + d, seed, (unsigned long long)(base + p), keep);
+        const float4 y4 = *reinterpret_cast<const float4*>(yp[d] + base + p), g4 = *reinterpret_cast<const float4*>(gpp[d] + base + p);
+        const float yv[4] = {y4.x, y4.y, y4.z, y4.w}, gv[4] = {g4.x, g4.y, g4.z, g4.w};
+        float o[4];
+#pragma unroll
+        for (int j = 0; j < 4; ++j) {
+          float u;
+          const float x = cg_tail_x(at[d], ad[d], yv[j], rv[j], keep[j], u);
+          const float z = wv[d] * x;
+          const float dz = train ? scale_p[d] * (gv[j] - m1[d] - (z - ap[d].mean) * ap[d].rstd * m2[d]) : gv[j] * scale_p[d];
+          sw[d] += dz * x;
+          const float dx = wv[d] * dz;
+          const float gd = u > 0.f ? dx : ad[d] * dx;
+          if (!(u > 0.f)) sa[d] += (double)dx * (double)u;
+          gsum[j] = SHARED ? gsum[j] + gd : gd;
+          o[j] = train ? scale_t[d] * (gd * keep[j] - mt1[d] - (yv[j] - at[d].mean) * rmt2[d]) : gd * keep[j] * scale_t[d];
+          if (!train) { const float gt = gd * keep[j]; s1[d] += (double)gt; s2[d] += (double)gt * (double)((yv[j] - at[d].mean) * at[d].rstd); }
+        }
+        *reinterpret_cast<float4*>(dyp[d] + base + p) = make_float4(o[0], o[1], o[2], o[3]);
+      }
+      *reinterpret_cast<float4*>(dr0p + base + p) = make_float4(gsum[0], gsum[1], gsum[2], gsum[3]);
+    }
+#pragma unroll
+    for (int d = 0; d < ND; ++d) {
+      const double swd = cg_wave_sum((double)sw[d]);
+      if (lane == 0) t.dw[i0 + d][(long long)b * C + c] = (float)swd;
+    }
+  }
+#pragma unroll
+  for (int d = 0; d < ND; ++d) {
+    const double s = cg_wave_sum(sa[d]);
+    if (lane == 0) atomicAdd(&t.red_t[i0 + d][2 * C + ((c + 5 * (int)blockIdx.y + 17 * wave) & (CG_ALPHA_SLOTS - 1))], s);
+    if (!train) {
+      const double e1 = cg_wave_sum(s1[d]), e2 = cg_wave_sum(s2[d]);
+      if (lane == 0) { atomicAdd(&t.red_t[i0 + d][2 * c], e1); atomicAdd(&t.red_t[i0 + d][2 * c + 1], e2); }
+    }
+  }
+}
+
+__global__ void cg_tail_params_kernel(CgDstdTail t) {
+  const int C = t.C;
+  for (int e = threadIdx.x; e < 2 * C; e += blockDim.x) {
+    const int i = e / C, c = e - i * C;
+    t.dgamma_t[i][c] = (float)t.red_t[i][2 * c + 1]; t.dbeta_t[i][c] = (float)t.red_t[i][2 * c];
+    t.dgamma_p[i][c] = (float)t.red_p[i][2 * c + 1]; t.dbeta_p[i][c] = (float)t.red_p[i][2 * c];
+    if (i == 0) { t.dgamma_c[c] = (float)t.red_c[2 * c + 1]; t.dbeta_c[c] = (float)t.red_c[2 * c]; }
+  }
+  if (threadIdx.x < 2) {
+    const int i = threadIdx.x;
+    t.dalpha_d[i][0] = (float)cg_alpha_sum(t.red_t[i] + 2 * C); t.dalpha_p[i][0] = (float)cg_alpha_sum(t.red_p[i] + 2 * C);
+  }
+  if (threadIdx.x == 64) t.dalpha_c[0] = (float)cg_alpha_sum(t.red_c + 2 * C);
+}
+
 __global__ void cg_tail_fold_kernel(const float* __restrict__ ws, int replicas, int n, float* __restrict__ dW) {
   const int i = blockIdx.x * blockDim.x + threadIdx.x;
   if (i >= n) return;
@@ -1000,7 +1230,9 @@
   if (phase == 1) {
     if (!t->train) return CG_OK;
     if (!t->bn_t[0].stats || !t->bn_t[1].stats || !t->bn_p[0].stats || !t->bn_p[1].stats) return CG_EARG;
-    hipLaunchKernelGGL(cg_tail_f1_kernel, dim3(rows.x, rows.y, 2), dim3(256), 0, stream, *t, rb);
+    if ((t->fmom[0] != nullptr) != (t->fmom[1] != nullptr)) return CG_EARG;
+    if (t->fmom[0] && (P & 3) == 0) hipLaunchKernelGGL(cg_tail_f1_kernel<true>, dim3(rows.x, rows.y, 2), dim3(256), 0, stream, *t, rb);
+    else hipLaunchKernelGGL(cg_tail_f1_kernel<false>, dim3(rows.x, rows.y, 2), dim3(256), 0, stream, *t, rb);
   } else if (phase == 2) {
     if (t->train && (!t->bn_p[0].stats || !t->bn_p[1].stats || !t->bn_c.stats)) return CG_EARG;
     const CgTailRanges rg = cg_tail_ranges(t->B, P, CG_TAIL_PT);
@@ -1029,20 +1261,27 @@
   return cg_launch_status();
 }
 
+static bool cg_tail_last_pass(const CgDstdTail* t) { return t->red_q[0] && t->red_q[1] && ((t->T * t->V) & 3) == 0; }
+
 extern "C" int cg_dstd_tail_bwd(const CgDstdTail* t, int phase, void* stream_) {
   int st = cg_tail_check(t);
   if (st != CG_OK) return st;
   if (!t->dout || !t->gate) return CG_EARG;
+  if ((t->red_q[0] != nullptr) != (t->red_q[1] != nullptr)) return CG_EARG;
+  if (t->rs_shared && (t->r[0] != t->r[1] || !cg_tail_last_pass(t))) return CG_EARG;
   hipStream_t stream = (hipStream_t)stream_;
   const int P = t->T * t->V, C = t->C;
   const int rb = cg_tail_rows(t->B, C, P);
   const dim3 rows = cg_tail_row_grid(t->B, C, rb);
   if (phase == 1) {
     if (!t->dgate) return CG_EARG;
-    hipLaunchKernelGGL(cg_tail_k1_kernel, rows, dim3(256), 0, stream, *t, rb);
+    if (t->rows_c) hipLaunchKernelGGL(cg_tail_k1_kernel<true>, rows, dim3(256), 0, stream, *t, rb);
+    else hipLaunchKernelGGL(cg_tail_k1_kernel<false>, rows, dim3(256), 0, stream, *t, rb);
   } else if (phase == 2) {
     if (!t->dpooled || !t->red_c) return CG_EARG;
-    hipLaunchKernelGGL(cg_tail_k2_kernel, rows, dim3(256), 0, stream, *t, rb);
+    static_assert(CG_ALPHA_SLOTS >= 64, "cg_tail_k2_rows_kernel: one slope word per channel, C <= 64");
+    if (t->rows_c) hipLaunchKernelGGL(cg_tail_k2_rows_kernel, dim3((unsigned)C), dim3(256), 0, stream, *t);
+    else hipLaunchKernelGGL(cg_tail_k2_kernel, rows, dim3(256), 0, stream, *t, rb);
   } else if (phase == 3) {
     if (!t->dpooled || !t->red_c || !t->gp[0] || !t->gp[1] || !t->red_p[0] || !t->red_p[1] || !t->dWc_ws || !t->dWc) return CG_EARG;
     const CgTailRanges rg = cg_tail_ranges(t->B, P, CG_TAIL_PT3);
@@ -1066,9 +1305,26 @@
     const int n = C * 2 * C;
     hipLaunchKernelGGL(cg_tail_fold_kernel, dim3((unsigned)((n + 255) / 256)), dim3(256), 0, stream, t->dWc_ws, CG_TAIL_REPLICAS, n, t->dWc);
   } else if (phase == 4) {
-    if (!t->gp[0] || !t->gp[1] || !t->dr[0] || !t->dr[1] || !t->dw[0] || !t->dw[1] || !t->red_t[0] || !t->red_t[1] || !t->red_p[0]) return CG_EARG;
-    hipLaunchKernelGGL(cg_tail_k4_kernel, dim3(rows.x, rows.y, 2), dim3(256), 0, stream, *t, rb);
+    if (!t->gp[0] || !t->gp[1] || !t->dr[0] || !t->dw[0] || !t->dw[1] || !t->red_t[0] || !t->red_t[1] || !t->red_p[0] || !t->red_p[1]) return CG_EARG;
+    if (cg_tail_last_pass(t)) {
+      if (!t->dy[0] || !t->dy[1]) return CG_EARG;
+      if (t->train && (!t->fmom[0] || !t->fmom[1])) return CG_EARG;
+      if (t->rs_shared) hipLaunchKernelGGL(cg_tail_k45_kernel<true>, dim3(rows.x, rows.y, 1), dim3(256), 0, stream, *t, rb);
+      else {
+        if (!t->dr[1]) return CG_EARG;
+        hipLaunchKernelGGL(cg_tail_k45_kernel<false>, dim3(rows.x, rows.y, 2), dim3(256), 0, stream, *t, rb);
+      }
+    } else {
+      if (!t->dr[1]) return CG_EARG;
+      hipLaunchKernelGGL(cg_tail_k4_kernel, dim3(rows.x, rows.y, 2), dim3(256), 0, stream, *t, rb);
+    }
+  } else if (phase == 6) {
+    if (!t->red_c || !t->red_t[0] || !t->red_t[1] || !t->red_p[0] || !t->red_p[1] || !t->dgamma_t[0] || !t->dgamma_t[1] || !t->dbeta_t[0] || !t->dbeta_t[1] ||
+        !t->dgamma_p[0] || !t->dgamma_p[1] || !t->dbeta_p[0] || !t->dbeta_p[1] || !t->dalpha_d[0] || !t->dalpha_d[1] || !t->dalpha_p[0] || !t->dalpha_p[1] ||
+        !t->dgamma_c || !t->dbeta_c || !t->dalpha_c) return CG_EARG;
+    hipLaunchKernelGGL(cg_tail_params_kernel, dim3(1), dim3(128), 0, stream, *t);
   } else if (phase == 5) {
+    if (cg_tail_last_pass(t)) return CG_EARG;
     if (!t->dy[0] || !t->dy[1] || !t->dr[0] || !t->dr[1] || !t->red_t[0] || !t->red_t[1] || !t->dgamma_t[0] || !t->dgamma_p[0] || !t->dgamma_c) return CG_EARG;
     hipLaunchKernelGGL(cg_tail_k5_kernel, dim3(rows.x, rows.y, 2), dim3(256), 0, stream, *t, rb);
   } else return CG_EARG;
diff --git a/cistgcn_amd/models/CISTGCN/CISTGCN.py b/cistgcn_amd/models/CISTGCN/CISTGCN.py
--- a/cistgcn_amd/models/CISTGCN/CISTGCN.py
+++ b/cistgcn_amd/models/CISTGCN/CISTGCN.py
@@ -194,6 +194,7 @@
         self.fused_maps = True
         self.fused_defer = True
         self.fused_mid = True
+        self.fused_tail_sums = True
         self.stack_min_elements = 1 << 21
         widths = [self.in_ch] + list(p.input_gcn.model_complexity) + [self.in_ch]
         widths_o = [3] + list(p.output_gcn.model_complexity)
@@ -632,10 +633,12 @@
             if self.drop_trace is not None:
                 self.drop_trace[doms[0].tcn[1]], self.drop_trace[doms[1].tcn[1]] = self._site - 1, self._site
             taps = [] if self.act_trace is not None else None
+            rs_shared = self.fused_tail_sums and not has_res and res[0].data_ptr() == res[1].data_ptr()
             out, ost = ops.dstd_tail([y[0] for y in ys], [y[1] for y in ys], res, (m.w1, m.w2),
                                      (doms[0].tcn[1], doms[1].tcn[1], m.prelu1[0], m.prelu2[0], c[1]),
                                      (doms[0].prelu, doms[1].prelu, m.prelu1[1], m.prelu2[1], c[2]), c[0].weight, c[3], bres, tr,
-                                     drop_p=self.dropout, salts=(self._site - 1, self._site), emit_stats=tr, taps=taps)
+                                     drop_p=self.dropout, salts=(self._site - 1, self._site), emit_stats=tr, taps=taps,
+                                     tail_sums=self.fused_tail_sums, rs_shared=rs_shared)
             if taps is not None:
                 for mod, tap in zip((doms[0].prelu, doms[1].prelu, m.prelu1[1], m.prelu2[1], c[2]), taps):
                     self.act_trace[mod] = (tap, None)
diff --git a/cistgcn_amd/ops.py b/cistgcn_amd/ops.py
--- a/cistgcn_amd/ops.py
+++ b/cistgcn_amd/ops.py
@@ -1627,6 +1627,13 @@
                 taps.append(torch.empty(B, C, T, V, dtype=f32, device=dev))
             t.tap_x[0], t.tap_x[1], t.tap_a[0], t.tap_a[1], t.tap_h = (v.data_ptr() for v in taps[-5:])
         stream = _stream(y1)
+        last_pass = bool(cfg.get("tail_sums", True)) and (T * V) % 4 == 0
+        fmom = None
+        if cfg.get("rs_shared") and r1.data_ptr() != r2.data_ptr():
+            raise ValueError("dstd_tail: rs_shared needs r1 and r2 to be the same tensor")
+        if last_pass and train:
+            fmom = arena.take(2 * _lib.STAT_REPLICAS * C * 4).view(2, -1)
+            t.fmom[0], t.fmom[1] = fmom[0].data_ptr(), fmom[1].data_ptr()
         for phase in (1, 2, 3):
             _lib.call("cg_dstd_tail_fwd", ctypes.byref(t), phase, stream)
         gate = torch.empty(B, C, dtype=f32, device=dev)
@@ -1635,8 +1642,9 @@
         t.gate = gate.data_ptr()
         _lib.call("cg_dstd_tail_fwd", ctypes.byref(t), 4, stream)
         ctx.cfg, ctx.p = cfg, p
+        ctx.last_pass, ctx.has_fmom = last_pass, fmom is not None
         ctx.seed_epoch = seed_epoch(dev) if p > 0.0 else None
-        ctx.save_for_backward(*ts, h0, pooled, gate, saves)
+        ctx.save_for_backward(*ts, h0, pooled, gate, saves, *([fmom] if fmom is not None else []))
         if ostats is not None:
             ctx.mark_non_differentiable(ostats)
         return out, ostats
@@ -1645,7 +1653,8 @@
     def backward(ctx, dout, _=None):
         sv = ctx.saved_tensors
         (y1, y2, r1, r2, w1, w2, gt1, bt1, ad1, gt2, bt2, ad2, gp1, bp1, ap1, gp2, bp2, ap2, wc, gc, bc, ac, sw1, sw2, bres) = sv[:25]
-        h0, pooled, gate, saves = sv[25:]
+        h0, pooled, gate, saves = sv[25:29]
+        fmom = sv[29] if ctx.has_fmom else None
         cfg = ctx.cfg
         _check_seed_epoch(ctx, y1.device, "dstd_tail")
         B, C, T, V = y1.shape
@@ -1667,6 +1676,9 @@
         stream = _stream(y1)
         dgate = torch.empty(B, C, dtype=f32, device=dev)
         t.dgate = dgate.data_ptr()
+        if cfg.get("tail_sums", True):
+            rows_c = torch.empty(B, C, 6, dtype=torch.float64, device=dev)
+            t.rows_c = rows_c.data_ptr()
         _lib.call("cg_dstd_tail_bwd", ctypes.byref(t), 1, stream)
         H = sw1.shape[0]
         dpooled = torch.empty(B, C, dtype=f32, device=dev)
@@ -1679,21 +1691,32 @@
         red_c = arena.take(2 * C + _lib.ALPHA_SLOTS)
         red_p = [arena.take(2 * C + _lib.ALPHA_SLOTS) for _ in range(2)]
         red_t = [arena.take(2 * C + _lib.ALPHA_SLOTS) for _ in range(2)]
-        big = [torch.empty(B, C, T, V, dtype=f32, device=dev) for _ in range(6)]
+        shared = ctx.last_pass and bool(cfg.get("rs_shared"))
+        big = [None if (k == 3 and shared) else torch.empty(B, C, T, V, dtype=f32, device=dev) for k in range(6)]
         dws = [torch.empty(B, C, dtype=f32, device=dev) for _ in range(2)]
         small = torch.empty(15, C, dtype=f32, device=dev)
         dwc = torch.empty(C, 2 * C, dtype=f32, device=dev)
         t.dpooled, t.red_c = dpooled.data_ptr(), red_c.data_ptr()
         for i in range(2):
-            t.gp[i], t.red_p[i], t.dr[i], t.dw[i], t.red_t[i], t.dy[i] = (big[i].data_ptr(), red_p[i].data_ptr(), big[2 + i].data_ptr(),
+            t.gp[i], t.red_p[i], t.dr[i], t.dw[i], t.red_t[i], t.dy[i] = (big[i].data_ptr(), red_p[i].data_ptr(), _ptr(big[2 + i]),
                                                                           dws[i].data_ptr(), red_t[i].data_ptr(), big[4 + i].data_ptr())
             t.dgamma_t[i], t.dbeta_t[i], t.dgamma_p[i], t.dbeta_p[i] = (small[2 * i].data_ptr(), small[2 * i + 1].data_ptr(),
                                                                         small[4 + 2 * i].data_ptr(), small[5 + 2 * i].data_ptr())
             t.dalpha_d[i], t.dalpha_p[i] = small[10 + i].data_ptr(), small[12 + i].data_ptr()
         t.dgamma_c, t.dbeta_c, t.dalpha_c = small[8].data_ptr(), small[9].data_ptr(), small[14].data_ptr()
         t.dWc_ws, t.dWc = zb[2 * C * H:].data_ptr(), dwc.data_ptr()
-        for phase in (2, 3, 4, 5):
+        if ctx.last_pass:
+            red_q = arena.take(2 * _lib.STAT_REPLICAS * 2 * C).view(2, -1)
+            t.red_q[0], t.red_q[1] = red_q[0].data_ptr(), red_q[1].data_ptr()
+            if fmom is not None:
+                t.fmom[0], t.fmom[1] = fmom[0].data_ptr(), fmom[1].data_ptr()
+            t.rs_shared = 1 if shared else 0
+        for phase in ((2, 3, 4, 6) if ctx.last_pass else (2, 3, 4, 5)):
             _lib.call("cg_dstd_tail_bwd", ctypes.byref(t), phase, stream)
+        sums_tap = cfg.get("sums_tap")
+        if sums_tap is not None:
+            sums_tap.update(red_c=red_c.clone(), red_t=[r.clone() for r in red_t], red_p=[r.clone() for r in red_p],
+                            dr1=big[3], last_pass=ctx.last_pass, shared=shared)
         al = lambda k: small[k, :1].reshape(1)
         grads = (big[4], big[5], big[2], big[3], dws[0], dws[1],
                  small[0], small[1], al(10), small[2], small[3], al(11),
@@ -1702,10 +1725,12 @@
         return (None,) + tuple(g if ctx.needs_input_grad[1 + k] else None for k, g in enumerate(grads))
 
 
-def dstd_tail(ys, ystats, rs, ws, bns, alphas, wc, se, bres, train, drop_p=0.0, salts=(0, 0), emit_stats=False, taps=None):
+def dstd_tail(ys, ystats, rs, ws, bns, alphas, wc, se, bres, train, drop_p=0.0, salts=(0, 0), emit_stats=False, taps=None, tail_sums=True,
+              rs_shared=False, sums_tap=None):
     C = ys[0].shape[1]
     cfg = {"train": bool(train), "drop_p": float(drop_p), "salts": tuple(int(s) for s in salts), "ystats": tuple(ystats), "bn": tuple(bns),
-           "emit_stats": bool(emit_stats), "taps": taps}
+           "emit_stats": bool(emit_stats), "taps": taps, "tail_sums": bool(tail_sums),
+           "rs_shared": bool(rs_shared), "sums_tap": sums_tap}
     ts = (ys[0], ys[1], rs[0], rs[1], ws[0], ws[1],
           bns[0].weight, bns[0].bias, alphas[0].weight, bns[1].weight, bns[1].bias, alphas[1].weight,
           bns[2].weight, bns[2].bias, alphas[2].weight, bns[3].weight, bns[3].bias, alphas[3].weight,
diff --git a/include/cistgcn_hip.h b/include/cistgcn_hip.h
--- a/include/cistgcn_hip.h
+++ b/include/cistgcn_hip.h
@@ -124,6 +124,10 @@
   float* dgamma_t[2]; float* dbeta_t[2]; float* dalpha_d[2];
   float* dgamma_p[2]; float* dbeta_p[2]; float* dalpha_p[2];
   float* dgamma_c; float* dbeta_c; float* dalpha_c;
+  double* rows_c;
+  double* fmom[2];
+  double* red_q[2];
+  int rs_shared, pad2;
 } CgDstdTail;
 int cg_dstd_tail_fwd(const CgDstdTail* t, int phase, void* stream);
 int cg_dstd_tail_bwd(const CgDstdTail* t, int phase, void* stream);
```

New measurement: 15240 sequences/sec (median of 6 runs). 1.8% higher.
